# youmi-zym/TemporalStereo

Hardware: AMD Instinct MI355X
Metric: stereo pairs/sec, FlyingThings3D 540x960 D=192 (aggregation hot path) (higher is better)
Workload: dtype f32

## Files before the change

include/ts_hip.h:

```cpp
#ifndef TS_HIP_H
#define TS_HIP_H

#include <stddef.h>
#include <stdint.h>

#ifdef __cplusplus
extern "C" {
#endif

#define TS_OK 0
#define TS_ERR_NULL (-1)
#define TS_ERR_SHAPE (-2)
#define TS_ERR_UNSUPPORTED (-3)
#define TS_ERR_ALIGN (-4)

int ts_version(void);
const char* ts_last_error_string(void);

size_t ts_block_cost_workspace_bytes(int B, int C, int H, int W, int D, int scales);

int ts_block_cost_int_fwd(const float* left, const float* right, float* out, void* workspace,
                          int B, int C, int H, int W, int D, int scales, void* stream);

int ts_block_cost_sampled_fwd(const float* left, const float* right, const float* disp, float* out,
// ... 92 lines not shown

size_t ts_wasserstein_loss_workspace_bytes(int B, int H, int W);
int ts_wasserstein_loss_fwd(const float* cost, const float* offset, const float* sample, const float* gt, float* loss,
                            float* gt_scaled, void* workspace, int B, int D, int H, int W, int Hg, int Wg, float max_disp,
                            float start_disp, int sparse, void* stream);
int ts_wasserstein_loss_bwd(const float* cost, const float* offset, const float* sample, const float* gt_scaled,
                            const float* grad_loss, float* grad_cost, float* grad_offset, int B, int D, int H, int W, int Wg,
                            float max_disp, float start_disp, void* stream);
size_t ts_disp_smooth_l1_workspace_bytes(int B, int Hg, int Wg);
int ts_disp_smooth_l1_fwd(const float* est, const float* gt, float* loss_count, void* workspace, int B, int h, int w, int Hg,
                          int Wg, float max_disp, float start_disp, void* stream);
int ts_disp_smooth_l1_bwd(const float* est, const float* gt, const float* grad_loss, const float* loss_count, float* grad_est,
                          int B, int h, int w, int Hg, int Wg, float max_disp, float start_disp, void* stream);

size_t ts_disp_metrics_workspace_bytes(int B, int Hg, int Wg);
int ts_disp_metrics_fwd(const float* est0, const float* est1, const float* est2, const float* est3, int n_est, int h0, int w0,
                        int h1, int w1, int h2, int w2, int h3, int w3, const float* gt, const float* gt_right, int B, int Hg,
                        int Wg, float lb, float ub, int flags, float* out, void* workspace, void* stream);

#define TS_RENDER_EST_COLOR 1
#define TS_RENDER_GT_COLOR 2
#define TS_RENDER_ERR_CLASS 4
#define TS_RENDER_ERR_JET 8
#define TS_RENDER_U16 16
#define TS_RENDER_UINT8 32
#define TS_RENDER_CHW 64
#define TS_RENDER_BAR 128
#define TS_RENDER_CLIP 256
#define TS_RENDER_MAX_SHARED 512
#define TS_RENDER_MAX_GIVEN 1024
#define TS_RENDER_STATS_FLOATS 32
size_t ts_disp_render_workspace_bytes(int B, int Hg, int Wg);
int ts_disp_render_fwd(const float* est, const float* gt, const float* max_disp, const float* jet, int B, int h, int w, int Hg,
                       int Wg, int flags, float scale16, void* disp_color, void* err_class, void* err_jet, void* disp_u16,
                       float* stats, void* workspace, void* stream);

#define TS_FLOW_SPARSE 1
#define TS_FLOW_EST_HWC 2
#define TS_FLOW_GT_HWC 4
#define TS_FLOW_RENDER_EST_COLOR 1
#define TS_FLOW_RENDER_GT_COLOR 2
#define TS_FLOW_RENDER_ERR_CLASS 4
#define TS_FLOW_RENDER_STATS 8
#define TS_FLOW_RENDER_UINT8 16
#define TS_FLOW_RENDER_CHW 32
#define TS_FLOW_RENDER_MAX_SHARED 64
#define TS_FLOW_RENDER_MAX_GIVEN 128
#define TS_FLOW_RENDER_EST_HWC 256
#define TS_FLOW_RENDER_GT_HWC 512
#define TS_FLOW_STATS_FLOATS 16
#define TS_FLOW_U16_CHW 1
size_t ts_flow_metrics_workspace_bytes(int B, int Hg, int Wg);
int ts_flow_metrics_fwd(const float* est0, const float* est1, const float* est2, const float* est3, int n_est, int h0, int w0,
                        int h1, int w1, int h2, int w2, int h3, int w3, const float* gt, int B, int Hg, int Wg, float lb, float ub,
                        int flags, float* out, void* workspace, void* stream);
size_t ts_flow_render_workspace_bytes(int B, int Hg, int Wg);
int ts_flow_render_fwd(const float* est, const float* gt, const float* gt_val, const float* max_rad, const float* wheel, int B,
                       int h, int w, int Hg, int Wg, int flags, void* flow_color, void* err_class, float* stats, void* workspace,
                       void* stream);
int ts_flow_u16_decode_fwd(const void* raw, int B, int H, int W, int flags, float* flow, void* valid, void* stream);

#define TS_PREPARE_CHW 1
int ts_frames_prepare_fwd(const void* left, const void* right, int B, int Hs, int Ws, int flags, float mean0, float mean1,
                          float mean2, float std0, float std1, float std2, int H, int W, const int* crop, float* color_l,
                          float* color_r, long long color_stride, float* color_aug_l, float* color_aug_r,
                          long long color_aug_stride, void* stream);
int ts_intrinsics_pyramid_fwd(const void* K_norm, int is_fp64, int B, int kh, int kw, int S, float* K, float* inv_K, void* stream);
int ts_disp_u16_decode_fwd(const void* raw, int B, int H, int W, float scale, float* disp, void* valid, void* stream);

#define TS_AUGMENT_ROW_INTS 96
#define TS_AUGMENT_MAX_RECTS 4
#define TS_AUGMENT_GAMMA 1
size_t ts_frames_augment_workspace_bytes(int B, int Hs, int Ws);
int ts_frames_augment_fwd(const void* left, const void* right, int B, int Hs, int Ws, int flags, float mean0, float mean1,
                          float mean2, float std0, float std1, float std2, int H, int W, const int* table, float* color_l,
                          float* color_r, long long color_stride, float* color_aug_l, float* color_aug_r,
                          long long color_aug_stride, void* workspace, size_t workspace_bytes, void* stream);
int ts_disp_u16_window_fwd(const void* raw, int B, int Hs, int Ws, int H, int W, const int* table, float scale, float* disp,
                           void* valid, void* stream);

int ts_topk_softargmax_fwd(const float* cost, const float* sample, const float* offset, float* disp,
                           float* topk_disp, float* topk_cost, int* topk_index,
                           int B, int D, int H, int W, int k, void* stream);

int ts_topk_softargmax_bwd(const float* topk_disp, const float* topk_cost, const int* topk_index,
                           const float* disp, const float* grad_disp, const float* grad_topk_disp,
                           const float* grad_topk_cost, float* grad_cost, float* grad_sample,
                           int B, int D, int H, int W, int k, void* stream);

int ts_softargmin_fwd(const float* cost, const float* sample, float* disp, float temperature,
                      int normalize, int B, int D, int H, int W, void* stream);

int ts_softargmin_bwd(const float* cost, const float* sample, const float* disp, const float* grad_disp,
                      float* grad_cost, float* grad_sample, float temperature, int normalize,
                      int B, int D, int H, int W, void* stream);

int ts_argmax_select_fwd(const float* cost, const float* sample, float* disp, int* index,
                         int B, int D, int H, int W, void* stream);

int ts_softsplat_sum_fwd(const float* input, const float* flow, float* output,
                         int B, int C, int H, int W, void* stream);
int ts_softsplat_sum_fwd_deterministic(const float* input, const float* flow, float* output, void* workspace,
                                       int B, int C, int H, int W, void* stream);
int ts_softsplat_sum_bwd_input(const float* flow, const float* grad_output, float* grad_input,
                               int B, int C, int H, int W, void* stream);
int ts_softsplat_sum_bwd_flow(const float* input, const float* flow, const float* grad_output,
                              float* grad_flow, int B, int C, int H, int W, void* stream);
size_t ts_softsplat_softmax_workspace_bytes(int B, int C, int H, int W);
int ts_softsplat_softmax_fwd(const float* input, const float* flow, const float* metric, float* output,
                             void* workspace, int B, int C, int H, int W, void* stream);
int ts_project_to_3d_fwd(const float* depth, const float* K, const float* inv_K, const float* T,
                         float* triangular_depth, float* optical_flow, unsigned char* flow_mask,
                         int B, int C, int H, int W, int k_dim, int inv_k_dim, float eps, void* stream);

#define TS_WARP_DISPARITY 0
#define TS_WARP_FLOW 1
#define TS_WARP_DEPTH 2
#define TS_WARP_BILINEAR 0
#define TS_WARP_NEAREST 1
#define TS_WARP_BICUBIC 2
#define TS_WARP_ZEROS 0
#define TS_WARP_BORDER 1
#define TS_WARP_REFLECTION 2
int ts_inverse_warp_fwd(const float* img, const float* motion, const float* K, const float* inv_K, const float* T, float* out,
                        float* triangular_depth, float* src_pixel_coord, float* optical_flow, unsigned char* flow_mask,
                        float* homo_points_3d, int B, int C, int Hi, int Wi, int H, int W, int mode, int interp, int pad,
                        int k_dim, int inv_k_dim, float eps, void* stream);
int ts_inverse_warp_bwd(const float* img, const float* motion, const float* K, const float* inv_K, const float* T,
                        const float* grad_out, float* grad_img, float* grad_motion, int B, int C, int Hi, int Wi, int H, int W,
                        int mode, int interp, int pad, int k_dim, int inv_k_dim, float eps, void* stream);

int ts_raft_corr_pyramid_fwd(const float* fmap1, const float* fmap2, float* pyramid, int B, int C, int H, int W, int num_levels,
                             void* stream);
int ts_raft_corr_lookup_fwd(const float* pyramid, const float* disp, float* out, int B, int H, int W, int num_levels, int radius,
                            void* stream);
int ts_raft_corr_lookup_bwd(const float* pyramid, const float* disp, const float* grad_out, float* grad_disp, float* grad_pyramid,
                            int B, int H, int W, int num_levels, int radius, int fold, void* stream);
int ts_raft_corr_pyramid_bwd(const float* grad_pyramid, const float* fmap1, const float* fmap2, float* grad_fmap1, float* grad_fmap2,
                             int B, int C, int H, int W, int levels, void* stream);

int ts_flow_corr_pyramid_fwd(const float* fmap1, const float* fmap2, float* pyramid, int B, int C, int H, int W, int num_levels,
                             void* stream);
int ts_flow_corr_lookup_fwd(const float* pyramid, const float* coords, float* out, int B, int H, int W, int num_levels, int radius,
                            void* stream);
int ts_flow_corr_lookup_bwd(const float* pyramid, const float* coords, const float* grad_out, float* grad_coords, float* grad_pyramid,
                            int B, int H, int W, int num_levels, int radius, int fold, void* stream);
int ts_flow_corr_pyramid_bwd(const float* grad_pyramid, const float* fmap1, const float* fmap2, float* grad_fmap1, float* grad_fmap2,
                             int B, int C, int H, int W, int levels, void* stream);

int ts_spp3d_pool_fwd(const float* x, float* pooled, int B, int C, int D, int H, int W, int num_levels, int s0, int s1, int s2, int s3,
                      long long x_bstride, long long x_cstride, void* stream);
int ts_spp3d_pool_bwd(const float* g0, const float* g1, const float* g2, const float* g3, const float* addend, float* grad_x, int B,
                      int C, int D, int H, int W, int num_levels, int s0, int s1, int s2, int s3, long long addend_bstride,
                      long long addend_cstride, long long gx_bstride, long long gx_cstride, void* stream);
int ts_spp3d_expand_fwd(const float* x, const float* lv0, const float* lv1, const float* lv2, const float* lv3, float* cat, int B, int C,
                        int Cl, int D, int H, int W, int num_levels, int s0, int s1, int s2, int s3, long long x_bstride,
                        long long x_cstride, void* stream);
int ts_spp3d_expand_bwd(const float* grad_cat, float* g0, float* g1, float* g2, float* g3, int B, int C, int Cl, int D, int H, int W,
                        int num_levels, int s0, int s1, int s2, int s3, long long g_bstride, long long g_cstride, void* stream);
int ts_depth_sum3_fwd(const float* z0, const float* z1, const float* z2, const float* scale, const float* shift, float* y, int B, int C,
                      int D, int H, int W, int act, long long z0_bstride, long long z0_cstride, long long z1_bstride,
                      long long z1_cstride, long long z2_bstride, long long z2_cstride, long long y_bstride, long long y_cstride,
                      void* stream);

int ts_bn_small_train_bwd(const float* y, const float* g, const float* gamma, const float* beta, float* sum_g, float* sum_gx, float* dy,
                          int B, int C, int N, long long y_bstride, long long y_cstride, long long g_bstride, long long g_cstride,
                          long long dy_bstride, long long dy_cstride, float eps, int act, void* stream);

size_t ts_reproject_memory_workspace_bytes(int B, int h, int w, int k, int n_local_out);
int ts_reproject_memory_fwd(const float* prev_disp, long long disp_bstride, int full_h, int full_w,
                            const float* mem_disp, const float* mem_cost, int k,
                            const float* local_map, int n_local_in, int n_local_out,
                            const float* K, int k_dim, const float* T_a, const float* T_b,
                            const float* baseline_ptr, float baseline, float factor,
                            float* out_disp, float* out_cost, float* out_local, void* workspace,
                            int B, int h, int w, void* stream);

int ts_conv_cout_pad(int cout);
int ts_conv_weight_layout(const float* w, float* out, int A, int T, int nb, int bpad, long long stride_a, long long stride_b,
                          long long stride_t, int flip, void* stream);
typedef struct {
  const float* w; float* out;
  int A, T, nb, bpad;
  long long stride_a, stride_b, stride_t;
  int flip, reserved;
} ts_weight_layout_desc;
int ts_conv_weight_layout_many(const void* table, int n, int blocks_x, void* stream);
typedef struct {
  const float* w; float* out;
  int A, T, nb, col0;
  long long stride_a, stride_b, stride_t;
  long long out_stride_a, out_stride_t;
  int flip, reserved;
} ts_weight_layout_desc2;
int ts_conv_weight_layout_many2(const void* table, int n, int blocks_x, void* stream);
typedef struct { const float* part; float* dw; int gx, nitems, cob, Cin, Cout, KT, ciblocks, block0; } ts_wgrad_finish_desc;
int ts_conv_wgrad_defer(int on);
int ts_conv_wgrad_pending(void);
int ts_conv_wgrad_take(void* host_table, size_t capacity_bytes, int* n, int* total_blocks);
int ts_conv_wgrad_finish_many(const void* table, int n, int total_blocks, void* stream);
int ts_conv_set_chunk_cap(int cap);
int ts_conv3d_hw_fwd(const float* x, const float* w_t, const float* scale, const float* shift, float* y,
                     int B, int Cin, int Cout, int D, int H, int W, int stride, int dilation,
                     int transposed, int act, float act_param,
                     long long in_bstride, long long in_cstride, long long out_bstride,
                     long long out_cstride, const float* addend, long long addend_bstride,
                     void* workspace, size_t workspace_bytes, void* stream);
size_t ts_conv3d_hw_warp_workspace_bytes(int B, int Cout, int D, int H, int W);
int ts_conv3d_hw_warp_fwd(const float* corr, const float* w_t, const float* scale, const float* shift, float* y,
                          const float* q, const float* disp, const float* base,
                          int B, int Cc, int Cout, int D, int H, int W, int dilation, int act, float act_param,
                          long long in_bstride, long long in_cstride, long long out_bstride, long long out_cstride,
                          long long base_bstride, void* workspace, size_t workspace_bytes, void* stream);

size_t ts_conv3d_hw_workspace_bytes(int B, int Cin, int Cout, int D, int H, int W, int stride, int transposed);
int ts_conv3d_hw_x6_supported(int Cin, int Cout, int W, int stride, int dilation, int transposed);
size_t ts_conv3d_hw_x6_weight_bytes(int Cin, int Cout);
size_t ts_conv3d_hw_x6_workspace_bytes(int B, int Cin, int Cout, int D, int H, int W);
int ts_conv3d_hw_x6_weight_split(const float* w_t, void* w6, int Cin, int Cout, void* stream);
int ts_conv3d_hw_x6_weight_split_from(const float* w, void* w6, int Cin, int Cout, long long stride_ci, long long stride_co,
                                      long long stride_t, int flip, void* stream);
int ts_conv3d_hw_x6_fwd(const float* x, const void* w6, const float* scale, const float* shift, float* y,
                        int B, int Cin, int Cout, int D, int H, int W, int dilation, int act, float act_param,
                        long long in_bstride, long long in_cstride, long long out_bstride, long long out_cstride,
                        const float* addend, long long addend_bstride, void* workspace, size_t workspace_bytes, void* stream);
typedef struct ts_peer_ctx {
  void* region[8];
  int rank, world;
} ts_peer_ctx;
size_t ts_peer_region_bytes(void);
int ts_peer_max_floats(void);
int ts_peer_max_ranks(void);
int ts_peer_alloc(void** region, void* handle64);
int ts_peer_open(const void* handle64, void** region);
int ts_peer_close(void* region);
int ts_peer_free(void* region);
int ts_peer_status(const void* ctx, int* status, void* stream);
int ts_peer_status_async(const void* ctx, int* host_status, void* stream);
long long ts_peer_set_timeout_ms(long long ms);
int ts_peer_reset(const void* ctx, void* stream);
int ts_peer_all_gather(const void* ctx, const float* src, float* dst, int n, void* stream);
int ts_peer_all_reduce_sum(const void* ctx, float* buf, int n, const float* scale, void* stream);

int ts_conv3d_hw_x6s_supported(int Cin, int Cout, int H, int W, int mode);
size_t ts_conv3d_hw_x6s_weight_bytes(int Cin, int Cout, int mode);
int ts_conv3d_hw_x6s_weight_split(const float* w_t, void* w6, int Cin, int Cout, int w_pad, int mode, void* stream);
int ts_conv3d_hw_x6s_fwd(const float* x, const void* w6, const float* scale, const float* shift, float* y,
                         int B, int Cin, int Cout, int D, int H, int W, int mode, int act, float act_param,
                         long long in_bstride, long long in_cstride, long long out_bstride, long long out_cstride, void* stream);
int ts_conv3d_d_fwd(const float* x, const float* w_t, const float* scale, const float* shift, float* y,
                    int B, int Cin, int Cout, int Din, int H, int W, int k, int stride, int dilation,
                    int padding, int transposed, int act, float act_param,
                    long long in_bstride, long long in_cstride, long long out_bstride,
                    long long out_cstride, void* stream);
size_t ts_conv3d_bwd_weight_workspace_bytes(int Cin, int Cout, int taps);
int ts_conv3d_hw_bwd_data(const float* dy, const float* w_b, float* dx, int B, int Cin, int Cout, int D, int H, int W,
                          int stride, int dilation, int transposed, long long dy_bstride, long long dy_cstride,
                          long long dx_bstride, long long dx_cstride, void* stream);
int ts_conv3d_hw_bwd_weight(const float* x, const float* dy, float* dw, int B, int Cin, int Cout, int D, int H, int W,
                            int stride, int dilation, long long x_bstride, long long x_cstride, long long dy_bstride,
                            long long dy_cstride, void* workspace, size_t workspace_bytes, void* stream);
int ts_conv3d_d_bwd_data(const float* dy, const float* w_b, float* dx, int B, int Cin, int Cout, int Din, int H, int W,
                         int k, int stride, int dilation, int padding, int transposed, long long dy_bstride,
                         long long dy_cstride, long long dx_bstride, long long dx_cstride, void* stream);
int ts_conv3d_d_bwd_weight(const float* x, const float* dy, float* dw, int B, int Cin, int Cout, int Din, int H, int W,
                           int k, int stride, int dilation, int padding, long long x_bstride, long long x_cstride,
                           long long dy_bstride, long long dy_cstride, void* workspace, size_t workspace_bytes,
                           void* stream);
int ts_resize3d_add_act_fwd(const float* a, const float* add, float* out, int B, int C, int Da, int Ha, int Wa,
                            int D, int H, int W, int act, long long a_bstride, long long a_cstride,
                            long long add_bstride, long long add_cstride, long long out_bstride,
                            long long out_cstride, void* stream);
int ts_pool3d5_avgmax_fwd(const float* x, float* out_avg, float* out_max, int B, int C, int D, int H, int W,
                          long long x_bstride, long long x_cstride, long long avg_bstride, long long avg_cstride,
                          long long max_bstride, long long max_cstride, void* stream);
int ts_merge_candidates_fwd(const float* volume, const float* sample, const float* mem_sample, const float* mem_cost,
                            const float* past_w, const float* past_scale, const float* past_shift,
                            float* out_sample, float* out_volume, int B, int C, int D0, int K, int H, int W,
                            long long vol_bstride, long long vol_cstride, long long out_bstride,
                            long long out_cstride, void* stream);
int ts_convex_upsample_fwd(const float* mask, const float* disp, float* out, int B, int H, int W, int factor,
                           float disp_scale, void* stream);
int ts_convex_upsample_candidates_fwd(const float* mask, const float* disp, float* out, float* low, float* high,
                                      float* candidates, int B, int H, int W, int factor, float disp_scale, float range,
                                      int channel_offset, int channels_total, void* stream);
int ts_unet_upsample_fwd(const float* mask, const float* disp, float* out, int B, int h, int w, int Ho, int Wo,
                         void* stream);
int ts_convex_upsample_bwd(const float* mask, const float* disp, const float* grad_out, float* grad_mask, float* grad_disp,
                           int B, int H, int W, int factor, float disp_scale, void* stream);
int ts_unet_upsample_bwd(const float* mask, const float* disp, const float* grad_out, float* grad_mask, float* grad_disp,
                         void* workspace, int B, int h, int w, int Ho, int Wo, void* stream);
int ts_deconv2d_k4s2_fwd(const float* x, const float* w_t, const float* scale, const float* shift, float* y,
                         int B, int Cin, int Cout, int H, int W, int act, long long out_bstride, void* stream);
int ts_resize_bilinear_fwd(const float* x, float* out, int B, int C, int h, int w, int Ho, int Wo, float value_scale,
                           long long out_bstride, void* stream);
int ts_resize_bilinear_pair_fwd(const float* x0, const float* x1, float* out0, float* out1, int B, int C, int h, int w,
                                int Ho, int Wo, float value_scale0, float value_scale1, void* stream);
int ts_range_candidates_fwd(const float* disp, float* low, float* high, float* candidates, int B, int H, int W,
                            float range, int channel_offset, int channels_total, void* stream);

int ts_resize3d_add_act_bwd(const float* a, const float* add, const float* grad_out, float* grad_a, float* grad_add,
                            int B, int C, int Da, int Ha, int Wa, int D, int H, int W, int act, void* stream);
int ts_pool3d5_avgmax_bwd(const float* x, const float* grad_avg, const float* grad_max, float* grad_x,
                          int B, int C, int D, int H, int W, void* stream);
int ts_merge_candidates_bwd(const float* sample, const float* grad_out_volume, const float* grad_out_sample,
                            float* grad_volume, float* grad_sample, int B, int C, int DT, int H, int W, void* stream);

int ts_channel_splice_fwd(const float* first, const float* second, float* out, int B, int C, int mc, long long N,
                          long long first_bstride, long long second_bstride, long long out_bstride, void* stream);
int ts_copy_rows_fwd(const float* src, float* dst, long long rows, long long row_elems, long long src_pitch,
                     long long dst_pitch, void* stream);

typedef struct ts_opt_entry { float* param; const float* grad; float* square_avg; long long n; } ts_opt_entry;
int ts_candidates_in_range_fwd(const float* low, const float* high, float* candidates, int B, int H, int W,
                               int channel_offset, int channels_total, void* stream);
int ts_candidates_in_range_bwd(const float* low, const float* high, const float* grad_candidates, float* grad_low,
                               float* grad_high, int B, int H, int W, int channel_offset, int channels_total, void* stream);
int ts_offset_head_fwd(const float* x, float* y, long long n, float delta, void* stream);
int ts_offset_head_bwd(const float* x, const float* grad_y, float* grad_x, long long n, float delta, void* stream);
int ts_space_to_depth2_fwd(const float* x, float* z, int B, int C, int H, int W, void* stream);
int ts_deconv2d_k4s2_weight_to_conv3(const float* w, float* out, int Cin, int Cout, int cin_pad, void* stream);
int ts_deconv2d_k4s2_wgrad_from_conv3(const float* dw3, float* dw, int Cin, int Cout, void* stream);
typedef struct ts_bn_fold_entry { const float* gamma; const float* beta; const float* mean; const float* var; const float* bias;
                                  float* scale; float* shift; int C, pad; } ts_bn_fold_entry;
int ts_bn_fold_many(const void* table, int n, float eps, void* stream);
size_t ts_clip_rmsprop_workspace_bytes(int n_tensors);
int ts_clip_rmsprop_step(const void* table, int n_tensors, float max_norm, float lr, float alpha, float eps,
                         void* workspace, size_t workspace_bytes, void* stream);

typedef struct ts_plan ts_plan;
ts_plan* ts_plan_create(void);
void ts_plan_destroy(ts_plan* plan);
// ... 14 lines not shown
```

temporalstereo_amd/_lib.py:

```python
import ctypes
import os
import threading

_HERE = os.path.dirname(os.path.abspath(__file__))
LIB_PATH = os.path.join(_HERE, "libts_hip.so")

_lock = threading.Lock()
_lib = None

c_f32p = ctypes.c_void_p
c_ptr = ctypes.c_void_p
c_int = ctypes.c_int
c_size = ctypes.c_size_t
c_float = ctypes.c_float

SIGNATURES = {
    "ts_version": (c_int, []),
    "ts_last_error_string": (ctypes.c_char_p, []),
    "ts_block_cost_workspace_bytes": (c_size, [c_int] * 6),
    "ts_block_cost_int_fwd": (c_int, [c_f32p, c_f32p, c_f32p, c_ptr] + [c_int] * 6 + [c_ptr]),
    "ts_block_cost_sampled_fwd": (c_int, [c_f32p, c_f32p, c_f32p, c_f32p, c_ptr] + [c_int] * 6 + [c_ptr]),
    "ts_block_cost_sampled_warped_fwd": (c_int, [c_f32p, c_f32p, c_f32p, c_f32p, c_ptr] + [c_int] * 6 + [c_ptr]),
    "ts_block_cost_sampled_corr_fwd": (c_int, [c_f32p, c_f32p, c_f32p, c_f32p, c_ptr] + [c_int] * 6 + [c_ptr]),
    "ts_block_cost_corr_split_supported": (c_int, [c_int] * 2),
    "ts_block_cost_sampled_corr_split_fwd": (c_int, [c_f32p] * 6 + [c_ptr] + [c_int] * 7 + [ctypes.c_longlong] * 4 + [c_ptr]),
    "ts_conv3d_hw_split_supported": (c_int, [c_int] * 10),
    "ts_conv3d_hw_split_fwd": (c_int, [c_f32p] * 6 + [c_int] * 11 + [c_float] + [ctypes.c_longlong] * 6 +
                               [c_f32p, ctypes.c_longlong, c_ptr, c_size, c_ptr]),
    "ts_conv3d_d_split_supported": (c_int, [c_int] * 2),
    "ts_conv3d_d_split_fwd": (c_int, [c_f32p] * 6 + [c_int] * 13 + [c_float] + [ctypes.c_longlong] * 6 + [c_ptr]),
    "ts_conv3d_hw_x6_split_supported": (c_int, [c_int] * 5),
    "ts_conv3d_hw_x6_split_fwd": (c_int, [c_f32p, c_f32p, c_ptr, c_f32p, c_f32p, c_f32p] + [c_int] * 9 + [c_float] + [ctypes.c_longlong] * 6 +
                                  [c_f32p, ctypes.c_longlong, c_ptr, c_size, c_ptr]),
    "ts_conv3d_hw_warp_workspace_bytes": (c_size, [c_int] * 5),
    "ts_conv3d_hw_warp_fwd": (c_int, [c_f32p] * 8 + [c_int] * 8 + [c_float] + [ctypes.c_longlong] * 5 + [c_ptr, c_size, c_ptr]),
    "ts_cat_fms_fwd": (c_int, [c_f32p] * 4 + [c_int] * 5 + [c_ptr]),
    "ts_inverse_warp_3d_fwd": (c_int, [c_f32p] * 3 + [c_int] * 5 + [c_ptr]),
    "ts_dif_fms_workspace_bytes": (c_size, []),
    "ts_dif_fms_fwd": (c_int, [c_f32p] * 4 + [c_ptr] + [c_int] * 5 + [c_ptr]),
    "ts_correlation_fwd": (c_int, [c_f32p] * 3 + [c_int] * 7 + [c_ptr]),
    "ts_correlation_bwd": (c_int, [c_f32p] * 6 + [c_int] * 7 + [c_ptr]),
    "ts_block_cost_bwd_workspace_bytes": (c_size, [c_int] * 6),
    "ts_block_cost_int_bwd": (c_int, [c_f32p] * 5 + [c_ptr] + [c_int] * 6 + [c_ptr]),
    "ts_block_cost_sampled_bwd": (c_int, [c_f32p] * 7 + [c_ptr] + [c_int] * 6 + [c_ptr]),
    "ts_block_cost_sampled_warped_bwd": (c_int, [c_f32p] * 7 + [c_ptr] + [c_int] * 6 + [c_ptr]),
    "ts_calib_stream": (c_int, [c_int, c_ptr, c_ptr, c_size, c_ptr]),
    "ts_candidates_in_range_fwd": (c_int, [c_f32p] * 3 + [c_int] * 5 + [c_ptr]),
    "ts_candidates_in_range_bwd": (c_int, [c_f32p] * 5 + [c_int] * 5 + [c_ptr]),
    "ts_offset_head_fwd": (c_int, [c_f32p] * 2 + [ctypes.c_longlong, c_float, c_ptr]),
    "ts_offset_head_bwd": (c_int, [c_f32p] * 3 + [ctypes.c_longlong, c_float, c_ptr]),
    "ts_space_to_depth2_fwd": (c_int, [c_f32p] * 2 + [c_int] * 4 + [c_ptr]),
    "ts_deconv2d_k4s2_weight_to_conv3": (c_int, [c_f32p] * 2 + [c_int] * 3 + [c_ptr]),
    "ts_deconv2d_k4s2_wgrad_from_conv3": (c_int, [c_f32p] * 2 + [c_int] * 2 + [c_ptr]),
    "ts_bn_fold_many": (c_int, [c_ptr, c_int, c_float, c_ptr]),
    "ts_clip_rmsprop_workspace_bytes": (c_size, [c_int]),
    "ts_clip_rmsprop_step": (c_int, [c_ptr, c_int] + [c_float] * 4 + [c_ptr, c_size, c_ptr]),
    "ts_topk_softargmax_fwd": (c_int, [c_f32p] * 7 + [c_int] * 5 + [c_ptr]),
    "ts_topk_softargmax_bwd": (c_int, [c_f32p] * 9 + [c_int] * 5 + [c_ptr]),
    "ts_softargmin_fwd": (c_int, [c_f32p] * 3 + [c_float, c_int] + [c_int] * 4 + [c_ptr]),
    "ts_softargmin_bwd": (c_int, [c_f32p] * 6 + [c_float, c_int] + [c_int] * 4 + [c_ptr]),
    "ts_argmax_select_fwd": (c_int, [c_f32p] * 4 + [c_int] * 4 + [c_ptr]),
    "ts_bn_workspace_bytes": (c_size, [c_int, c_int, ctypes.c_longlong]),
    "ts_channel_splice_fwd": (c_int, [c_f32p] * 3 + [c_int] * 3 + [ctypes.c_longlong] * 4 + [c_ptr]),
    "ts_bn_sync_merge": (c_int, [c_f32p, c_int, c_int] + [c_f32p] * 4 + [c_float, c_f32p, c_ptr]),
    "ts_bn_train_fwd": (c_int, [c_f32p] * 5 + [c_float, c_ptr] + [c_f32p] * 3 + [c_ptr, c_int, c_int] + [ctypes.c_longlong] * 5 +
                        [c_float, c_int, c_ptr]),
    "ts_bn_train_bwd": (c_int, [c_f32p] * 9 + [c_ptr, c_int, c_int] + [ctypes.c_longlong] * 5 + [c_float, c_int, c_float, c_ptr]),
    "ts_bn_stats_fwd": (c_int, [c_f32p] * 5 + [c_float, c_ptr, c_ptr, c_int, c_int] + [ctypes.c_longlong] * 3 + [c_ptr]),
    "ts_bn_apply_act_fwd": (c_int, [c_f32p] * 6 + [c_int, c_int] + [ctypes.c_longlong] * 5 + [c_float, c_int, c_ptr]),
    "ts_bn_act_bwd_reduce": (c_int, [c_f32p] * 8 + [c_ptr, c_int, c_int] + [ctypes.c_longlong] * 5 + [c_float, c_int, c_ptr]),
    "ts_bn_act_bwd_apply": (c_int, [c_f32p] * 9 + [c_int, c_int] + [ctypes.c_longlong] * 5 + [c_float, c_int, c_int, c_float, c_ptr]),
    "ts_wasserstein_loss_workspace_bytes": (c_size, [c_int] * 3),
    "ts_wasserstein_loss_fwd": (c_int, [c_f32p] * 6 + [c_ptr] + [c_int] * 6 + [c_float, c_float, c_int, c_ptr]),
    "ts_wasserstein_loss_bwd": (c_int, [c_f32p] * 7 + [c_int] * 5 + [c_float, c_float, c_ptr]),
    "ts_disp_smooth_l1_workspace_bytes": (c_size, [c_int] * 3),
    "ts_disp_smooth_l1_fwd": (c_int, [c_f32p] * 3 + [c_ptr] + [c_int] * 5 + [c_float, c_float, c_ptr]),
    "ts_disp_smooth_l1_bwd": (c_int, [c_f32p] * 5 + [c_int] * 5 + [c_float, c_float, c_ptr]),
    "ts_disp_metrics_workspace_bytes": (c_size, [c_int] * 3),
    "ts_disp_metrics_fwd": (c_int, [c_f32p] * 4 + [c_int] * 9 + [c_f32p] * 2 + [c_int] * 3 + [c_float, c_float, c_int, c_f32p, c_ptr, c_ptr]),
    "ts_disp_render_workspace_bytes": (c_size, [c_int] * 3),
    "ts_disp_render_fwd": (c_int, [c_f32p] * 4 + [c_int] * 6 + [c_float] + [c_ptr] * 4 + [c_f32p, c_ptr, c_ptr]),
    "ts_flow_metrics_workspace_bytes": (c_size, [c_int] * 3),
    "ts_flow_metrics_fwd": (c_int, [c_f32p] * 4 + [c_int] * 9 + [c_f32p] + [c_int] * 3 + [c_float, c_float, c_int, c_f32p, c_ptr, c_ptr]),
    "ts_flow_render_workspace_bytes": (c_size, [c_int] * 3),
    "ts_flow_render_fwd": (c_int, [c_f32p] * 5 + [c_int] * 6 + [c_ptr] * 2 + [c_f32p, c_ptr, c_ptr]),
    "ts_flow_u16_decode_fwd": (c_int, [c_ptr] + [c_int] * 4 + [c_f32p, c_ptr, c_ptr]),
    "ts_frames_prepare_fwd": (c_int, [c_ptr] * 2 + [c_int] * 4 + [c_float] * 6 + [c_int] * 2 + [c_ptr] + [c_f32p] * 2 +
                              [ctypes.c_longlong] + [c_f32p] * 2 + [ctypes.c_longlong, c_ptr]),
    "ts_intrinsics_pyramid_fwd": (c_int, [c_ptr] + [c_int] * 5 + [c_f32p] * 2 + [c_ptr]),
    "ts_disp_u16_decode_fwd": (c_int, [c_ptr] + [c_int] * 3 + [c_float, c_f32p, c_ptr, c_ptr]),
    "ts_frames_augment_workspace_bytes": (c_size, [c_int] * 3),
    "ts_frames_augment_fwd": (c_int, [c_ptr] * 2 + [c_int] * 4 + [c_float] * 6 + [c_int] * 2 + [c_ptr] + [c_f32p] * 2 +
                              [ctypes.c_longlong] + [c_f32p] * 2 + [ctypes.c_longlong, c_ptr, c_size, c_ptr]),
    "ts_disp_u16_window_fwd": (c_int, [c_ptr] + [c_int] * 5 + [c_ptr, c_float, c_f32p, c_ptr, c_ptr]),
    "ts_softsplat_sum_fwd": (c_int, [c_f32p] * 3 + [c_int] * 4 + [c_ptr]),
    "ts_softsplat_sum_fwd_deterministic": (c_int, [c_f32p] * 3 + [c_ptr] + [c_int] * 4 + [c_ptr]),
    "ts_softsplat_sum_bwd_input": (c_int, [c_f32p] * 3 + [c_int] * 4 + [c_ptr]),
    "ts_softsplat_sum_bwd_flow": (c_int, [c_f32p] * 4 + [c_int] * 4 + [c_ptr]),
    "ts_softsplat_softmax_workspace_bytes": (c_size, [c_int] * 4),
    "ts_softsplat_softmax_fwd": (c_int, [c_f32p] * 4 + [c_ptr] + [c_int] * 4 + [c_ptr]),
    "ts_conv_cout_pad": (c_int, [c_int]),
    "ts_peer_region_bytes": (c_size, []),
    "ts_peer_max_floats": (c_int, []),
    "ts_peer_max_ranks": (c_int, []),
    "ts_peer_alloc": (c_int, [ctypes.POINTER(c_ptr), c_ptr]),
    "ts_peer_open": (c_int, [c_ptr, ctypes.POINTER(c_ptr)]),
    "ts_peer_close": (c_int, [c_ptr]),
    "ts_peer_free": (c_int, [c_ptr]),
    "ts_peer_status": (c_int, [c_ptr, ctypes.POINTER(c_int), c_ptr]),
    "ts_bn_set_small_elems": (ctypes.c_longlong, [ctypes.c_longlong]),
    "ts_channel_sum_fwd": (c_int, [c_f32p, c_f32p, c_ptr, c_int, c_int, ctypes.c_longlong, ctypes.c_longlong, ctypes.c_longlong, c_ptr]),
    "ts_peer_status_async": (c_int, [c_ptr, c_ptr, c_ptr]),
    "ts_peer_set_timeout_ms": (ctypes.c_longlong, [ctypes.c_longlong]),
    "ts_peer_reset": (c_int, [c_ptr, c_ptr]),
    "ts_peer_all_gather": (c_int, [c_ptr, c_f32p, c_f32p, c_int, c_ptr]),
    "ts_peer_all_reduce_sum": (c_int, [c_ptr, c_f32p, c_int, c_f32p, c_ptr]),
    "ts_conv_weight_layout": (c_int, [c_f32p, c_f32p] + [c_int] * 4 + [ctypes.c_longlong] * 3 + [c_int, c_ptr]),
    "ts_conv_weight_layout_many": (c_int, [c_ptr, c_int, c_int, c_ptr]),
    "ts_conv_weight_layout_many2": (c_int, [c_ptr, c_int, c_int, c_ptr]),
    "ts_conv_wgrad_defer": (c_int, [c_int]),
    "ts_conv_wgrad_pending": (c_int, []),
    "ts_conv_wgrad_take": (c_int, [c_ptr, c_size, ctypes.POINTER(c_int), ctypes.POINTER(c_int)]),
    "ts_conv_wgrad_finish_many": (c_int, [c_ptr, c_int, c_int, c_ptr]),
    "ts_conv_set_chunk_cap": (c_int, [c_int]),
    "ts_conv3d_hw_x6_supported": (c_int, [c_int] * 6),
    "ts_conv3d_hw_x6_weight_bytes": (ctypes.c_size_t, [c_int] * 2),
    "ts_conv3d_hw_x6_weight_split": (c_int, [c_f32p, c_ptr, c_int, c_int, c_ptr]),
    "ts_conv3d_hw_x6_weight_split_from": (c_int, [c_f32p, c_ptr, c_int, c_int] + [ctypes.c_longlong] * 3 + [c_int, c_ptr]),
    "ts_conv3d_hw_x6_workspace_bytes": (c_size, [c_int] * 6),
    "ts_conv3d_hw_x6s_supported": (c_int, [c_int] * 5),
    "ts_conv3d_hw_x6s_weight_bytes": (c_size, [c_int] * 3),
    "ts_conv3d_hw_x6s_weight_split": (c_int, [c_f32p, c_ptr, c_int, c_int, c_int, c_int, c_ptr]),
    "ts_conv3d_hw_x6s_fwd": (c_int, [c_f32p, c_ptr, c_f32p, c_f32p, c_f32p] + [c_int] * 8 + [c_float] + [ctypes.c_longlong] * 4 + [c_ptr]),
    "ts_conv3d_hw_x6_fwd": (c_int, [c_f32p, c_ptr, c_f32p, c_f32p, c_f32p] + [c_int] * 8 + [c_float] + [ctypes.c_longlong] * 4 +
                            [c_f32p, ctypes.c_longlong, c_ptr, c_size, c_ptr]),
    "ts_conv3d_hw_fwd": (c_int, [c_f32p] * 5 + [c_int] * 10 + [c_float] + [ctypes.c_longlong] * 4 +
                         [c_f32p, ctypes.c_longlong, c_ptr, c_size, c_ptr]),
    "ts_conv3d_hw_workspace_bytes": (c_size, [c_int] * 8),
    "ts_conv3d_hw_bwd_data": (c_int, [c_f32p] * 3 + [c_int] * 9 + [ctypes.c_longlong] * 4 + [c_ptr]),
    "ts_conv3d_bwd_weight_workspace_bytes": (ctypes.c_size_t, [c_int] * 3),
    "ts_conv3d_hw_bwd_weight": (c_int, [c_f32p] * 3 + [c_int] * 8 + [ctypes.c_longlong] * 4 + [c_ptr, ctypes.c_size_t, c_ptr]),
    "ts_conv3d_d_bwd_data": (c_int, [c_f32p] * 3 + [c_int] * 11 + [ctypes.c_longlong] * 4 + [c_ptr]),
    "ts_conv3d_d_bwd_weight": (c_int, [c_f32p] * 3 + [c_int] * 10 + [ctypes.c_longlong] * 4 + [c_ptr, ctypes.c_size_t, c_ptr]),
    "ts_conv3d_d_fwd": (c_int, [c_f32p] * 5 + [c_int] * 12 + [c_float] + [ctypes.c_longlong] * 4 + [c_ptr]),
    "ts_resize3d_add_act_fwd": (c_int, [c_f32p] * 3 + [c_int] * 9 + [ctypes.c_longlong] * 6 + [c_ptr]),
    "ts_pool3d5_avgmax_fwd": (c_int, [c_f32p] * 3 + [c_int] * 5 + [ctypes.c_longlong] * 6 + [c_ptr]),
    "ts_merge_candidates_fwd": (c_int, [c_f32p] * 9 + [c_int] * 6 + [ctypes.c_longlong] * 4 + [c_ptr]),
    "ts_convex_upsample_fwd": (c_int, [c_f32p] * 3 + [c_int] * 4 + [c_float, c_ptr]),
    "ts_convex_upsample_candidates_fwd": (c_int, [c_f32p] * 6 + [c_int] * 4 + [c_float, c_float, c_int, c_int, c_ptr]),
    "ts_unet_upsample_fwd": (c_int, [c_f32p] * 3 + [c_int] * 5 + [c_ptr]),
    "ts_convex_upsample_bwd": (c_int, [c_f32p] * 5 + [c_int] * 4 + [c_float, c_ptr]),
    "ts_unet_upsample_bwd": (c_int, [c_f32p] * 5 + [c_ptr] + [c_int] * 5 + [c_ptr]),
    "ts_deconv2d_k4s2_fwd": (c_int, [c_f32p] * 5 + [c_int] * 6 + [ctypes.c_longlong, c_ptr]),
    "ts_resize_bilinear_fwd": (c_int, [c_f32p] * 2 + [c_int] * 6 + [c_float, ctypes.c_longlong, c_ptr]),
    "ts_resize_bilinear_pair_fwd": (c_int, [c_f32p] * 4 + [c_int] * 6 + [c_float, c_float, c_ptr]),
    "ts_range_candidates_fwd": (c_int, [c_f32p] * 4 + [c_int] * 3 + [c_float, c_int, c_int, c_ptr]),
    "ts_project_to_3d_fwd": (c_int, [c_f32p] * 7 + [c_int] * 6 + [c_float, c_ptr]),
    "ts_inverse_warp_fwd": (c_int, [c_f32p] * 9 + [c_ptr, c_f32p] + [c_int] * 11 + [c_float, c_ptr]),
    "ts_inverse_warp_bwd": (c_int, [c_f32p] * 8 + [c_int] * 11 + [c_float, c_ptr]),
    "ts_raft_corr_pyramid_fwd": (c_int, [c_f32p] * 3 + [c_int] * 5 + [c_ptr]),
    "ts_raft_corr_lookup_fwd": (c_int, [c_f32p] * 3 + [c_int] * 5 + [c_ptr]),
    "ts_raft_corr_lookup_bwd": (c_int, [c_f32p] * 5 + [c_int] * 6 + [c_ptr]),
    "ts_raft_corr_pyramid_bwd": (c_int, [c_f32p] * 5 + [c_int] * 5 + [c_ptr]),
    "ts_flow_corr_pyramid_fwd": (c_int, [c_f32p] * 3 + [c_int] * 5 + [c_ptr]),
    "ts_flow_corr_lookup_fwd": (c_int, [c_f32p] * 3 + [c_int] * 5 + [c_ptr]),
    "ts_flow_corr_lookup_bwd": (c_int, [c_f32p] * 5 + [c_int] * 6 + [c_ptr]),
    "ts_flow_corr_pyramid_bwd": (c_int, [c_f32p] * 5 + [c_int] * 5 + [c_ptr]),
    "ts_spp3d_pool_fwd": (c_int, [c_f32p] * 2 + [c_int] * 10 + [ctypes.c_longlong] * 2 + [c_ptr]),
    "ts_spp3d_pool_bwd": (c_int, [c_f32p] * 6 +[c_int] * 10 + [ctypes.c_longlong] * 4 + [c_ptr]),
    "ts_spp3d_expand_fwd": (c_int, [c_f32p] * 6 + [c_int] * 11 + [ctypes.c_longlong] * 2 + [c_ptr]),
    "ts_spp3d_expand_bwd": (c_int, [c_f32p] * 5 + [c_int] * 11 + [ctypes.c_longlong] * 2 + [c_ptr]),
    "ts_depth_sum3_fwd": (c_int, [c_f32p] * 6 + [c_int] * 6 + [ctypes.c_longlong] * 8 + [c_ptr]),
    "ts_bn_small_train_bwd": (c_int, [c_f32p] * 7 + [c_int] * 3 + [ctypes.c_longlong] * 6 + [c_float, c_int, c_ptr]),
    "ts_reproject_memory_workspace_bytes": (c_size, [c_int] * 5),
    "ts_reproject_memory_fwd": (c_int, [c_f32p, ctypes.c_longlong, c_int, c_int, c_f32p, c_f32p, c_int, c_f32p, c_int, c_int,
                                        c_f32p, c_int, c_f32p, c_f32p, c_f32p, c_float, c_float, c_f32p, c_f32p, c_f32p,
                                        c_ptr, c_int, c_int, c_int, c_ptr]),
    "ts_resize3d_add_act_bwd": (c_int, [c_f32p] * 5 + [c_int] * 9 + [c_ptr]),
    "ts_pool3d5_avgmax_bwd": (c_int, [c_f32p] * 4 + [c_int] * 5 + [c_ptr]),
    "ts_merge_candidates_bwd": (c_int, [c_f32p] * 5 + [c_int] * 5 + [c_ptr]),
    "ts_copy_rows_fwd": (c_int, [c_f32p] * 2 + [ctypes.c_longlong] * 4 + [c_ptr]),
    "ts_plan_create": (c_ptr, []),
    "ts_plan_destroy": (None, [c_ptr]),
    "ts_plan_length": (c_int, [c_ptr]),
    "ts_plan_add_call": (c_int, [c_ptr, ctypes.c_char_p, ctypes.POINTER(ctypes.c_ulonglong), c_int]),
    "ts_plan_run": (c_int, [c_ptr]),
    "ts_stream_fork": (c_int, [c_ptr, c_ptr]),
    "ts_event_record": (c_int, [c_int, c_ptr]),
    "ts_event_wait": (c_int, [c_int, c_ptr]),
}

_QUERIES = frozenset(n for n in SIGNATURES if n.endswith("_bytes") or n.startswith("ts_plan_") or
                     n.endswith("_split_supported") or
                     n in ("ts_version", "ts_last_error_string", "ts_conv_cout_pad", "ts_conv3d_hw_x6_supported", "ts_conv3d_hw_x6s_supported", "ts_peer_max_floats", "ts_peer_max_ranks",
                           "ts_peer_alloc", "ts_peer_open", "ts_peer_close", "ts_peer_free", "ts_peer_status", "ts_peer_status_async",
                           "ts_peer_set_timeout_ms", "ts_peer_reset", "ts_bn_set_small_elems",
                           "ts_conv_wgrad_defer", "ts_conv_wgrad_pending", "ts_conv_wgrad_take"))


def lib():
    rec = getattr(_tls, "recorder", None)
    if rec is not None:
        return rec.proxy
    return _real_lib()


def _real_lib():
    global _lib
    if _lib is None:
        with _lock:
            if _lib is None:
                if not os.path.exists(LIB_PATH):
                    raise RuntimeError(
                        "temporalstereo_amd: %s is missing -- build it with "
                        "`python -m temporalstereo_amd.build` (there is no fallback path)" % LIB_PATH)
                handle = ctypes.CDLL(LIB_PATH)
# ... 116 lines not shown
```

temporalstereo_amd/aggregation/native.py:

```python
import os
import time

import torch
import torch.nn as nn

from .. import _lib
from .. import functional as TF

ACT_NONE, ACT_SILU, ACT_RELU, ACT_TANH_OFFSET, ACT_HEAD_PAIR = 0, 1, 2, 3, 4


def _stream():
    return _lib.current_stream_handle()


_PAR = {"on": False, "aux": None, "kinds": frozenset(__import__("os").environ.get("TS_BRANCHES", "hourglass").split(","))}


def _aux_stream():
    return _PAR["aux"]


_STAGE_CAP = int(os.environ.get("TS_STAGE_CHUNK_CAP", "8"))

# ... 354 lines not shown
        _lib.ptr(second)
    ob, oc = _strides5(out)
    if out_second is not None:
        if second is None or out.shape[0] != 1 or out_second.shape != out.shape or _strides5(out_second)[1] != oc:
            raise ValueError("conv_hw(out_second=...): needs `second` and two outputs of one shape and channel stride")
        ob = (out_second.data_ptr() - out.data_ptr()) // 4
        _lib.ptr(out_second)
    L = _lib.lib()
    if X6 and X6S and addend is None and (stride == 2 or transposed) and dilation == 1:
        mode = X6S_T3 if transposed else X6S_S2
        if L.ts_conv3d_hw_x6s_supported(Cin, f.cout, H, W, mode) and x6s_grid(B, f.cout, D, H, W, mode) >= (_X6S_MIN_GRID_T3 if transposed else _X6S_MIN_GRID):
            rc = L.ts_conv3d_hw_x6s_fwd(_lib.ptr(x), _lib.ptr(x6s_weights(f, mode)), _lib.ptr(f.scale), _lib.ptr(f.shift), _lib.ptr(out),
                                        B, Cin, f.cout, D, H, W, mode, f.act if act is None else act, float(act_param),
                                        ib, ic, ob, oc, _stream())
            _lib.check(rc, "ts_conv3d_hw_x6s_fwd")
            return out
    wsb = int(L.ts_conv3d_hw_workspace_bytes(B, Cin, f.cout, D, H, W, stride, int(transposed)))
    x6_grid = ((H + 7) // 8) * ((W + 31) // 32) * D * B * ((f.cout + 31) // 32)
    x6_ok = X6 and L.ts_conv3d_hw_x6_supported(Cin, f.cout, W, stride, dilation, int(transposed))
    wsb6 = int(L.ts_conv3d_hw_x6_workspace_bytes(B, Cin, f.cout, D, H, W)) if x6_ok else 0
    if x6_ok and Cin < 32 and x6_grid < 512:
        x6_ok = False
    if x6_ok and (x6_grid >= _X6_MIN_GRID or wsb6 or (not wsb and x6_grid >= _X6_MIN_GRID_UNSPLIT)):
        ws6 = torch.empty(wsb6, device=x.device, dtype=torch.uint8) if wsb6 else None
        if split is not None:
            rc = L.ts_conv3d_hw_x6_split_fwd(_lib.ptr(x), _lib.ptr(split), _lib.ptr(x6_weights(f)), _lib.ptr(f.scale), _lib.ptr(f.shift),
                                             _lib.ptr(out), B, Cin, Cs, f.cout, D, H, W, dilation, f.act if act is None else act,
                                             float(act_param), ib, ic, i2b, i2c, ob, oc, _lib.ptr(addend),
                                             addend.stride(0) if addend is not None else 0, _lib.ptr(ws6), wsb6, _stream())
            _lib.check(rc, "ts_conv3d_hw_x6_split_fwd")
            return out
        rc = L.ts_conv3d_hw_x6_fwd(_lib.ptr(x), _lib.ptr(x6_weights(f)), _lib.ptr(f.scale), _lib.ptr(f.shift), _lib.ptr(out),
                                   B, Cin, f.cout, D, H, W, dilation, f.act if act is None else act, float(act_param),
                                   ib, ic, ob, oc, _lib.ptr(addend), addend.stride(0) if addend is not None else 0, _lib.ptr(ws6), wsb6,
                                   _stream())
        _lib.check(rc, "ts_conv3d_hw_x6_fwd")
        return out
    ws = torch.empty(wsb, device=x.device, dtype=torch.uint8) if wsb else None
    if split is not None:
        rc = L.ts_conv3d_hw_split_fwd(_lib.ptr(x), _lib.ptr(split), _lib.ptr(f.w), _lib.ptr(f.scale), _lib.ptr(f.shift), _lib.ptr(out),
                                      B, Cin, Cs, f.cout, D, H, W, stride, dilation, 0, f.act if act is None else act,
                                      float(act_param), ib, ic, i2b, i2c, ob, oc, _lib.ptr(addend),
                                      addend.stride(0) if addend is not None else 0, _lib.ptr(ws), wsb, _stream())
        _lib.check(rc, "ts_conv3d_hw_split_fwd")
        return out
    rc = L.ts_conv3d_hw_fwd(_lib.ptr(x), _lib.ptr(f.w), _lib.ptr(f.scale), _lib.ptr(f.shift), _lib.ptr(out),
                            B, Cin, f.cout, D, H, W, stride, dilation, int(transposed),
                            f.act if act is None else act, float(act_param), ib, ic, ob, oc,
                            _lib.ptr(addend), addend.stride(0) if addend is not None else 0, _lib.ptr(ws), wsb, _stream())
    _lib.check(rc, "ts_conv3d_hw_fwd")
    return out


def conv_d(x, f, k, stride=1, dilation=1, padding=0, transposed=False, out=None, act=None, act_param=0.0):
    split = None
    if isinstance(x, Split):
        x, split = x.a, x.b
    B, Cin, Din, H, W = x.shape
    if split is not None:
        Cs, Cin = Cin, Cin + split.shape[1]
        i2b, i2c = _strides5(split)
    assert Cin == f.cin, (Cin, f.cin)
    Dout = 2 * Din if transposed else (Din + 2 * padding - dilation * (k - 1) - 1) // stride + 1
    if out is None:
        out = torch.empty((B, f.cout, Dout, H, W), device=x.device, dtype=torch.float32)
    ib, ic = _strides5(x)
    ob, oc = _strides5(out)
    if split is not None:
        rc = _lib.lib().ts_conv3d_d_split_fwd(_lib.ptr(x), _lib.ptr(split), _lib.ptr(f.w), _lib.ptr(f.scale), _lib.ptr(f.shift),
                                              _lib.ptr(out), B, Cin, Cs, f.cout, Din, H, W, k, stride, dilation, padding,
                                              int(transposed), f.act if act is None else act, float(act_param),
                                              ib, ic, i2b, i2c, ob, oc, _stream())
        _lib.check(rc, "ts_conv3d_d_split_fwd")
        return out
    rc = _lib.lib().ts_conv3d_d_fwd(_lib.ptr(x), _lib.ptr(f.w), _lib.ptr(f.scale), _lib.ptr(f.shift), _lib.ptr(out),
                                    B, Cin, f.cout, Din, H, W, k, stride, dilation, padding, int(transposed),
                                    f.act if act is None else act, float(act_param), ib, ic, ob, oc, _stream())
    _lib.check(rc, "ts_conv3d_d_fwd")
    return out


FUSED_K1 = os.environ.get("TS_FUSED_K1", "1") != "0"
SPLIT_INPUT = os.environ.get("TS_SPLIT_INPUT", "1") != "0"


def block_cost_corr(left, right, disp, scales):
    return TF.block_cost_corr(left, right, disp, scales)


def conv_hw_warp(corr, f, q, disp, base, dilation=1):
    B, Cc, D, H, W = corr.shape
    assert Cc == f.cin, (Cc, f.cin)
    out = torch.empty((B, f.cout, D, H, W), device=corr.device, dtype=torch.float32)
    ib, ic = _strides5(corr)
    ob, oc = _strides5(out)
    wsb = TF._q("ts_conv3d_hw_warp_workspace_bytes", B, f.cout, D, H, W)
    ws = torch.empty(wsb, device=corr.device, dtype=torch.uint8)
    rc = _lib.lib().ts_conv3d_hw_warp_fwd(_lib.ptr(corr), _lib.ptr(f.w), _lib.ptr(f.scale), _lib.ptr(f.shift), _lib.ptr(out),
                                          _lib.ptr(q), _lib.ptr(disp), _lib.ptr(base), B, Cc, f.cout, D, H, W, dilation, f.act, 0.0,
                                          ib, ic, ob, oc, base.stride(0) if base is not None else 0, _lib.ptr(ws), wsb, _stream())
    _lib.check(rc, "ts_conv3d_hw_warp_fwd")
    return out


def resize_add_act(a, add, size, act=ACT_SILU):
    B, C, Da, Ha, Wa = a.shape
    D, H, W = size
    out = torch.empty((B, C, D, H, W), device=a.device, dtype=torch.float32)
    ab, ac = _strides5(a)
    bb, bc = _strides5(add) if add is not None else (0, 0)
    ob, oc = _strides5(out)
    rc = _lib.lib().ts_resize3d_add_act_fwd(_lib.ptr(a), _lib.ptr(add), _lib.ptr(out), B, C, Da, Ha, Wa, D, H, W, act,
                                            ab, ac, bb, bc, ob, oc, _stream())
    _lib.check(rc, "ts_resize3d_add_act_fwd")
    return out


def pool5(x, out_avg, out_max):
    B, C, D, H, W = x.shape
    xb, xc = _strides5(x); ab, ac = _strides5(out_avg); mb, mc = _strides5(out_max)
    rc = _lib.lib().ts_pool3d5_avgmax_fwd(_lib.ptr(x), _lib.ptr(out_avg), _lib.ptr(out_max), B, C, D, H, W,
                                          xb, xc, ab, ac, mb, mc, _stream())
    _lib.check(rc, "ts_pool3d5_avgmax_fwd")


def resize_bilinear(x, size, value_scale=1.0, out=None):
    B, C, h, w = x.shape
    if out is None:
        out = torch.empty((B, C, size[0], size[1]), device=x.device, dtype=torch.float32)
    x = _lib.contiguous(x)
    rc = _lib.lib().ts_resize_bilinear_fwd(_lib.ptr(x), _lib.ptr(out), B, C, h, w, size[0], size[1],
                                           float(value_scale), out.stride(0), _stream())
    _lib.check(rc, "ts_resize_bilinear_fwd")
    return out


def resize_bilinear_pair(x0, x1, size, scale0, scale1):
    B, C, h, w = x0.shape
    if x1.shape != x0.shape:
        raise RuntimeError("resize_bilinear_pair: shapes differ")
    o0 = torch.empty((B, C, size[0], size[1]), device=x0.device, dtype=torch.float32)
    o1 = torch.empty_like(o0)
    x0, x1 = _lib.contiguous(x0), _lib.contiguous(x1)
    rc = _lib.lib().ts_resize_bilinear_pair_fwd(_lib.ptr(x0), _lib.ptr(x1), _lib.ptr(o0), _lib.ptr(o1),
                                                B, C, h, w, size[0], size[1], float(scale0), float(scale1), _stream())
    _lib.check(rc, "ts_resize_bilinear_pair_fwd")
    return o0, o1


def copy_rows(src, dst):
    B = src.shape[0]
    n = src[0].numel()
    src = _lib.contiguous(src)
    rc = _lib.lib().ts_copy_rows_fwd(_lib.ptr(src), _lib.ptr(dst), B, n, n, dst.stride(0), _stream())
    _lib.check(rc, "ts_copy_rows_fwd")


def range_candidates(disp, rng, extra_front=0):
    B, _, H, W = disp.shape
    low = torch.empty_like(disp)
    high = torch.empty_like(disp)
    cand = torch.empty((B, extra_front + 5, H, W), device=disp.device, dtype=torch.float32)
    rc = _lib.lib().ts_range_candidates_fwd(_lib.ptr(disp), _lib.ptr(low), _lib.ptr(high), _lib.ptr(cand), B, H, W,
                                            float(rng), extra_front, extra_front + 5, _stream())
    _lib.check(rc, "ts_range_candidates_fwd")
    return low, high, cand
# ... 39 lines not shown
        return conv_d(y, self.f1, self.k, self.stride, self.dil, self.pad_d, self.transposed, out=out)


class Hourglass:

    def __init__(self, mod):
        self.c1, self.c2, self.c3, self.c4 = (SepConv(getattr(mod, n)) for n in ("conv1", "conv2", "conv3", "conv4"))
        self.c5, self.c6 = SepConv(mod.conv5, True), SepConv(mod.conv6, True)
        self.s5, self.s6 = SepConv(mod.shortcut5), SepConv(mod.shortcut6)
        self.c4.f1.act = ACT_SILU

    def __call__(self, x):
        pre = self.c2(self.c1(x))
        br = Branch("hourglass")
        with br:
            s6 = self.s6(x)
            s5 = self.s5(pre)
        out = self.c5(self.c4(self.c3(pre)))
        br.join()
        out = resize_add_act(out, s5, pre.shape[-3:])
        return resize_add_act(self.c6(out), s6, x.shape[-3:])


class Heads:

    def __init__(self, mod):
        self.delta = float(mod.delta)
        c0, self.c1 = fold_wrapper(mod.cost_head[0], "d"), fold_wrapper(mod.cost_head[1], "hw")
        o0, self.o1 = fold_wrapper(mod.off_head[0], "d"), fold_wrapper(mod.off_head[1], "hw")
        self.C = C = c0.cout
        self.co0 = fold_concat(c0, o0)
        f = object.__new__(Folded)
        f.cin, f.cout, f.kind, f.act, f.kshape = 2 * C, 2, "hw", ACT_HEAD_PAIR, self.c1.kshape
        pad = int(_lib.lib().ts_conv_cout_pad(2))
        f.w = torch.zeros(2 * C, self.c1.w.shape[1], pad, device=self.c1.w.device, dtype=torch.float32)
        f.w[:C, :, 0] = self.c1.w[:, :, 0]
        f.w[C:, :, 1] = self.o1.w[:, :, 0]
        f.scale = torch.ones(pad, device=f.w.device); f.shift = torch.zeros(pad, device=f.w.device)
        f.scale[0], f.scale[1] = self.c1.scale[0], self.o1.scale[0]
        f.shift[0], f.shift[1] = self.c1.shift[0], self.o1.shift[0]
        f._tape = _TAPE
        if _TAPE is not None:
            for k, (m, g) in enumerate(((mod.cost_head[1], self.c1), (mod.off_head[1], self.o1))):
                _TAPE.layout(f.w[k * C:(k + 1) * C], m.weight.detach(), False, col0=k)
                _TAPE.fold(f.scale[k:k + 1], f.shift[k:k + 1], m.bias, getattr(m, "norm", None), 1)
        self.pair = f

    def __call__(self, x):
        y = conv_d(x, self.co0, 3, 1, 1, 1)
        B, _, D, H, W = y.shape
        both = torch.empty((2, B, D, H, W), device=y.device, dtype=torch.float32)
        conv_hw(y, self.pair, out=both.permute(1, 0, 2, 3, 4), act_param=self.delta)
        return both[0], both[1]


class ConvexUp:

    def __init__(self, mod):
        self.r, self.k = mod.upscale_factor, mod.window_size
        if self.k != 3:
            raise NotImplementedError("window_size != 3")
        self.m0 = Folded(mod.mask[0].weight.unsqueeze(2), mod.mask[0].bias, mod.mask[1], ACT_SILU, False, "hw")
        w3 = mod.mask[3].weight
        self.m3 = Folded(w3.reshape(w3.shape[0], w3.shape[1], 1, 1, 1), mod.mask[3].bias, None, ACT_NONE, False, "d")

    def mask(self, feat):
        return conv_d(conv_hw(feat.unsqueeze(2), self.m0), self.m3, 1)

    def with_candidates(self, feat, disp, m, rng, extra_front=0):
        B, _, H, W = disp.shape
        if m is None:
            m = self.mask(feat)
        Ho, Wo = H * self.r, W * self.r
        out = torch.empty((B, 1, Ho, Wo), device=disp.device, dtype=torch.float32)
        low, high = torch.empty_like(out), torch.empty_like(out)
        cand = torch.empty((B, extra_front + 5, Ho, Wo), device=disp.device, dtype=torch.float32)
        disp = _lib.contiguous(disp)
        rc = _lib.lib().ts_convex_upsample_candidates_fwd(_lib.ptr(m), _lib.ptr(disp), _lib.ptr(out), _lib.ptr(low),
                                                          _lib.ptr(high), _lib.ptr(cand), B, H, W, self.r, float(self.r), float(rng),
                                                          extra_front, extra_front + 5, _stream())
        _lib.check(rc, "ts_convex_upsample_candidates_fwd")
        return out, low, high, cand

    def __call__(self, feat, disp, m=None):
        B, _, H, W = disp.shape
        if m is None:
            m = self.mask(feat)
        out = torch.empty((B, 1, H * self.r, W * self.r), device=disp.device, dtype=torch.float32)
        disp = _lib.contiguous(disp)
        rc = _lib.lib().ts_convex_upsample_fwd(_lib.ptr(m), _lib.ptr(disp), _lib.ptr(out), B, H, W, self.r,
                                               float(self.r), _stream())
        _lib.check(rc, "ts_convex_upsample_fwd")
        return out


class _LevelBase:
    def __init__(self, mod):
        self.mod = mod
        self.C, self.topk, self.scales = mod.C, mod.topk, mod.block_cost_scale
        self.init0, self.hg, self.init2 = SepConv(mod.init3d[0]), Hourglass(mod.init3d[1]), SepConv(mod.init3d[2])
        self.heads = Heads(mod.pred_heads)

    def init3d(self, raw, addend=None):
        return self.init2(self.hg(self.init0(raw, addend=addend)))

    def split_reference_half(self):
        if self.init0.stride != 1 or self.init0.transposed:
            raise NotImplementedError("first aggregation layer is not a stride-1 conv over [left | warped | corr]")
        self.init0_left, self.init0.f0, self.init0_corr, self.init0_q = split_sampled_first_layer(self.init0.f0, self.scales)

    def left_term(self, left):
        return conv_hw(left.unsqueeze(2), self.init0_left, 1, self.init0.dil)

    def right_term(self, right):
        return conv_d(right.unsqueeze(2), self.init0_q, 1).squeeze(2)

    def first_layer_fused(self, left, right, ds, lterm, rterm):
        corr = block_cost_corr(left, right, ds, self.scales)
        i0 = self.init0
        y = conv_hw_warp(corr, self.init0_corr, rterm, ds, lterm.squeeze(2) if lterm.dim() == 5 else lterm, i0.dil)
        return conv_d(y, i0.f1, i0.k, i0.stride, i0.dil, i0.pad_d, i0.transposed)

    def init3d_from(self, first):
        return self.init2(self.hg(first))

    def feature_terms(self, left, right):
        return self.left_term(left), (self.right_term(right) if FUSED_K1 else None)


class _MergingLevel(_LevelBase):
    def __init__(self, mod):
        super().__init__(mod)
        pc = mod.past_conv
        f = fold_wrapper(pc, "d")
        self.past_w = f.w.reshape(-1)[:self.C].contiguous()
        self.past_scale, self.past_shift = f.scale[:self.C].contiguous(), f.shift[:self.C].contiguous()
        self.fusion = mod.spatial_fusion
        if self.fusion:
            self.conv5 = fold_wrapper(mod.fuse.conv_5x5, "d")
            self.fuse_conv = SepConv(mod.fuse.conv_fuse)
        self.up = ConvexUp(mod.convex_upsample)

    def merge(self, vol, samples, prev_info, resize_memory):
        B, C, D0, H, W = vol.shape
        K = self.topk
        memory = prev_info.get('cost_memory', None)
        mem_s = mem_c = None
        if memory is not None and prev_info.get('use_past_cost', False):
            mem_s, mem_c = memory['disp_sample'], memory['cost_volume']
            if resize_memory:
                mem_s, mem_c = resize_bilinear_pair(mem_s, mem_c, (H, W), W / mem_s.shape[-1], 1.0)
            mem_s, mem_c = _lib.contiguous(mem_s), _lib.contiguous(mem_c)
        Dm = D0 + K
        nch = 4 * C if self.fusion else C
        cat4 = torch.empty((B, nch, Dm, H, W), device=vol.device, dtype=torch.float32)
        samp = torch.empty((B, Dm, H, W), device=vol.device, dtype=torch.float32)
        x0 = cat4[:, :C]
        vb, vc = _strides5(vol); ob, oc = _strides5(x0)
        rc = _lib.lib().ts_merge_candidates_fwd(_lib.ptr(vol), _lib.ptr(samples), _lib.ptr(mem_s), _lib.ptr(mem_c),
                                                _lib.ptr(self.past_w), _lib.ptr(self.past_scale), _lib.ptr(self.past_shift),
                                                _lib.ptr(samp), _lib.ptr(x0), B, C, D0, K, H, W, vb, vc, ob, oc, _stream())
        _lib.check(rc, "ts_merge_candidates_fwd")
        return cat4, samp

    def fuse(self, cat4):
        C = self.C
        x0 = cat4[:, :C]
        if not self.fusion:
            return x0
        br = Branch("pool")
        with br:
            pool5(x0, cat4[:, 2 * C:3 * C], cat4[:, 3 * C:])
        conv_d(x0, self.conv5, 5, 1, 1, 2, out=cat4[:, C:2 * C])
        br.join()
        return self.fuse_conv(cat4)

    def merge_fuse_predict(self, vol, samples, prev_info, feat, resize_memory, mask=None, next_range=None):
        cat4, samp = self.merge(vol, samples, prev_info, resize_memory)
        cost, off = self.heads(self.fuse(cat4))
        disp, _, _ = TF.topk_softargmax(cost, samp, off, k=self.topk)
        if callable(mask):
            mask = mask()
        if next_range is not None:
            return self.up.with_candidates(feat, disp, mask, *next_range), cost, off, samp
        return self.up(feat, disp, mask), cost, off, samp


class NativeCoarse(_MergingLevel):
    def early(self, left, right):
        return self.init3d(TF.block_cost(left, right, int(self.mod.num_sample), self.scales))

    def __call__(self, left, right, prev_info, mask=None, next_range=None, vol=None):
        if vol is None:
            vol = self.early(left, right)
        return self.merge_fuse_predict(vol, None, prev_info, left, resize_memory=True, mask=mask, next_range=next_range)


class NativeFine(_MergingLevel):
    def __init__(self, mod):
        super().__init__(mod)
        self.split_reference_half()

    def early(self, left, right, ds, terms=None):
        lt, rt = terms() if callable(terms) else (terms if terms is not None else self.feature_terms(left, right))
        if rt is not None:
            return self.init3d_from(self.first_layer_fused(left, right, ds, lt, rt))
        return self.init3d(TF.block_cost_warped(left, right, ds, self.scales), lt)

    def __call__(self, left, right, ds, prev_info, mask=None, terms=None, next_range=None, vol=None):
        if vol is None:
            vol = self.early(left, right, ds, terms)
        return self.merge_fuse_predict(vol, ds, prev_info, left, resize_memory=False, mask=mask, next_range=next_range)


class SplitBoth:

    def __init__(self, left, right, spx4):
        self.left, self.right, self.spx4 = left, right, spx4

    device = property(lambda self: self.spx4.device)
    shape = property(lambda self: (self.spx4.shape[0], self.left.shape[1] + self.spx4.shape[1]) + tuple(self.spx4.shape[2:]))

    def pair(self):
        B = self.left.shape[0]
        return Split(self.left, self.spx4[:B]), Split(self.right, self.spx4[B:])

    def __getitem__(self, idx):
        return torch.cat([s.cat() for s in self.pair()], 0)[idx]


class NativePrecise(_LevelBase):
    def __init__(self, mod):
        super().__init__(mod)
        u = mod.refinement
        self.enc = [fold_wrapper(m, "hw") for m in (u.conv2[0], u.conv2[1], u.conv4[0], u.conv4[1])]
        self.enc_stride = [u.conv2[0].stride[0], u.conv2[1].stride[0], u.conv4[0].stride[0], u.conv4[1].stride[0]]
        self.fuse = [fold_wrapper(u.fuse[0], "hw"), fold_wrapper(u.fuse[1], "hw")]
        self.deconv4 = Folded(u.deconv4.weight, u.deconv4.bias, u.deconv4.norm, _act_code(u.deconv4.activation), True, "deconv2d")
        self.concat = fold_wrapper(u.concat, "hw")
        self.deconv2 = Folded(u.deconv2.weight, u.deconv2.bias, None, ACT_NONE, True, "deconv2d")
        self.in_planes = mod.in_planes
        self.split_reference_half()

    @staticmethod
    def _c2d(x, f, stride, out=None):
        return conv_hw(x, f, stride, 1, out=out)

    def encode(self, left_image, right_image, cat4, s2_left):
        B = left_image.shape[0]
        e, st = self.enc, self.enc_stride
        li, ri = left_image.unsqueeze(2), right_image.unsqueeze(2)
        s2_right = torch.empty((B,) + tuple(s2_left.shape[1:]), device=li.device, dtype=torch.float32)
        if B == 1:
            x = conv_hw(li, e[0], st[0], 1, second=ri)
            conv_hw(x[:1], e[1], st[1], 1, out=s2_left, second=x[1:], out_second=s2_right)
            x = conv_hw(s2_left, e[2], st[2], 1, second=s2_right)
        else:
            Hx, Wx = (li.shape[-2] - 1) // st[0] + 1, (li.shape[-1] - 1) // st[0] + 1
            x = torch.empty((2 * B, e[0].cout, 1, Hx, Wx), device=li.device, dtype=torch.float32)
            conv_hw(li, e[0], st[0], 1, out=x[:B]); conv_hw(ri, e[0], st[0], 1, out=x[B:])
            conv_hw(x[:B], e[1], st[1], 1, out=s2_left); conv_hw(x[B:], e[1], st[1], 1, out=s2_right)
            Hy, Wy = (s2_left.shape[-2] - 1) // st[2] + 1, (s2_left.shape[-1] - 1) // st[2] + 1
            y = torch.empty((2 * B, e[2].cout, 1, Hy, Wy), device=li.device, dtype=torch.float32)
            conv_hw(s2_left, e[2], st[2], 1, out=y[:B]); conv_hw(s2_right, e[2], st[2], 1, out=y[B:])
            x = y
        self._c2d(x, e[3], st[3], out=(cat4.spx4 if isinstance(cat4, SplitBoth) else cat4[:, self.in_planes:]).unsqueeze(2))

    def _deconv(self, x, f, out, out_bstride):
        B, Cin, H, W = x.shape
        L = _lib.lib()
        if X6 and X6S and L.ts_conv3d_hw_x6s_supported(Cin, f.cout, H, W, X6S_T4) and x6s_grid(B, f.cout, 1, H, W, X6S_T4) >= _X6S_MIN_GRID:
            rc = L.ts_conv3d_hw_x6s_fwd(_lib.ptr(x), _lib.ptr(x6s_weights(f, X6S_T4)), _lib.ptr(f.scale), _lib.ptr(f.shift), _lib.ptr(out),
                                        B, Cin, f.cout, 1, H, W, X6S_T4, f.act, 0.0, Cin * H * W, H * W, out_bstride, 4 * H * W, _stream())
            _lib.check(rc, "ts_conv3d_hw_x6s_fwd")
            return
        rc = _lib.lib().ts_deconv2d_k4s2_fwd(_lib.ptr(x), _lib.ptr(f.w), _lib.ptr(f.scale), _lib.ptr(f.shift), _lib.ptr(out),
                                             B, Cin, f.cout, H, W, f.act, out_bstride, _stream())
        _lib.check(rc, "ts_deconv2d_k4s2_fwd")

    def unet_features(self, left, right, left_image, right_image):
        both, lterm, st = self.unet_encode(left, right, left_image, right_image)
        return both, (self.unet_decode(st), lterm)

    def split_input_ok(self, B, Cf, H, W):
        L = _lib.lib()
        if self.in_planes != Cf or self.enc[3].cout != Cf:
            return False
        hw = lambda f, dil: L.ts_conv3d_hw_split_supported(B, 2 * Cf, Cf, f.cout, 1, H, W, 1, dil, 0)
        return bool(L.ts_block_cost_corr_split_supported(2 * Cf, Cf) and hw(self.init0_left, self.init0.dil) and hw(self.fuse[0], 1) and
                    (not FUSED_K1 or L.ts_conv3d_d_split_supported(2 * Cf, Cf)) and
                    (not X6 or not L.ts_conv3d_hw_x6_supported(2 * Cf, self.fuse[0].cout, W, 1, 1, 0) or
                     L.ts_conv3d_hw_x6_split_supported(2 * Cf, Cf, self.fuse[0].cout, W, 1)))

    def unet_encode(self, left, right, left_image, right_image):
        B, Cf, H, W = left.shape
        if SPLIT_INPUT and FUSED_K1 and self.split_input_ok(B, Cf, H, W):
            left, right = _lib.contiguous(left), _lib.contiguous(right)
            both = SplitBoth(left, right, torch.empty((2 * B, Cf, H, W), device=left.device, dtype=torch.float32))
            lcat, rcat = both.pair()
        else:
            both = torch.empty((2 * B, 2 * Cf, H, W), device=left.device, dtype=torch.float32)
            lcat, rcat = both[:B], both[B:]
            copy_rows(left, lcat[:, :Cf]); copy_rows(right, rcat[:, :Cf])
        C32, C2 = self.deconv4.cout, self.enc[1].cout
        cat2 = torch.empty((B, C32 + C2, 2 * H, 2 * W), device=left.device, dtype=torch.float32)
        self.encode(left_image, right_image, both, cat2[:, C32:].unsqueeze(2))
        lterm = self.feature_terms(lcat, rcat)
        return both, lterm, (lcat, cat2, B, H, W)

    def unet_decode(self, st):
        lcat, cat2, B, H, W = st
        f = self._c2d(self._c2d(lcat.unsqueeze(2), self.fuse[0], 1), self.fuse[1], 1).squeeze(2)
        self._deconv(_lib.contiguous(f), self.deconv4, cat2, cat2.stride(0))
        g = _lib.contiguous(self._c2d(cat2.unsqueeze(2), self.concat, 1).squeeze(2))
        mask = torch.empty((B, 9, 4 * H, 4 * W), device=lcat.device, dtype=torch.float32)
        self._deconv(g, self.deconv2, mask, mask.stride(0))
        return mask

    def early(self, both, lterm, ds):
        B = both.shape[0] // 2
        lcat, rcat = both.pair() if isinstance(both, SplitBoth) else (both[:B], both[B:])
        lt, rt = lterm
        if rt is not None:
            return self.init3d_from(self.first_layer_fused(lcat, rcat, ds, lt, rt))
        return self.init3d(TF.block_cost_warped(lcat, rcat, ds, self.scales), lt)

    def __call__(self, both, mask_lterm, ds, prev_info, vol=None):
        B = both.shape[0] // 2
        H, W = both.shape[-2:]
        mask, lterm = mask_lterm
        mask = mask() if callable(mask) else mask
        if vol is None:
            vol = self.early(both, lterm, ds)
        cost, off = self.heads(vol)
        disp, mem_s, mem_c = TF.topk_softargmax(cost, ds, off, k=self.topk)
        full = torch.empty((B, 1, 4 * H, 4 * W), device=both.device, dtype=torch.float32)
        rc = _lib.lib().ts_unet_upsample_fwd(_lib.ptr(mask), _lib.ptr(disp), _lib.ptr(full), B, H, W, 4 * H, 4 * W, _stream())
        _lib.check(rc, "ts_unet_upsample_fwd")
        prev_info['prev_disp'] = full
        mem_s, mem_c = resize_bilinear_pair(mem_s, mem_c, (H // 2, W // 2), 0.5, 1.0)
        prev_info['cost_memory'] = {'disp_sample': mem_s, 'cost_volume': mem_c}
        return full, disp, cost, off, ds


class NativeAggregator:

    def __init__(self, net, private_streams=False):
        if net.training:
            raise RuntimeError("NativeAggregator folds BatchNorm: put the module in eval() first")
        if any(p.device.type != "cuda" for p in net.parameters()):
            raise RuntimeError("NativeAggregator needs the module on the GPU (there is no CPU path)")
        dev = next(net.parameters()).device
        self.device = dev
        with torch.cuda.device(dev):
            self._build(net)
            torch.cuda.synchronize(dev)
        self.fast, self.aux = qualified_streams(dev, 2, private=private_streams)
        self._extra_streams = qualified_streams(dev, 3, private=True)
        self._stage_sets = {}
        self.pipeline_slot = None
        self.overlap = True

    def _build(self, net):
        self.tape = Tape()
        with self.tape:
            self.coarse, self.fine, self.precise = NativeCoarse(net.coarse), NativeFine(net.fine), NativePrecise(net.precise)

    def refresh_weights(self):
        with torch.cuda.device(self.device):
            self.tape.refresh(self.device)

    def _coarse_level(self, l16, r16, prev_info, out, mask=None, vol=None):
        rng = 4
        disps, costs, offs, samples, ranges = out
        lm = prev_info.get('local_map', None)
        nl = lm.shape[1] if (lm is not None and prev_info.get('local_map_size', 0) > 0) else 0
        (d, low, high, ds), c, o, s = self.coarse(_lib.contiguous(l16), _lib.contiguous(r16), prev_info, mask, (rng, nl), vol=vol)
        if nl:
            resize_bilinear(lm, d.shape[-2:], d.shape[-1] / lm.shape[-1], out=ds[:, :nl])
        disps.append(d); costs.append(c); offs.append(o); samples.append(s); ranges.append({'low': low, 'high': high})
        return ds

    def _fine_level(self, l8, r8, ds, prev_info, out, mask=None, terms=None, vol=None):
        rng = 4
        disps, costs, offs, samples, ranges = out
        (d, low, high, ds), c, o, s = self.fine(_lib.contiguous(l8), _lib.contiguous(r8), ds, prev_info, mask, terms, (rng, 0), vol=vol)
        disps.append(d); costs.append(c); offs.append(o); samples.append(s); ranges.append({'low': low, 'high': high})
        return ds

    def _stages_for(self, batch):
        nst = int(os.environ.get("TS_STAGES", "6" if batch == 1 else "5"))
        key = (nst, os.environ.get("TS_STAGE_ORDER", ""), batch == 1)
        smap = os.environ.get("TS_STAGE_MAP", "")
        if smap:
            key = ("map", smap)
            if key not in self._stage_sets:
                pool = [self.fast, self.aux] + list(self._extra_streams)
                S = {"coarse": self.fast, "fine": self.aux, "unet": None, "coarse2": self.fast, "fine2": self.aux, "tail": None, "unet2": None}
                for item in smap.split(","):
                    role, idx = item.split(":")
                    S[role] = None if idx == "m" else pool[int(idx)]
                self._stage_sets[key] = S
            return self._stage_sets[key]
        if key not in self._stage_sets:
            extra = self._extra_streams[:max(0, min(nst, 6) - 3)]
            S = {"coarse": self.fast, "fine": self.aux}
            order = [r for r in os.environ.get("TS_STAGE_ORDER", "unet,coarse2,fine2" if batch == 1 else "unet,unet2").split(",") if r]
            order += [r for r in ("unet", "coarse2", "fine2", "tail", "unet2") if r not in order]
            parent = {"unet": None, "coarse2": "coarse", "fine2": "fine", "tail": None, "unet2": "unet"}
            for i, role in enumerate(order):
                S[role] = extra[i] if i < len(extra) else None
            for role in order:
                if S[role] is None and parent[role]:
                    S[role] = S[parent[role]]
            self._stage_sets[key] = S
        return self._stage_sets[key]

    def _staged_pass(self, l4, l8, l16, r4, r8, r16, left_image, right_image, prev_info, out):
        L = _lib.lib()
        main = torch.cuda.current_stream()
        slot = self.pipeline_slot
        P = lambda st: _lib.ctypes.c_void_p(st.cuda_stream)
        S = {k: (v if v is not None else main) for k, v in self._stages_for(l4.shape[0]).items()}
        for st in {id(v): v for v in S.values() if v is not main}.values():
            _lib.check(L.ts_event_wait(slot, P(st)), "ts_event_wait")
        on = torch.cuda.stream

        def edge(a, b):
            if a is not b:
                _edge(a, b)
        try:
            _chunk_cap(8)
            l16c, r16c, l8c, r8c = _lib.contiguous(l16), _lib.contiguous(r16), _lib.contiguous(l8), _lib.contiguous(r8)
            with on(S["coarse"]):
                mc = self.coarse.up.mask(l16c)
                cvol = self.coarse.early(l16c, r16c)
            with on(S["fine"]):
                mf = self.fine.up.mask(l8c)
                ltf = self.fine.feature_terms(l8c, r8c)
            with on(S["unet"]):
                both, lterm, ust = self.precise.unet_encode(l4, r4, left_image, right_image)
            edge(S["unet"], S["unet2"])
            with on(S["unet2"]):
                mask = self.precise.unet_decode(ust)
            edge(S["coarse"], S["coarse2"])
            with on(S["coarse2"]):
                ds = self._coarse_level(l16, r16, prev_info, out, lambda: mc, vol=cvol)
            edge(S["coarse2"], S["fine"])
            with on(S["fine"]):
                fvol = self.fine.early(l8c, r8c, ds, ltf)
            edge(S["fine"], S["fine2"])
            with on(S["fine2"]):
                ds = self._fine_level(l8, r8, ds, prev_info, out, lambda: mf, None, vol=fvol)
            edge(S["fine2"], S["tail"]); edge(S["unet"], S["tail"])
            with on(S["tail"]):
                pvol = self.precise.early(both, lterm, ds)
            edge(S["tail"], main); edge(S["unet2"], main)
            res = self.precise(both, (mask, lterm), ds, prev_info, vol=pvol)
            _lib.check(L.ts_event_record(slot, P(main)), "ts_event_record")
        finally:
            _chunk_cap(32)
        return res

    @torch.no_grad()
    def begin(self, left_feats, right_feats, left_image, right_image, slots):
        with torch.cuda.device(self.device):
            L = _lib.lib()
            P = lambda st: _lib.ctypes.c_void_p(st.cuda_stream)
            l4, l8, l16 = left_feats
            r4, r8, r16 = right_feats
            left_image, right_image = _lib.contiguous(left_image), _lib.contiguous(right_image)
            _lib.check(L.ts_event_wait(slots[0], P(self.fast)), "ts_event_wait")
            _lib.check(L.ts_event_wait(slots[0], P(self.aux)), "ts_event_wait")
            try:
                _chunk_cap(8)
                with torch.cuda.stream(self.aux):
                    mc, mf = self.coarse.up.mask(_lib.contiguous(l16)), self.fine.up.mask(_lib.contiguous(l8))
                    ltf = self.fine.feature_terms(_lib.contiguous(l8), _lib.contiguous(r8))
                    _lib.check(L.ts_event_record(slots[1], P(self.aux)), "ts_event_record")
                with torch.cuda.stream(self.fast):
                    vol = self.coarse.early(_lib.contiguous(l16), _lib.contiguous(r16))
                with torch.cuda.stream(self.aux):
                    both, mask = self.precise.unet_features(l4, r4, left_image, right_image)
            finally:
                _chunk_cap(32)
            return dict(mc=mc, mf=mf, ltf=ltf, vol=vol, both=both, mask=mask, feats=(l8, l16, r8, r16), slots=slots)

    @torch.no_grad()
    def finish(self, ctx, prev_info):
        with torch.cuda.device(self.device):
            L = _lib.lib()
            P = lambda st: _lib.ctypes.c_void_p(st.cuda_stream)
            main = torch.cuda.current_stream()
            l8, l16, r8, r16 = ctx["feats"]
            out = ([], [], [], [], [])
            disps, costs, offs, samples, ranges = out
            _edge(main, self.fast)
            try:
                _chunk_cap(8)
                with torch.cuda.stream(self.fast):
                    _lib.check(L.ts_event_wait(ctx["slots"][1], P(self.fast)), "ts_event_wait")
                    ds = self._coarse_level(l16, r16, prev_info, out, ctx["mc"], vol=ctx["vol"])
                    ds = self._fine_level(l8, r8, ds, prev_info, out, ctx["mf"], ctx["ltf"])
                _edge(self.fast, main)
                _edge(self.aux, main)
                full, d, c, o, s = self.precise(ctx["both"], ctx["mask"], ds, prev_info)
                _lib.check(L.ts_event_record(ctx["slots"][0], P(main)), "ts_event_record")
            finally:
                _chunk_cap(32)
            disps += [d, full]; costs.append(c); offs.append(o); samples.append(s)
            return disps[::-1], costs[::-1], samples[::-1], offs[::-1], ranges[::-1], prev_info

    @torch.no_grad()
    def __call__(self, left_feats, right_feats, left_image, right_image, prev_info):
        if left_image.device != self.device:
            raise RuntimeError("NativeAggregator lives on %s, inputs are on %s" % (self.device, left_image.device))
        with torch.cuda.device(self.device):
            return self._pass(left_feats, right_feats, left_image, right_image, prev_info)

    def _pass(self, left_feats, right_feats, left_image, right_image, prev_info):
        l4, l8, l16 = left_feats
        r4, r8, r16 = right_feats
        out = ([], [], [], [], [])
        disps, costs, offs, samples, ranges = out
        left_image, right_image = _lib.contiguous(left_image), _lib.contiguous(right_image)
        if self.overlap and self.pipeline_slot is not None:
            full, d, c, o, s = self._staged_pass(l4, l8, l16, r4, r8, r16, left_image, right_image, prev_info, out)
# ... 40 lines not shown
```

temporalstereo_amd/csrc/conv_x6s.hip:

```cpp
#include "conv_common.hpp"

namespace {

enum { XS_S2 = 0, XS_T3 = 1, XS_T4 = 2 };

template <int MODE, int TR = 8>
struct XG {
  static constexpr bool T = MODE != XS_S2;
  static constexpr int in_rows = T ? TR + 2 : 9;
  static constexpr int QPR = T ? 10 : 18;
  static constexpr int LCOLS = 4 * QPR;
  static constexpr int NPIX = in_rows * LCOLS, NPIXP = NPIX + 1;
  static constexpr int SLOTS = in_rows * QPR;
  static constexpr int NSLOT = T ? 16 : 12;
  static constexpr int NU = T ? 4 : 3;
  static constexpr int NPB = T ? TR / 2 : 2;
  static constexpr int EPI = T ? TR * 64 + 4 : 132;
};
constexpr int kEpiS2 = 132;

inline int slot_tap(int mode, int s) {
  if (mode == XS_S2) return s < 9 ? s : -1;
  const int ks = mode == XS_T4 ? 4 : 3;
  const int cls = s >> 2, a = (s >> 1) & 1, b = s & 1, pa = cls >> 1, pb = cls & 1;
  auto k = [&](int par, int opt) { return par ? (opt ? 0 : 2) : (opt ? (ks == 4 ? 3 : -1) : 1); };
  const int ky = k(pa, a), kx = k(pb, b);
  return (ky < 0 || kx < 0) ? -1 : ky * ks + kx;
}

struct SlotMap { int tap[16]; };

__global__ void __launch_bounds__(256)
weight_split6_g8_kernel(const float* __restrict__ w_t, u32x4* __restrict__ w6, int Cin, int ntaps, int wpad, int coutp, int nchunk,
                        int nslot, const SlotMap m) {
  const int n = nchunk * nslot * coutp;
  for (int i = blockIdx.x * blockDim.x + threadIdx.x; i < n; i += gridDim.x * blockDim.x) {
    const int co = i % coutp;
    const int r = i / coutp;
    const int slot = r % nslot, chunk = r / nslot;
    const int tap = m.tap[slot];
    float v[8];
#pragma unroll
    for (int e = 0; e < 8; ++e) {
      const int ci = chunk * 8 + e;
      v[e] = (tap >= 0 && ci < Cin && co < wpad) ? w_t[(static_cast<size_t>(ci) * ntaps + tap) * wpad + co] : 0.f;
    }
    unsigned part[3][4];
#pragma unroll
    for (int e = 0; e < 4; ++e) split6(v[2 * e], v[2 * e + 1], part[0][e], part[1][e], part[2][e]);
#pragma unroll
    for (int pt = 0; pt < 3; ++pt)
      w6[((static_cast<size_t>(chunk) * 3 + pt) * nslot + slot) * coutp + co] = u32x4{part[pt][0], part[pt][1], part[pt][2], part[pt][3]};
  }
}

template <int MODE, int CB, int TR = 8>
__global__ void __launch_bounds__(256, TR == 4 ? 3 : 2)
ig_conv_x6s_kernel(const float* __restrict__ x, const u32x4* __restrict__ w6, const float* __restrict__ scale,
                   const float* __restrict__ shift, float* __restrict__ y, const IG p) {
  extern __shared__ __attribute__((aligned(16))) u32x4 lds6[];
  using G = XG<MODE, TR>;
  constexpr bool T = G::T;
  static_assert(!T || CB == 1, "transposed forms: 16 output channels per workgroup (four classes of accumulators)");
  constexpr int LCOLS = G::LCOLS, NPIXP = G::NPIXP, NSLOT = G::NSLOT, NU = G::NU, NPB = G::NPB, SLOTS = G::SLOTS;
  constexpr int COB = CB * 16;
  constexpr int WV = 3 * NSLOT * COB, RWN = (WV + 255) / 256;
  constexpr int NCH = T ? 4 : 8;
  u32x4* in6 = lds6;
  u32x4* w6s = lds6 + 3 * NPIXP;

  const int wave = threadIdx.x >> 6, lane = threadIdx.x & 63;
  const int j = lane & 15, kq = lane >> 4;
  unsigned lin = blockIdx.x + gridDim.x * (blockIdx.y + gridDim.y * blockIdx.z);
  {
    const unsigned total = gridDim.x * gridDim.y * gridDim.z, per = total / 8;
    if (p.xcd && lin < per * 8) lin = (lin % 8) * per + lin / 8;
  }
  const int tile = lin % gridDim.x;
  const int od = (lin / gridDim.x) % gridDim.y;
  const int bz = lin / (gridDim.x * gridDim.y);
  const int cog = bz % p.co_groups, b = bz / p.co_groups;
  const int co0 = cog * COB;
  const int ty0 = (tile / p.tiles_x) * (T ? TR : 4), tx0 = (tile % p.tiles_x) * 32;
  const int row0 = T ? ty0 - 1 : 2 * ty0 - 1, col0 = T ? tx0 - 4 : 2 * tx0 - 4;
  const unsigned HW = static_cast<unsigned>(p.H) * p.W;
  const unsigned cstride_b = static_cast<unsigned>(p.in_cstride) * 4u;

  const int half = T ? static_cast<int>(threadIdx.x >> 7) : 0;
  const int sslot = T ? static_cast<int>(threadIdx.x & 127) : static_cast<int>(threadIdx.x);
  const bool stager = sslot < SLOTS;
  const int srow = sslot / G::QPR, squad = sslot - srow * G::QPR;
  unsigned goff = kOOB;
  {
    const int gy = row0 + srow, gx = col0 + 4 * squad;
    if (stager && gy >= 0 && gy < p.H && gx >= 0 && gx < p.W)
      goff = (static_cast<unsigned>(od) * HW + static_cast<unsigned>(gy) * p.W + gx) * 4u;
  }
  const int lpix = srow * LCOLS + 4 * squad;

  unsigned woff[RWN];
  int wl[RWN];
#pragma unroll
  for (int q = 0; q < RWN; ++q) {
    const int v = threadIdx.x + 256 * q;
    const int col = v % COB, r = v / COB;
    const bool ok = v < WV && co0 + col < p.coutp;
    woff[q] = ok ? static_cast<unsigned>(r * p.coutp + co0 + col) * 16u : kOOB;
    wl[q] = v < WV ? v : WV;
  }
  const __amdgpu_buffer_rsrc_t xr = ig_rsrc(x + static_cast<long long>(b) * p.in_bstride, p.in_bytes);
  const __amdgpu_buffer_rsrc_t wr = ig_rsrc(w6, p.w_bytes);
  const unsigned wchunk_b = static_cast<unsigned>(3 * NSLOT * p.coutp) * 16u;

  int boff[NPB], toff[NU];
#pragma unroll
  for (int pb = 0; pb < NPB; ++pb) {
    if (T) boff[pb] = ((TR == 8 ? wave * 2 + (pb >> 1) : wave) + 1) * LCOLS + 4 + (pb & 1) * 16 + j;
    else boff[pb] = (2 * wave) * LCOLS + 3 + 2 * (pb * 16 + j);
  }
#pragma unroll
  for (int u = 0; u < NU; ++u) {
    if (T) {
      const int pa = u >> 1, pbit = u & 1, a = kq >> 1, bq = kq & 1;
      const int dy = a ? (pa ? 1 : (MODE == XS_T4 ? -1 : 0)) : 0, dx = bq ? (pbit ? 1 : (MODE == XS_T4 ? -1 : 0)) : 0;
      toff[u] = dy * LCOLS + dx;
    } else {
      const int s = 4 * u + kq;
      toff[u] = s < 9 ? (s / 3) * LCOLS + (s % 3) : 0;
    }
  }
  const int aoff = kq * COB + j;

  v4f acc[T ? 4 : 1][CB][NPB];
#pragma unroll
  for (int c = 0; c < (T ? 4 : 1); ++c)
#pragma unroll
    for (int cb = 0; cb < CB; ++cb)
#pragma unroll
      for (int pb = 0; pb < NPB; ++pb) acc[c][cb][pb] = v4f{0.f, 0.f, 0.f, 0.f};
  float esc[CB][4], esh[CB][4];
#pragma unroll
  for (int cb = 0; cb < CB; ++cb)
// ... 36 lines not shown

  fetch(0);
  for (int c0 = 0; c0 < p.Cin; c0 += 8) {
    __syncthreads();
    commit();
    __syncthreads();
    if (c0 + 8 < p.Cin) fetch(c0 + 8);
    v4f part[CB][NPB];
    auto zero_part = [&]() {
#pragma unroll
      for (int cb = 0; cb < CB; ++cb)
#pragma unroll
        for (int pb = 0; pb < NPB; ++pb) part[cb][pb] = v4f{0.f, 0.f, 0.f, 0.f};
    };
    zero_part();
    bf16x8 a[2][3][CB], bv[2][3][NPB];
    auto load_frag = [&](int u, int buf) {
#pragma unroll
      for (int pt = 0; pt < 3; ++pt) {
#pragma unroll
        for (int cb = 0; cb < CB; ++cb) a[buf][pt][cb] = __builtin_bit_cast(bf16x8, w6s[(pt * NSLOT + 4 * u) * COB + aoff + cb * 16]);
#pragma unroll
        for (int pb = 0; pb < NPB; ++pb) bv[buf][pt][pb] = __builtin_bit_cast(bf16x8, in6[pt * NPIXP + boff[pb] + toff[u]]);
      }
    };
    load_frag(0, 0);
#pragma unroll
    for (int u = 0; u < NU; ++u) {
      if (u + 1 < NU) load_frag(u + 1, (u + 1) & 1);
      constexpr int PA[6] = {0, 2, 1, 0, 1, 0}, PB[6] = {2, 0, 1, 1, 0, 0};
#pragma unroll
      for (int t = 0; t < 6; ++t)
#pragma unroll
        for (int cb = 0; cb < CB; ++cb)
#pragma unroll
          for (int pb = 0; pb < NPB; ++pb)
            part[cb][pb] = __builtin_amdgcn_mfma_f32_16x16x32_bf16(a[u & 1][PA[t]][cb], bv[u & 1][PB[t]][pb], part[cb][pb], 0, 0, 0);
      if (T) {
#pragma unroll
        for (int cb = 0; cb < CB; ++cb)
#pragma unroll
          for (int pb = 0; pb < NPB; ++pb) acc[u][cb][pb] += part[cb][pb];
        zero_part();
      }
    }
    if (!T) {
#pragma unroll
      for (int cb = 0; cb < CB; ++cb)
#pragma unroll
        for (int pb = 0; pb < NPB; ++pb) acc[0][cb][pb] += part[cb][pb];
    }
  }

  const unsigned hw_o = static_cast<unsigned>(p.Ho) * p.Wo;
  const __amdgpu_buffer_rsrc_t yr = ig_rsrc(y + static_cast<long long>(b) * p.out_bstride, p.out_bytes);
  const unsigned ocs = static_cast<unsigned>(p.out_cstride) * 4u;
  const unsigned obase = static_cast<unsigned>(od) * hw_o;
  float* epi = reinterpret_cast<float*>(lds6);
  if constexpr (!T) {
    __syncthreads();
#pragma unroll
    for (int cb = 0; cb < CB; ++cb)
#pragma unroll
      for (int pb = 0; pb < NPB; ++pb)
#pragma unroll
        for (int r = 0; r < 4; ++r) {
          const int co = co0 + cb * 16 + kq * 4 + r;
          epi[(cb * 16 + kq * 4 + r) * kEpiS2 + wave * 32 + pb * 16 + j] =
              apply_act(acc[0][cb][pb][r] * esc[cb][r] + esh[cb][r], p.act, p.act_param, co);
        }
    __syncthreads();
#pragma unroll
    for (int it = 0; it < CB * 2; ++it) {
      const int idx = static_cast<int>(threadIdx.x) + 256 * it;
      const int col = idx >> 5, q = idx & 31;
      const int oy = ty0 + (q >> 3), ox = tx0 + (q & 7) * 4;
      const u32x4 val = *reinterpret_cast<const u32x4*>(epi + col * kEpiS2 + q * 4);
      const int co = co0 + col;
      const unsigned off = (oy < p.Ho && ox < p.Wo && co < p.Cout)
          ? (obase + static_cast<unsigned>(oy) * p.Wo + ox) * 4u + static_cast<unsigned>(co) * ocs : kOOB;
      __builtin_amdgcn_raw_buffer_store_b128(val, yr, off, 0, 0);
    }
  } else {
#pragma unroll
    for (int pa = 0; pa < 2; ++pa) {
      __syncthreads();
#pragma unroll
      for (int pbit = 0; pbit < 2; ++pbit)
#pragma unroll
        for (int pb = 0; pb < NPB; ++pb)
#pragma unroll
          for (int r = 0; r < 4; ++r) {
            const int co = co0 + kq * 4 + r;
            epi[(kq * 4 + r) * G::EPI + (TR == 8 ? wave * 2 + (pb >> 1) : wave) * 64 + 2 * ((pb & 1) * 16 + j) + pbit] =
                apply_act(acc[pa * 2 + pbit][0][pb][r] * esc[0][r] + esh[0][r], p.act, p.act_param, co);
          }
      __syncthreads();
#pragma unroll
      for (int it = 0; it < TR; ++it) {
        const int idx = static_cast<int>(threadIdx.x) + 256 * it;
        const int col = idx / (TR * 16), rem = idx % (TR * 16);
        const int row = rem >> 4, q = rem & 15;
        const int iy = ty0 + row, oy = 2 * iy + pa, ox = 2 * tx0 + 4 * q;
        const u32x4 val = *reinterpret_cast<const u32x4*>(epi + col * G::EPI + row * 64 + q * 4);
        const int co = co0 + col;
        const unsigned off = (iy < p.H && oy < p.Ho && ox < p.Wo && co < p.Cout)
            ? (obase + static_cast<unsigned>(oy) * p.Wo + ox) * 4u + static_cast<unsigned>(co) * ocs : kOOB;
        __builtin_amdgcn_raw_buffer_store_b128(val, yr, off, 0, 0);
      }
    }
  }
}

template <int MODE, int CB, int TR = 8>
int launch_x6s(const float* x, const void* w6, const float* scale, const float* shift, float* y, const IG& p, dim3 grid, hipStream_t st) {
  using G = XG<MODE, TR>;
  constexpr size_t main_b = (static_cast<size_t>(3) * G::NPIXP + 3 * G::NSLOT * CB * 16 + 1) * 16;
  constexpr size_t epi_b = G::T ? static_cast<size_t>(16) * G::EPI * 4 : static_cast<size_t>(CB) * 16 * kEpiS2 * 4;
  constexpr size_t lds = main_b > epi_b ? main_b : epi_b;
  static_assert(lds <= 64 * 1024, "ig_conv_x6s_kernel: LDS tile");
  hipLaunchKernelGGL((ig_conv_x6s_kernel<MODE, CB, TR>), grid, dim3(256), lds, st, x, static_cast<const u32x4*>(w6), scale, shift, y, p);
  return ts::launched("ig_conv_x6s_kernel");
}

inline int coutp6(int Cout) { return (Cout + 15) / 16 * 16; }
inline int mode_taps(int mode) { return mode == XS_T4 ? 16 : 9; }
inline int mode_slots(int mode) { return mode == XS_S2 ? 12 : 16; }
}

extern "C" int ts_conv3d_hw_x6s_supported(int Cin, int Cout, int H, int W, int mode) {
  if (mode < 0 || mode > 2 || Cin < 16 || Cout <= 0 || Cout > 512 || H <= 0 || W <= 0 || W % 4) return 0;
  if (mode == XS_S2) return (((W - 1) / 2 + 1) % 4) == 0;
  return 1;
}

extern "C" size_t ts_conv3d_hw_x6s_weight_bytes(int Cin, int Cout, int mode) {
  if (Cin <= 0 || Cout <= 0 || Cout > 512 || mode < 0 || mode > 2) return 0;
  return static_cast<size_t>((Cin + 7) / 8) * 3 * mode_slots(mode) * coutp6(Cout) * 16;
}

extern "C" int ts_conv3d_hw_x6s_weight_split(const float* w_t, void* w6, int Cin, int Cout, int w_pad, int mode, void* stream) {
  TS_REQUIRE(Cin > 0 && Cout > 0 && Cout <= 512 && w_pad >= Cout, TS_ERR_SHAPE, "conv3d_hw_x6s_weight_split: bad channel counts");
  TS_REQUIRE(mode >= 0 && mode <= 2, TS_ERR_SHAPE, "conv3d_hw_x6s_weight_split: unknown mode %d", mode);
  TS_REQUIRE_PTR(w_t); TS_REQUIRE_PTR(w6);
  const int nchunk = (Cin + 7) / 8, nslot = mode_slots(mode), cp = coutp6(Cout);
  SlotMap m;
  for (int s = 0; s < 16; ++s) m.tap[s] = s < nslot ? slot_tap(mode, s) : -1;
  const int n = nchunk * nslot * cp;
  hipLaunchKernelGGL(weight_split6_g8_kernel, dim3((n + 255) / 256), dim3(256), 0, ts::as_stream(stream), w_t,
                     static_cast<u32x4*>(w6), Cin, mode_taps(mode), w_pad, cp, nchunk, nslot, m);
  return ts::launched("weight_split6_g8_kernel");
}

extern "C" int ts_conv3d_hw_x6s_fwd(const float* x, const void* w6, const float* scale, const float* shift, float* y,
                                    int B, int Cin, int Cout, int D, int H, int W, int mode, int act, float act_param,
                                    long long in_bstride, long long in_cstride, long long out_bstride, long long out_cstride,
                                    void* stream) {
  TS_REQUIRE(B > 0 && Cin > 0 && Cout > 0 && D > 0 && H > 0 && W > 0, TS_ERR_SHAPE, "conv3d_hw_x6s: non-positive size");
  TS_REQUIRE(ts_conv3d_hw_x6s_supported(Cin, Cout, H, W, mode), TS_ERR_UNSUPPORTED,
             "conv3d_hw_x6s: needs Cin >= 16, Cout <= 512, W %% 4 == 0 and Wo %% 4 == 0 (Cin=%d Cout=%d W=%d mode=%d)", Cin, Cout, W, mode);
  TS_REQUIRE(act >= 0 && act <= 4, TS_ERR_SHAPE, "conv3d_hw_x6s: unknown activation");
  TS_REQUIRE(D <= 65535, TS_ERR_UNSUPPORTED, "conv3d_hw_x6s: grid too large");
  TS_REQUIRE_PTR(x); TS_REQUIRE_PTR(w6); TS_REQUIRE_PTR(y);
  IG p;
  p.Cin = Cin; p.Cout = Cout; p.coutp = coutp6(Cout); p.D = D; p.H = H; p.W = W; p.Do = D;
  if (mode == XS_S2) { p.Ho = (H - 1) / 2 + 1; p.Wo = (W - 1) / 2 + 1; }
  else { p.Ho = 2 * H; p.Wo = 2 * W; }
  p.stride = 2; p.dil = 1; p.pad = 1; p.k = mode == XS_T4 ? 4 : 3; p.transposed = mode != XS_S2;
  p.act = act; p.act_param = act_param;
  p.in_bstride = in_bstride; p.in_cstride = in_cstride; p.out_bstride = out_bstride; p.out_cstride = out_cstride;
  p.ksplit = 1; p.kspan = Cin; p.partial = nullptr; p.B = B; p.part_bytes = 0;
  p.addend = nullptr; p.add_bstride = p.add_cstride = p.add_dstride = 0;
  static const int xcd = ts::env_not_zero("TS_X6_XCD") ? 1 : 0;
  p.xcd = xcd;
  {
    const unsigned long long in_b = (static_cast<unsigned long long>(Cin - 1) * in_cstride + static_cast<unsigned long long>(D) * H * W) * 4ull;
    const unsigned long long out_b = (static_cast<unsigned long long>(Cout - 1) * out_cstride + static_cast<unsigned long long>(D) * p.Ho * p.Wo) * 4ull;
    const unsigned long long w_b = ts_conv3d_hw_x6s_weight_bytes(Cin, Cout, mode);
    TS_REQUIRE(in_b < 0x7fffffffull && out_b < 0x7fffffffull && w_b < 0x7fffffffull && in_cstride >= 0 && out_cstride >= 0,
               TS_ERR_UNSUPPORTED, "conv3d_hw_x6s: a batch element spans 2 GiB or more");
    p.in_bytes = static_cast<unsigned>(in_b); p.out_bytes = static_cast<unsigned>(out_b); p.w_bytes = static_cast<unsigned>(w_b);
  }
  hipStream_t st = ts::as_stream(stream);
  TS_REQUIRE(static_cast<long long>(B) * ((p.coutp + 15) / 16) <= 65535, TS_ERR_UNSUPPORTED, "conv3d_hw_x6s: batch x channel groups beyond the grid's z extent");
  if (mode == XS_S2) {
    p.tiles_x = (p.Wo + 31) / 32;
    const int tiles = ((p.Ho + 3) / 4) * p.tiles_x;
    const int cb = Cout > 16 ? 2 : 1;
    p.co_groups = (p.coutp / 16 + cb - 1) / cb;
    const dim3 grid(tiles, D, B * p.co_groups);
    return cb == 2 ? launch_x6s<XS_S2, 2>(x, w6, scale, shift, y, p, grid, st) : launch_x6s<XS_S2, 1>(x, w6, scale, shift, y, p, grid, st);
  }
  p.tiles_x = (W + 31) / 32;
  p.co_groups = p.coutp / 16;
  static const long long tr_env = ts::env_ll("TS_X6S_TR", 0);
  const long long wgs8 = static_cast<long long>((H + 7) / 8) * p.tiles_x * D * B * p.co_groups;
  const long long tr = tr_env ? tr_env : (wgs8 < 3 * ts::kNumCU / 2 ? 4 : 8);
  if (tr == 4) {
    const dim3 grid(((H + 3) / 4) * p.tiles_x, D, B * p.co_groups);
    return mode == XS_T4 ? launch_x6s<XS_T4, 1, 4>(x, w6, scale, shift, y, p, grid, st) : launch_x6s<XS_T3, 1, 4>(x, w6, scale, shift, y, p, grid, st);
  }
  const int tiles = ((H + 7) / 8) * p.tiles_x;
  const dim3 grid(tiles, D, B * p.co_groups);
  return mode == XS_T4 ? launch_x6s<XS_T4, 1>(x, w6, scale, shift, y, p, grid, st) : launch_x6s<XS_T3, 1>(x, w6, scale, shift, y, p, grid, st);
}
```

temporalstereo_amd/csrc/plan.hip:

```cpp
#include <cstdint>
#include <cstring>
#include <mutex>
#include <string>
#include <utility>
#include <vector>

#include "ts_common.hpp"

namespace {

constexpr int kMaxWords = 32;

template <class T>
T unpack(unsigned long long w) {
  static_assert(sizeof(T) <= sizeof(unsigned long long), "argument wider than a plan word");
  T v;
  std::memcpy(&v, &w, sizeof(T));
  return v;
}

template <class... A, size_t... I>
int call_with(int (*f)(A...), const unsigned long long* w, std::index_sequence<I...>) {
  return f(unpack<A>(w[I])...);
}
template <class... A>
int call_with(int (*f)(A...), const unsigned long long* w) {
  return call_with(f, w, std::index_sequence_for<A...>{});
}
template <class... A>
constexpr int arity(int (*)(A...)) { return static_cast<int>(sizeof...(A)); }

struct Entry {
  const char* name;
  int (*thunk)(const unsigned long long*);
  int nargs;
};

#define TS_PLAN_OP(fn) Entry{#fn, [](const unsigned long long* w) { return call_with(&fn, w); }, arity(&fn)}

const Entry kTable[] = {
    TS_PLAN_OP(ts_block_cost_int_fwd),      TS_PLAN_OP(ts_block_cost_sampled_fwd),
    TS_PLAN_OP(ts_block_cost_sampled_warped_fwd),
    TS_PLAN_OP(ts_block_cost_sampled_corr_fwd), TS_PLAN_OP(ts_conv3d_hw_warp_fwd),
    TS_PLAN_OP(ts_cat_fms_fwd),             TS_PLAN_OP(ts_dif_fms_fwd),             TS_PLAN_OP(ts_inverse_warp_3d_fwd),
    TS_PLAN_OP(ts_block_cost_int_bwd),      TS_PLAN_OP(ts_block_cost_sampled_bwd),
    TS_PLAN_OP(ts_topk_softargmax_fwd),     TS_PLAN_OP(ts_topk_softargmax_bwd),
    TS_PLAN_OP(ts_softargmin_fwd),          TS_PLAN_OP(ts_softargmin_bwd),
    TS_PLAN_OP(ts_argmax_select_fwd),       TS_PLAN_OP(ts_softsplat_sum_fwd),
    TS_PLAN_OP(ts_softsplat_sum_fwd_deterministic), TS_PLAN_OP(ts_softsplat_sum_bwd_input), TS_PLAN_OP(ts_softsplat_sum_bwd_flow),
    TS_PLAN_OP(ts_softsplat_softmax_fwd),   TS_PLAN_OP(ts_project_to_3d_fwd),
    TS_PLAN_OP(ts_conv3d_hw_fwd),           TS_PLAN_OP(ts_conv3d_d_fwd),
    TS_PLAN_OP(ts_conv3d_hw_bwd_data),      TS_PLAN_OP(ts_conv3d_hw_bwd_weight),
    TS_PLAN_OP(ts_conv3d_d_bwd_data),       TS_PLAN_OP(ts_conv3d_d_bwd_weight),
    TS_PLAN_OP(ts_resize3d_add_act_fwd),    TS_PLAN_OP(ts_pool3d5_avgmax_fwd),
    TS_PLAN_OP(ts_merge_candidates_fwd),    TS_PLAN_OP(ts_convex_upsample_fwd),
    TS_PLAN_OP(ts_convex_upsample_candidates_fwd),
    TS_PLAN_OP(ts_unet_upsample_fwd),       TS_PLAN_OP(ts_deconv2d_k4s2_fwd),
    TS_PLAN_OP(ts_resize_bilinear_fwd),     TS_PLAN_OP(ts_range_candidates_fwd),
    TS_PLAN_OP(ts_copy_rows_fwd),           TS_PLAN_OP(ts_stream_fork),
    TS_PLAN_OP(ts_event_record),            TS_PLAN_OP(ts_event_wait),
    TS_PLAN_OP(ts_resize3d_add_act_bwd),    TS_PLAN_OP(ts_pool3d5_avgmax_bwd),
    TS_PLAN_OP(ts_merge_candidates_bwd),
    TS_PLAN_OP(ts_reproject_memory_fwd),
    TS_PLAN_OP(ts_resize_bilinear_pair_fwd),
    TS_PLAN_OP(ts_calib_stream),             TS_PLAN_OP(ts_conv_set_chunk_cap),
    TS_PLAN_OP(ts_wasserstein_loss_fwd),     TS_PLAN_OP(ts_wasserstein_loss_bwd),
    TS_PLAN_OP(ts_disp_smooth_l1_fwd),       TS_PLAN_OP(ts_disp_smooth_l1_bwd),
    TS_PLAN_OP(ts_disp_metrics_fwd),         TS_PLAN_OP(ts_disp_render_fwd),
    TS_PLAN_OP(ts_correlation_fwd),          TS_PLAN_OP(ts_correlation_bwd),
    TS_PLAN_OP(ts_bn_stats_fwd),             TS_PLAN_OP(ts_bn_apply_act_fwd),
    TS_PLAN_OP(ts_bn_act_bwd_reduce),        TS_PLAN_OP(ts_bn_act_bwd_apply),
    TS_PLAN_OP(ts_convex_upsample_bwd),      TS_PLAN_OP(ts_unet_upsample_bwd),
    TS_PLAN_OP(ts_conv_weight_layout),      TS_PLAN_OP(ts_conv_weight_layout_many),
    TS_PLAN_OP(ts_conv3d_hw_x6_fwd),        TS_PLAN_OP(ts_conv3d_hw_x6_weight_split), TS_PLAN_OP(ts_conv3d_hw_x6_weight_split_from),
    TS_PLAN_OP(ts_conv3d_hw_x6s_fwd),       TS_PLAN_OP(ts_conv3d_hw_x6s_weight_split),
    TS_PLAN_OP(ts_peer_all_gather),         TS_PLAN_OP(ts_peer_all_reduce_sum),
    TS_PLAN_OP(ts_bn_train_fwd),            TS_PLAN_OP(ts_bn_train_bwd),
    TS_PLAN_OP(ts_channel_splice_fwd),
    TS_PLAN_OP(ts_candidates_in_range_fwd), TS_PLAN_OP(ts_candidates_in_range_bwd),
    TS_PLAN_OP(ts_offset_head_fwd),         TS_PLAN_OP(ts_offset_head_bwd),
    TS_PLAN_OP(ts_space_to_depth2_fwd),
    TS_PLAN_OP(ts_deconv2d_k4s2_weight_to_conv3), TS_PLAN_OP(ts_deconv2d_k4s2_wgrad_from_conv3),
    TS_PLAN_OP(ts_clip_rmsprop_step),       TS_PLAN_OP(ts_bn_sync_merge),
    TS_PLAN_OP(ts_bn_fold_many),
    TS_PLAN_OP(ts_conv_weight_layout_many2), TS_PLAN_OP(ts_conv_wgrad_finish_many), TS_PLAN_OP(ts_channel_sum_fwd),
    TS_PLAN_OP(ts_block_cost_sampled_warped_bwd),
    TS_PLAN_OP(ts_frames_prepare_fwd),      TS_PLAN_OP(ts_intrinsics_pyramid_fwd),  TS_PLAN_OP(ts_disp_u16_decode_fwd),
    TS_PLAN_OP(ts_frames_augment_fwd),      TS_PLAN_OP(ts_disp_u16_window_fwd),
    TS_PLAN_OP(ts_block_cost_sampled_corr_split_fwd), TS_PLAN_OP(ts_conv3d_hw_split_fwd),
    TS_PLAN_OP(ts_conv3d_d_split_fwd),      TS_PLAN_OP(ts_conv3d_hw_x6_split_fwd),
    TS_PLAN_OP(ts_inverse_warp_fwd),        TS_PLAN_OP(ts_inverse_warp_bwd),
    TS_PLAN_OP(ts_raft_corr_pyramid_fwd),   TS_PLAN_OP(ts_raft_corr_lookup_fwd),
    TS_PLAN_OP(ts_raft_corr_lookup_bwd),    TS_PLAN_OP(ts_raft_corr_pyramid_bwd),
    TS_PLAN_OP(ts_flow_corr_pyramid_fwd),   TS_PLAN_OP(ts_flow_corr_lookup_fwd),
    TS_PLAN_OP(ts_flow_corr_lookup_bwd),    TS_PLAN_OP(ts_flow_corr_pyramid_bwd),
    TS_PLAN_OP(ts_flow_metrics_fwd),        TS_PLAN_OP(ts_flow_render_fwd),         TS_PLAN_OP(ts_flow_u16_decode_fwd),
    TS_PLAN_OP(ts_spp3d_pool_fwd),          TS_PLAN_OP(ts_spp3d_pool_bwd),
    TS_PLAN_OP(ts_spp3d_expand_fwd),        TS_PLAN_OP(ts_spp3d_expand_bwd),        TS_PLAN_OP(ts_depth_sum3_fwd),
    TS_PLAN_OP(ts_bn_small_train_bwd),
};

struct Call {
  const Entry* op;
  unsigned long long w[kMaxWords];
};

__global__ void __launch_bounds__(256)
copy_rows_kernel(const float* __restrict__ src, float* __restrict__ dst, long long rows, long long row_elems,
                 long long src_pitch, long long dst_pitch) {
  const long long n = rows * row_elems;
  for (long long i = static_cast<long long>(blockIdx.x) * blockDim.x + threadIdx.x; i < n;
       i += static_cast<long long>(gridDim.x) * blockDim.x) {
    const long long r = i / row_elems, c = i - r * row_elems;
    dst[r * dst_pitch + c] = src[r * src_pitch + c];
  }
}

__global__ void __launch_bounds__(256)
copy_rows4_kernel(const float4* __restrict__ src, float4* __restrict__ dst, long long row_quads, long long src_pitch_q,
                  long long dst_pitch_q) {
  const float4* s = src + blockIdx.y * src_pitch_q;
  float4* d = dst + blockIdx.y * dst_pitch_q;
  for (long long i = static_cast<long long>(blockIdx.x) * blockDim.x + threadIdx.x; i < row_quads;
       i += static_cast<long long>(gridDim.x) * blockDim.x)
    d[i] = s[i];
}

}

struct ts_plan {
  std::vector<Call> calls;
};

extern "C" ts_plan* ts_plan_create(void) { return new (std::nothrow) ts_plan(); }

extern "C" void ts_plan_destroy(ts_plan* plan) { delete plan; }

extern "C" int ts_plan_length(const ts_plan* plan) { return plan ? static_cast<int>(plan->calls.size()) : -1; }

extern "C" int ts_plan_add_call(ts_plan* plan, const char* name, const unsigned long long* words, int n_words) {
  TS_REQUIRE_PTR(plan); TS_REQUIRE_PTR(name);
  TS_REQUIRE(n_words >= 0 && n_words <= kMaxWords, TS_ERR_SHAPE, "plan: %d argument words", n_words);
  TS_REQUIRE(n_words == 0 || words != nullptr, TS_ERR_NULL, "plan: words is NULL");
  for (const Entry& e : kTable) {
    if (std::strcmp(e.name, name) != 0) continue;
    TS_REQUIRE(e.nargs == n_words, TS_ERR_SHAPE, "plan: %s takes %d arguments, got %d", name, e.nargs, n_words);
    Call c;
    c.op = &e;
    std::memset(c.w, 0, sizeof(c.w));
    if (n_words) std::memcpy(c.w, words, sizeof(unsigned long long) * n_words);
    plan->calls.push_back(c);
    return TS_OK;
  }
  return ts::fail(TS_ERR_UNSUPPORTED, "plan: %s is not a launching entry point", name);
}

extern "C" int ts_plan_run(ts_plan* plan) {
  TS_REQUIRE_PTR(plan);
  for (const Call& c : plan->calls) {
    const int rc = c.op->thunk(c.w);
    if (rc != TS_OK) return rc;
  }
  return TS_OK;
}

extern "C" int ts_stream_fork(void* from_stream, void* to_stream) {
  constexpr int kRing = 64;
  constexpr int kMaxDev = 16;
  struct Ring { hipEvent_t ev[kRing]; int made = 0, next = 0; };
  static thread_local Ring rings[kMaxDev];
  int dev = 0;
  hipError_t e = hipGetDevice(&dev);
  if (e != hipSuccess) return ts::fail(static_cast<int>(e), "stream_fork: %s", hipGetErrorString(e));
  TS_REQUIRE(dev >= 0 && dev < kMaxDev, TS_ERR_UNSUPPORTED, "stream_fork: device %d", dev);
  Ring& r = rings[dev];
  if (r.made < kRing && r.next == r.made) {
    e = hipEventCreateWithFlags(&r.ev[r.made], hipEventDisableTiming);
    if (e != hipSuccess) return ts::fail(static_cast<int>(e), "stream_fork: %s", hipGetErrorString(e));
    ++r.made;
  }
  hipEvent_t ev = r.ev[r.next];
  r.next = (r.next + 1) % kRing;
// ... 81 lines not shown
```

temporalstereo_amd/csrc/pyramid_ops.hip:

```cpp
#include "ts_common.hpp"

namespace {

__device__ __forceinline__ float silu(float v) {
#ifdef TS_EXACT_SILU
  return v / (1.f + expf(-v));
#endif
  const float d = 1.f + __builtin_amdgcn_exp2f(v * -1.4426950408889634f);
  const float r = __builtin_amdgcn_rcpf(d);
  const float rn = fmaf(fmaf(-d, r, 1.f), r, r);
  return v * (d < 3.0e38f ? rn : r);
}

unsigned grid_for(long long n, int threads) {
  long long blocks = (n + threads - 1) / threads;
  const long long cap = static_cast<long long>(ts::kNumCU) * 16;
  if (blocks > cap) blocks = cap;
  if (blocks < 1) blocks = 1;
  return static_cast<unsigned>(blocks);
}

unsigned exact_grid(long long n) { return static_cast<unsigned>((n + 255) / 256); }

__device__ __forceinline__ void lin_src(float scale, int dst, int in_size, int& i0, int& i1, float& l1) {
  const float s = scale * static_cast<float>(dst);
  i0 = static_cast<int>(s);
  i1 = i0 + ((i0 < in_size - 1) ? 1 : 0);
  l1 = s - static_cast<float>(i0);
}

inline float ac_scale(int in_size, int out_size) {
  return out_size > 1 ? static_cast<float>(in_size - 1) / static_cast<float>(out_size - 1) : 0.f;
}

struct Resize3 {
  int C, Da, Ha, Wa, D, H, W;
  float sd, sh, sw;
  int act;
  long long a_bstride, a_cstride, b_bstride, b_cstride, o_bstride, o_cstride;
};

__global__ void __launch_bounds__(256)
resize_add_act_kernel(const float* __restrict__ a, const float* __restrict__ bsrc, float* __restrict__ out, const Resize3 p) {
  const int c = blockIdx.y, b = blockIdx.z;
  const int n = p.D * p.H * p.W;
  const float* ap = a + static_cast<size_t>(b) * p.a_bstride + static_cast<size_t>(c) * p.a_cstride;
  const float* bp = bsrc ? bsrc + static_cast<size_t>(b) * p.b_bstride + static_cast<size_t>(c) * p.b_cstride : nullptr;
  float* op = out + static_cast<size_t>(b) * p.o_bstride + static_cast<size_t>(c) * p.o_cstride;
  for (int i = blockIdx.x * blockDim.x + threadIdx.x; i < n; i += gridDim.x * blockDim.x) {
    const int x = i % p.W;
    const int t = i / p.W;
    const int y = t % p.H, d = t / p.H;
    int d0, d1, y0, y1, x0, x1;
    float ld, ly, lx;
    lin_src(p.sd, d, p.Da, d0, d1, ld);
    lin_src(p.sh, y, p.Ha, y0, y1, ly);
    lin_src(p.sw, x, p.Wa, x0, x1, lx);
    const size_t HWa = static_cast<size_t>(p.Ha) * p.Wa;
    const float* p0 = ap + d0 * HWa;
    const float* p1 = ap + d1 * HWa;
    const float v00 = (1.f - lx) * p0[y0 * p.Wa + x0] + lx * p0[y0 * p.Wa + x1];
    const float v01 = (1.f - lx) * p0[y1 * p.Wa + x0] + lx * p0[y1 * p.Wa + x1];
    const float v10 = (1.f - lx) * p1[y0 * p.Wa + x0] + lx * p1[y0 * p.Wa + x1];
    const float v11 = (1.f - lx) * p1[y1 * p.Wa + x0] + lx * p1[y1 * p.Wa + x1];
    float v = (1.f - ld) * ((1.f - ly) * v00 + ly * v01) + ld * ((1.f - ly) * v10 + ly * v11);
    if (bp) v += bp[i];
    op[i] = p.act == 1 ? silu(v) : v;
  }
}

constexpr int PT_Y = 8, PT_X = 32;
struct Pool5 {
  int C, D, H, W;
  long long x_bstride, x_cstride, avg_bstride, avg_cstride, max_bstride, max_cstride;
};

__global__ void __launch_bounds__(256)
pool5_avgmax_kernel(const float* __restrict__ x, float* __restrict__ oavg, float* __restrict__ omax, const Pool5 p) {
  __shared__ float tile_s[PT_Y + 4][PT_X + 4 + 1];
  __shared__ float tile_m[PT_Y + 4][PT_X + 4 + 1];
  const int tiles_x = (p.W + PT_X - 1) / PT_X;
  const int ty0 = (blockIdx.x / tiles_x) * PT_Y, tx0 = (blockIdx.x % tiles_x) * PT_X;
  const int c = blockIdx.y, b = blockIdx.z;
  const int tx = threadIdx.x & (PT_X - 1), ty = threadIdx.x / PT_X;
  const int y = ty0 + ty, xx = tx0 + tx;
  const size_t HW = static_cast<size_t>(p.H) * p.W;
  const float* xp = x + static_cast<size_t>(b) * p.x_bstride + static_cast<size_t>(c) * p.x_cstride;
  float* ap = oavg + static_cast<size_t>(b) * p.avg_bstride + static_cast<size_t>(c) * p.avg_cstride;
  float* mp = omax + static_cast<size_t>(b) * p.max_bstride + static_cast<size_t>(c) * p.max_cstride;
  constexpr int TW = PT_X + 4, TN = (PT_Y + 4) * TW;
  int soff[2], lidx[2];
  bool pad[2];
#pragma unroll
  for (int e = 0; e < 2; ++e) {
    const int i = min(static_cast<int>(threadIdx.x) + 256 * e, TN - 1);
    const int cx = i % TW, cy = i / TW;
    const int gy = ty0 + cy - 2, gx = tx0 + cx - 2;
    pad[e] = !(gy >= 0 && gy < p.H && gx >= 0 && gx < p.W);
    soff[e] = min(max(gy, 0), p.H - 1) * p.W + min(max(gx, 0), p.W - 1);
    lidx[e] = cy * (TW + 1) + cx;
  }
  float* tls = &tile_s[0][0];
  float* tlm = &tile_m[0][0];
  float nxt[2];
#pragma unroll
  for (int e = 0; e < 2; ++e) nxt[e] = xp[soff[e]];
  float rs[5], rm[5];
#pragma unroll
  for (int i = 0; i < 5; ++i) { rs[i] = 0.f; rm[i] = -INFINITY; }
  for (int d = 0; d < p.D + 2; ++d) {
    float s2 = 0.f, m2 = -INFINITY;
    if (d < p.D) {
// ... 28 lines not shown
    }
  }
}

constexpr int MERGE_DMAX = 20;
struct Merge {
  int B, C, D0, K, HW;
  int implicit_samples;
  long long vol_bstride, vol_cstride, out_bstride, out_cstride;
};

constexpr int MERGE_CPB = 2;

template <int DM>
__global__ void __launch_bounds__(256)
merge_candidates_kernel(const float* __restrict__ vol, const float* __restrict__ samp, const float* __restrict__ mem_samp,
                        const float* __restrict__ mem_cost, const float* __restrict__ pw, const float* __restrict__ pscale,
                        const float* __restrict__ pshift, float* __restrict__ out_samp, float* __restrict__ out_vol,
                        const Merge p) {
  const int DT = p.D0 + p.K;
  const int c0 = blockIdx.y * MERGE_CPB;
  const long long n = static_cast<long long>(p.B) * p.HW;
  const bool has_mem = mem_samp != nullptr && mem_cost != nullptr && p.K > 0;
  const float* ms = has_mem ? mem_samp : vol;
  const float* mc = has_mem ? mem_cost : vol;
  const int Kc = max(p.K, 1);
  float w_[MERGE_CPB], sc_[MERGE_CPB], sh_[MERGE_CPB];
#pragma unroll
  for (int cc = 0; cc < MERGE_CPB; ++cc) {
    const int c = min(c0 + cc, p.C - 1);
    w_[cc] = p.K > 0 ? pw[c] : 0.f; sc_[cc] = p.K > 0 ? pscale[c] : 0.f; sh_[cc] = p.K > 0 ? pshift[c] : 0.f;
  }
  for (long long i = static_cast<long long>(blockIdx.x) * blockDim.x + threadIdx.x; i < n;
       i += static_cast<long long>(gridDim.x) * blockDim.x) {
    const int b = static_cast<int>(i / p.HW);
    const int px = static_cast<int>(i - static_cast<long long>(b) * p.HW);
    float s[DM], m[DM], v[DM][MERGE_CPB];
    const float* vb = vol + static_cast<size_t>(b) * p.vol_bstride + px;
#pragma unroll
    for (int j = 0; j < DM; ++j) {
      const int jv = min(j, p.D0 - 1), jm = min(max(j - p.D0, 0), Kc - 1);
      const size_t mo = has_mem ? (static_cast<size_t>(b) * p.K + jm) * p.HW + px : 0;
      s[j] = p.implicit_samples ? static_cast<float>(j) : samp[(static_cast<size_t>(b) * p.D0 + jv) * p.HW + px];
      const float a = ms[mo];
      m[j] = mc[mo];
      if (j >= p.D0) s[j] = (j < DT) ? (has_mem ? a : 0.f) : INFINITY;
      if (!has_mem) m[j] = 0.f;
#pragma unroll
      for (int cc = 0; cc < MERGE_CPB; ++cc)
        v[j][cc] = vb[static_cast<size_t>(jv) * p.HW + static_cast<size_t>(min(c0 + cc, p.C - 1)) * p.vol_cstride];
    }
#pragma unroll
    for (int j = 0; j < DM; ++j) {
      int rank = 0;
#pragma unroll
      for (int q = 0; q < DM; ++q) rank += (s[q] < s[j]) || (s[q] == s[j] && q < j);
      if (j < DT) {
        if (c0 == 0) out_samp[(static_cast<size_t>(b) * DT + rank) * p.HW + px] = s[j];
        float* ov = out_vol + static_cast<size_t>(b) * p.out_bstride + static_cast<size_t>(rank) * p.HW + px;
#pragma unroll
        for (int cc = 0; cc < MERGE_CPB; ++cc) {
          const float val = (j < p.D0) ? v[j][cc] : silu(w_[cc] * m[j] * sc_[cc] + sh_[cc]);
          if (c0 + cc < p.C) ov[static_cast<size_t>(c0 + cc) * p.out_cstride] = val;
        }
      }
    }
  }
}

__global__ void __launch_bounds__(256)
convex_upsample_kernel(const float* __restrict__ mask, const float* __restrict__ disp, float* __restrict__ out,
                       int B, int H, int W, int r, float disp_scale,
                       float* __restrict__ low, float* __restrict__ high, float* __restrict__ cand, float range, int coff, int ctot) {
  const int HW = H * W, Ho = H * r, Wo = W * r;
  const long long n = static_cast<long long>(B) * Ho * Wo;
  for (long long i = static_cast<long long>(blockIdx.x) * blockDim.x + threadIdx.x; i < n;
       i += static_cast<long long>(gridDim.x) * blockDim.x) {
    const int ox = static_cast<int>(i % Wo);
    const long long t = i / Wo;
    const int oy = static_cast<int>(t % Ho), b = static_cast<int>(t / Ho);
    const int y = oy / r, ry = oy - y * r, x = ox / r, rx = ox - x * r;
    const float* mp = mask + (static_cast<size_t>(b) * 9 * r * r + ry * r + rx) * HW + static_cast<size_t>(y) * W + x;
    const float* dp = disp + static_cast<size_t>(b) * HW;
    float m[9], mx = -INFINITY;
#pragma unroll
    for (int k = 0; k < 9; ++k) { m[k] = mp[static_cast<size_t>(k) * r * r * HW]; mx = fmaxf(mx, m[k]); }
    float den = 0.f, acc = 0.f;
#pragma unroll
    for (int k = 0; k < 9; ++k) {
      const float e = expf(m[k] - mx);
      den += e;
      const int yy = y + k / 3 - 1, xx = x + k % 3 - 1;
      const float dv = dp[min(max(yy, 0), H - 1) * W + min(max(xx, 0), W - 1)];
      const float v = (yy >= 0 && yy < H && xx >= 0 && xx < W) ? dv * disp_scale : 0.f;
      acc += e * v;
    }
    const float dup = acc / den;
    out[i] = dup;
    if (low) {
      const float lo = dup - range, hi = dup + range;
      low[i] = lo; high[i] = hi;
      const float span = fabsf(hi - lo), base = fminf(lo, hi);
      const size_t HWo = static_cast<size_t>(Ho) * Wo;
      float* c = cand + (static_cast<size_t>(b) * ctot + coff) * HWo + static_cast<size_t>(oy) * Wo + ox;
      c[0] = span * 0.f + base;
      c[HWo] = span * 0.375f + base;
      c[2 * HWo] = span * 0.5f + base;
      c[3 * HWo] = span * 0.625f + base;
      c[4 * HWo] = span * 1.f + base;
    }
  }
}

template <int V>
__global__ void __launch_bounds__(256)
unet_upsample_kernel(const float* __restrict__ mask, const float* __restrict__ disp, float* __restrict__ out,
                     int B, int h, int w, int Ho, int Wo, float sh, float sw) {
  const int Wv = Wo / V;
  const long long n = static_cast<long long>(B) * Ho * Wv;
  const size_t HWo = static_cast<size_t>(Ho) * Wo;
  for (long long i = static_cast<long long>(blockIdx.x) * blockDim.x + threadIdx.x; i < n;
       i += static_cast<long long>(gridDim.x) * blockDim.x) {
    const int oxv = static_cast<int>(i % Wv) * V;
    const long long t = i / Wv;
    const int oy = static_cast<int>(t % Ho), b = static_cast<int>(t / Ho);
    const float* mp = mask + static_cast<size_t>(b) * 9 * HWo + static_cast<size_t>(oy) * Wo + oxv;
    const float* dp = disp + static_cast<size_t>(b) * h * w;
    float m[9][V];
#pragma unroll
    for (int k = 0; k < 9; ++k) {
      if constexpr (V == 4) {
        const float4 q = *reinterpret_cast<const float4*>(mp + k * HWo);
        m[k][0] = q.x; m[k][1] = q.y; m[k][2] = q.z; m[k][3] = q.w;
      } else {
        m[k][0] = mp[k * HWo];
      }
    }
    int y0, y1;
    float ly;
    lin_src(sh, oy, h, y0, y1, ly);
    const bool iy = y1 > y0;
    constexpr int XS = (V == 4) ? 1 : 0;
    int xb, xb1;
    float lxb;
    lin_src(sw, oxv, w, xb, xb1, lxb);
    int xe = xb, xe1;
    float lxe;
    if (V > 1) lin_src(sw, oxv + V - 1, w, xe, xe1, lxe);
    const bool shared = (xe - xb) <= XS;
    float P[4][4 + XS];
#pragma unroll
    for (int r = 0; r < 4; ++r)
#pragma unroll
      for (int c = 0; c < 4 + XS; ++c) {
        const int yy = y0 - 1 + r, xx = xb - 1 + c;
        const float dv = dp[min(max(yy, 0), h - 1) * w + min(max(xx, 0), w - 1)];
        P[r][c] = (yy >= 0 && yy < h && xx >= 0 && xx < w) ? dv * static_cast<float>(Wo) / static_cast<float>(w) : 0.f;
      }
    float res[V];
#pragma unroll
    for (int v = 0; v < V; ++v) {
      const int ox = oxv + v;
      int x0, x1;
      float lx;
      lin_src(sw, ox, w, x0, x1, lx);
      float pd[4][4];
      if (shared) {
        const bool sh = XS && (x0 != xb);
#pragma unroll
        for (int r = 0; r < 4; ++r)
#pragma unroll
          for (int c = 0; c < 4; ++c) pd[r][c] = sh ? P[r][c + XS] : P[r][c];
      } else {
#pragma unroll
        for (int r = 0; r < 4; ++r)
#pragma unroll
          for (int c = 0; c < 4; ++c) {
            const int yy = y0 - 1 + r, xx = x0 - 1 + c;
            const float dv = dp[min(max(yy, 0), h - 1) * w + min(max(xx, 0), w - 1)];
            pd[r][c] = (yy >= 0 && yy < h && xx >= 0 && xx < w) ? dv * static_cast<float>(Wo) / static_cast<float>(w) : 0.f;
          }
      }
      float mx = -INFINITY;
#pragma unroll
      for (int k = 0; k < 9; ++k) mx = fmaxf(mx, m[k][v]);
      const bool ix = x1 > x0;
      float den = 0.f, acc = 0.f;
#pragma unroll
      for (int k = 0; k < 9; ++k) {
        const float e = expf(m[k][v] - mx);
        den += e;
        const int ry = k / 3, rx = k % 3;
        const float a00 = pd[ry][rx];
        const float a01 = ix ? pd[ry][rx + 1] : a00;
        const float a10 = iy ? pd[ry + 1][rx] : a00;
        const float a11 = iy ? (ix ? pd[ry + 1][rx + 1] : pd[ry + 1][rx]) : a01;
        const float top = (1.f - lx) * a00 + lx * a01;
        const float bot = (1.f - lx) * a10 + lx * a11;
        acc += e * ((1.f - ly) * top + ly * bot);
      }
      res[v] = acc / den;
    }
    float* op = out + static_cast<size_t>(b) * HWo + static_cast<size_t>(oy) * Wo + oxv;
    if constexpr (V == 4) *reinterpret_cast<float4*>(op) = make_float4(res[0], res[1], res[2], res[3]);
    else op[0] = res[0];
  }
}

__global__ void __launch_bounds__(256)
resize_bilinear_kernel(const float* __restrict__ x, float* __restrict__ out, int BC, int C, int h, int w, int Ho, int Wo,
                       float sh, float sw, float vscale, long long out_bstride) {
  const long long n = static_cast<long long>(BC) * Ho * Wo;
  for (long long i = static_cast<long long>(blockIdx.x) * blockDim.x + threadIdx.x; i < n;
       i += static_cast<long long>(gridDim.x) * blockDim.x) {
    const int ox = static_cast<int>(i % Wo);
    const long long t = i / Wo;
    const int oy = static_cast<int>(t % Ho), bc = static_cast<int>(t / Ho);
    int y0, y1, x0, x1;
    float ly, lx;
    lin_src(sh, oy, h, y0, y1, ly);
    lin_src(sw, ox, w, x0, x1, lx);
    const float* p = x + static_cast<size_t>(bc) * h * w;
    const float top = (1.f - lx) * p[y0 * w + x0] + lx * p[y0 * w + x1];
    const float bot = (1.f - lx) * p[y1 * w + x0] + lx * p[y1 * w + x1];
    const int b = bc / C, c = bc - b * C;
    out[static_cast<size_t>(b) * out_bstride + (static_cast<size_t>(c) * Ho + oy) * Wo + ox] = ((1.f - ly) * top + ly * bot) * vscale;
  }
}

__global__ void __launch_bounds__(256)
resize_bilinear_pair_kernel(const float* __restrict__ x0, const float* __restrict__ x1, float* __restrict__ out0,
                            float* __restrict__ out1, int BC, int h, int w, int Ho, int Wo, float sh, float sw, float vs0,
                            float vs1) {
  const float* x = blockIdx.y ? x1 : x0;
  float* out = blockIdx.y ? out1 : out0;
  const float vscale = blockIdx.y ? vs1 : vs0;
  const long long n = static_cast<long long>(BC) * Ho * Wo;
  for (long long i = static_cast<long long>(blockIdx.x) * blockDim.x + threadIdx.x; i < n;
       i += static_cast<long long>(gridDim.x) * blockDim.x) {
    const int ox = static_cast<int>(i % Wo);
    const long long t = i / Wo;
    const int oy = static_cast<int>(t % Ho), bc = static_cast<int>(t / Ho);
    int y0, y1, xa, xb;
    float ly, lx;
    lin_src(sh, oy, h, y0, y1, ly);
    lin_src(sw, ox, w, xa, xb, lx);
    const float* p = x + static_cast<size_t>(bc) * h * w;
    const float top = (1.f - lx) * p[y0 * w + xa] + lx * p[y0 * w + xb];
    const float bot = (1.f - lx) * p[y1 * w + xa] + lx * p[y1 * w + xb];
    out[i] = ((1.f - ly) * top + ly * bot) * vscale;
  }
}

__global__ void __launch_bounds__(256)
range_candidates_kernel(const float* __restrict__ disp, float* __restrict__ low, float* __restrict__ high,
                        float* __restrict__ cand, int B, int HW, float range, int coff, int ctot) {
  const long long n = static_cast<long long>(B) * HW;
  for (long long i = static_cast<long long>(blockIdx.x) * blockDim.x + threadIdx.x; i < n;
       i += static_cast<long long>(gridDim.x) * blockDim.x) {
    const int b = static_cast<int>(i / HW);
    const int px = static_cast<int>(i - static_cast<long long>(b) * HW);
    const float d = disp[i];
    const float lo = d - range, hi = d + range;
    low[i] = lo; high[i] = hi;
    const float span = fabsf(hi - lo), base = fminf(lo, hi);
    float* c = cand + (static_cast<size_t>(b) * ctot + coff) * HW + px;
    c[0] = span * 0.f + base;
    c[static_cast<size_t>(1) * HW] = span * 0.375f + base;
    c[static_cast<size_t>(2) * HW] = span * 0.5f + base;
    c[static_cast<size_t>(3) * HW] = span * 0.625f + base;
    c[static_cast<size_t>(4) * HW] = span * 1.f + base;
  }
}

struct Resize3B {
  Resize3 f;
  long long g_bstride, g_cstride, ga_bstride, ga_cstride, gb_bstride, gb_cstride;
};

__global__ void __launch_bounds__(256)
resize_add_act_bwd_kernel(const float* __restrict__ a, const float* __restrict__ bsrc, const float* __restrict__ gout,
                          float* __restrict__ ga, float* __restrict__ gadd, const Resize3B q) {
  const Resize3& p = q.f;
  const int c = blockIdx.y, b = blockIdx.z;
  const int n = p.D * p.H * p.W;
  const float* ap = a + static_cast<size_t>(b) * p.a_bstride + static_cast<size_t>(c) * p.a_cstride;
  const float* bp = bsrc ? bsrc + static_cast<size_t>(b) * p.b_bstride + static_cast<size_t>(c) * p.b_cstride : nullptr;
  const float* gp = gout + static_cast<size_t>(b) * q.g_bstride + static_cast<size_t>(c) * q.g_cstride;
  float* gap = ga + static_cast<size_t>(b) * q.ga_bstride + static_cast<size_t>(c) * q.ga_cstride;
  float* gbp = gadd ? gadd + static_cast<size_t>(b) * q.gb_bstride + static_cast<size_t>(c) * q.gb_cstride : nullptr;
  const size_t HWa = static_cast<size_t>(p.Ha) * p.Wa;
  for (int i = blockIdx.x * blockDim.x + threadIdx.x; i < n; i += gridDim.x * blockDim.x) {
    const int x = i % p.W;
    const int t = i / p.W;
    const int y = t % p.H, d = t / p.H;
    int d0, d1, y0, y1, x0, x1;
    float ld, ly, lx;
    lin_src(p.sd, d, p.Da, d0, d1, ld);
    lin_src(p.sh, y, p.Ha, y0, y1, ly);
    lin_src(p.sw, x, p.Wa, x0, x1, lx);
    float g = gp[i];
    if (p.act == 1) {
      const float* p0 = ap + d0 * HWa;
      const float* p1 = ap + d1 * HWa;
      const float v00 = (1.f - lx) * p0[y0 * p.Wa + x0] + lx * p0[y0 * p.Wa + x1];
      const float v01 = (1.f - lx) * p0[y1 * p.Wa + x0] + lx * p0[y1 * p.Wa + x1];
      const float v10 = (1.f - lx) * p1[y0 * p.Wa + x0] + lx * p1[y0 * p.Wa + x1];
      const float v11 = (1.f - lx) * p1[y1 * p.Wa + x0] + lx * p1[y1 * p.Wa + x1];
      float v = (1.f - ld) * ((1.f - ly) * v00 + ly * v01) + ld * ((1.f - ly) * v10 + ly * v11);
      if (bp) v += bp[i];
      const float sg = 1.f / (1.f + expf(-v));
      g *= sg * (1.f + v * (1.f - sg));
    }
    if (gbp) gbp[i] = g;
    const float wd[2] = {1.f - ld, ld}, wy[2] = {1.f - ly, ly}, wx[2] = {1.f - lx, lx};
    const int dd[2] = {d0, d1}, yy[2] = {y0, y1}, xx[2] = {x0, x1};
#pragma unroll
    for (int k = 0; k < 8; ++k) {
      const int kd = k >> 2, ky = (k >> 1) & 1, kx = k & 1;
      const float w = wd[kd] * wy[ky] * wx[kx];
      if (w != 0.f) atomicAdd(gap + dd[kd] * HWa + static_cast<size_t>(yy[ky]) * p.Wa + xx[kx], g * w);
    }
  }
}

__global__ void __launch_bounds__(256)
pool5_max_bwd_kernel(const float* __restrict__ x, const float* __restrict__ gmax, float* __restrict__ gx, const Pool5 p) {
  __shared__ float tile[PT_Y + 4][PT_X + 4 + 1];
  const int tiles_x = (p.W + PT_X - 1) / PT_X;
  const int ty0 = (blockIdx.x / tiles_x) * PT_Y, tx0 = (blockIdx.x % tiles_x) * PT_X;
  const int c = blockIdx.y, b = blockIdx.z;
  const int tx = threadIdx.x & (PT_X - 1), ty = threadIdx.x / PT_X;
  const int y = ty0 + ty, xx = tx0 + tx;
// ... 480 lines not shown
```

temporalstereo_amd/csrc/regress.hip:

```cpp
#include "ts_common.hpp"

namespace {

constexpr int KMAX = 8;

template <int K>
__global__ void __launch_bounds__(256)
topk_softargmax_fwd(const float* __restrict__ cost, const float* __restrict__ samp, const float* __restrict__ off,
                    float* __restrict__ disp, float* __restrict__ tdisp, float* __restrict__ tcost,
                    int* __restrict__ tidx, int B, int D, int HW) {
  const long long n = static_cast<long long>(B) * HW;
  for (long long i = static_cast<long long>(blockIdx.x) * blockDim.x + threadIdx.x; i < n;
       i += static_cast<long long>(gridDim.x) * blockDim.x) {
    const int b = static_cast<int>(i / HW);
    const int p = static_cast<int>(i - static_cast<long long>(b) * HW);
    const size_t base = static_cast<size_t>(b) * D * HW + p;
    float bc[K];
    int bi[K];
#pragma unroll
    for (int j = 0; j < K; ++j) { bc[j] = -INFINITY; bi[j] = -1; }
    for (int d0 = 0; d0 < D; d0 += 8) {
      float cc[8];
#pragma unroll
      for (int u = 0; u < 8; ++u) cc[u] = cost[base + static_cast<size_t>(min(d0 + u, D - 1)) * HW];
#pragma unroll
      for (int u = 0; u < 8; ++u) {
        float c = cc[u];
        int ci = d0 + u;
        const bool real = ci < D;
#pragma unroll
        for (int j = 0; j < K; ++j) {
          const bool take = real && ((c > bc[j]) || (bi[j] < 0));
          const float tc = bc[j];
          const int ti = bi[j];
          if (take) { bc[j] = c; bi[j] = ci; c = tc; ci = ti; }
        }
      }
    }
    float w[K], den = 0.f;
#pragma unroll
    for (int j = 0; j < K; ++j) { w[j] = expf(bc[j] - bc[0]); den += w[j]; }
    float acc = 0.f;
#pragma unroll
    for (int j = 0; j < K; ++j) {
      const size_t o = base + static_cast<size_t>(bi[j]) * HW;
      const float td = samp[o] + off[o];
      acc += (w[j] / den) * td;
      const size_t ko = (static_cast<size_t>(b) * K + j) * HW + p;
      tdisp[ko] = td;
      tcost[ko] = bc[j];
      if (tidx) tidx[ko] = bi[j];
    }
    disp[i] = acc;
  }
}

template <int K>
__global__ void __launch_bounds__(256)
topk_softargmax_bwd(const float* __restrict__ tdisp, const float* __restrict__ tcost, const int* __restrict__ tidx,
                    const float* __restrict__ disp, const float* __restrict__ gdisp, const float* __restrict__ gtd,
                    const float* __restrict__ gtc, float* __restrict__ gcost, float* __restrict__ gsamp,
                    int B, int D, int HW) {
  const long long n = static_cast<long long>(B) * HW;
  for (long long i = static_cast<long long>(blockIdx.x) * blockDim.x + threadIdx.x; i < n;
       i += static_cast<long long>(gridDim.x) * blockDim.x) {
    const int b = static_cast<int>(i / HW);
    const int p = static_cast<int>(i - static_cast<long long>(b) * HW);
    const size_t base = static_cast<size_t>(b) * D * HW + p;
    for (int d = 0; d < D; ++d) {
      if (gcost) gcost[base + static_cast<size_t>(d) * HW] = 0.f;
      if (gsamp) gsamp[base + static_cast<size_t>(d) * HW] = 0.f;
    }
    float c[K], td[K], w[K], den = 0.f;
    int idx[K];
#pragma unroll
    for (int j = 0; j < K; ++j) {
      const size_t ko = (static_cast<size_t>(b) * K + j) * HW + p;
      c[j] = tcost[ko]; td[j] = tdisp[ko]; idx[j] = tidx[ko];
    }
#pragma unroll
    for (int j = 0; j < K; ++j) { w[j] = expf(c[j] - c[0]); den += w[j]; }
    const float g = gdisp ? gdisp[i] : 0.f;
    const float dv = disp[i];
#pragma unroll
    for (int j = 0; j < K; ++j) {
      const size_t ko = (static_cast<size_t>(b) * K + j) * HW + p;
      const float pj = w[j] / den;
      const size_t o = base + static_cast<size_t>(idx[j]) * HW;
      if (gcost) gcost[o] = g * pj * (td[j] - dv) + (gtc ? gtc[ko] : 0.f);
      if (gsamp) gsamp[o] = g * pj + (gtd ? gtd[ko] : 0.f);
    }
  }
}

struct Partial { float m, s, ws; };

__device__ __forceinline__ Partial merge(Partial a, Partial b) {
  const float m = fmaxf(a.m, b.m);
  const float ea = (a.m == -INFINITY) ? 0.f : expf(a.m - m);
  const float eb = (b.m == -INFINITY) ? 0.f : expf(b.m - m);
  return Partial{m, a.s * ea + b.s * eb, a.ws * ea + b.ws * eb};
}

template <bool NORMALIZE>
__global__ void __launch_bounds__(256)
soft_argmin_fwd(const float* __restrict__ cost, const float* __restrict__ samp, float* __restrict__ disp,
                float temperature, int B, int D, int HW) {
  const int lane = threadIdx.x & 63;
  const int slice = lane >> 4;
  const long long wave = (static_cast<long long>(blockIdx.x) * blockDim.x + threadIdx.x) >> 6;
  const long long nwave = (static_cast<long long>(gridDim.x) * blockDim.x) >> 6;
  const long long npix = static_cast<long long>(B) * HW;
  for (long long p0 = wave * 16; p0 < npix; p0 += nwave * 16) {
    const long long i = p0 + (lane & 15);
    const bool ok = i < npix;
    const int b = ok ? static_cast<int>(i / HW) : 0;
    const int p = ok ? static_cast<int>(i - static_cast<long long>(b) * HW) : 0;
    const size_t base = static_cast<size_t>(b) * D * HW + p;
    Partial a{-INFINITY, 0.f, 0.f};
    float lin = 0.f;
    if (ok) {
      for (int d = slice; d < D; d += 4) {
        const float c = cost[base + static_cast<size_t>(d) * HW] * temperature;
        const float sv = samp[base + static_cast<size_t>(d) * HW];
        if constexpr (NORMALIZE) {
          a = merge(a, Partial{c, 1.f, sv});
        } else {
          lin += c * sv;
        }
      }
    }
    if constexpr (NORMALIZE) {
#pragma unroll
      for (int s = 16; s <= 32; s <<= 1) {
        Partial o{__shfl_xor(a.m, s), __shfl_xor(a.s, s), __shfl_xor(a.ws, s)};
        a = merge(a, o);
      }
      if (ok && slice == 0) disp[i] = a.ws / a.s;
    } else {
      lin += __shfl_xor(lin, 16);
      lin += __shfl_xor(lin, 32);
      if (ok && slice == 0) disp[i] = lin;
    }
  }
}

template <bool NORMALIZE>
__global__ void __launch_bounds__(256)
soft_argmin_bwd(const float* __restrict__ cost, const float* __restrict__ samp, const float* __restrict__ disp,
                const float* __restrict__ gdisp, float* __restrict__ gcost, float* __restrict__ gsamp,
                float temperature, int B, int D, int HW) {
  const long long n = static_cast<long long>(B) * HW;
  for (long long i = static_cast<long long>(blockIdx.x) * blockDim.x + threadIdx.x; i < n;
       i += static_cast<long long>(gridDim.x) * blockDim.x) {
    const int b = static_cast<int>(i / HW);
    const int p = static_cast<int>(i - static_cast<long long>(b) * HW);
    const size_t base = static_cast<size_t>(b) * D * HW + p;
    const float g = gdisp[i];
    if constexpr (NORMALIZE) {
      float m = -INFINITY, s = 0.f;
      for (int d = 0; d < D; ++d) {
        const float c = cost[base + static_cast<size_t>(d) * HW] * temperature;
        const float mn = fmaxf(m, c);
        s = s * expf(m - mn) + expf(c - mn);
        m = mn;
      }
      const float dv = disp[i];
      for (int d = 0; d < D; ++d) {
        const size_t o = base + static_cast<size_t>(d) * HW;
        const float pd = expf(cost[o] * temperature - m) / s;
        if (gcost) gcost[o] = g * temperature * pd * (samp[o] - dv);
        if (gsamp) gsamp[o] = g * pd;
      }
    } else {
      for (int d = 0; d < D; ++d) {
        const size_t o = base + static_cast<size_t>(d) * HW;
        if (gcost) gcost[o] = g * temperature * samp[o];
        if (gsamp) gsamp[o] = g * temperature * cost[o];
      }
    }
  }
}

__global__ void __launch_bounds__(256)
argmax_select_fwd(const float* __restrict__ cost, const float* __restrict__ samp, float* __restrict__ disp,
                  int* __restrict__ idx, int B, int D, int HW) {
  const long long n = static_cast<long long>(B) * HW;
  for (long long i = static_cast<long long>(blockIdx.x) * blockDim.x + threadIdx.x; i < n;
       i += static_cast<long long>(gridDim.x) * blockDim.x) {
    const int b = static_cast<int>(i / HW);
    const int p = static_cast<int>(i - static_cast<long long>(b) * HW);
    const size_t base = static_cast<size_t>(b) * D * HW + p;
    float best = -INFINITY;
    int bi = 0;
    for (int d = 0; d < D; ++d) {
      const float c = cost[base + static_cast<size_t>(d) * HW];
      if (c > best) { best = c; bi = d; }
    }
    disp[i] = samp[base + static_cast<size_t>(bi) * HW];
    if (idx) idx[i] = bi;
  }
}

int check_bdhw(int B, int D, int H, int W, const char* who) {
  TS_REQUIRE(B > 0 && D > 0 && H > 0 && W > 0, TS_ERR_SHAPE, "%s: non-positive size", who);
  TS_REQUIRE(static_cast<long long>(H) * W < (1ll << 31), TS_ERR_UNSUPPORTED, "%s: plane too large", who);
  return TS_OK;
}

unsigned grid_for(long long n, int threads) {
  long long blocks = (n + threads - 1) / threads;
  const long long cap = static_cast<long long>(ts::kNumCU) * 8;
  if (blocks > cap) blocks = cap;
  if (blocks < 1) blocks = 1;
  return static_cast<unsigned>(blocks);
}

}

extern "C" int ts_topk_softargmax_fwd(const float* cost, const float* sample, const float* offset, float* disp,
                                      float* topk_disp, float* topk_cost, int* topk_index,
                                      int B, int D, int H, int W, int k, void* stream) {
  if (int rc = check_bdhw(B, D, H, W, "topk_softargmax")) return rc;
  TS_REQUIRE(k >= 1 && k <= KMAX && k <= D, TS_ERR_UNSUPPORTED, "topk_softargmax: k=%d outside 1..min(%d, D)", k, KMAX);
  TS_REQUIRE_PTR(cost); TS_REQUIRE_PTR(sample); TS_REQUIRE_PTR(offset);
  TS_REQUIRE_PTR(disp); TS_REQUIRE_PTR(topk_disp); TS_REQUIRE_PTR(topk_cost);
  const int HW = H * W;
  const dim3 grid(grid_for(static_cast<long long>(B) * HW, 256));
  hipStream_t st = ts::as_stream(stream);
#define TS_CASE(KK)                                                                                     \
  case KK:                                                                                              \
    hipLaunchKernelGGL(topk_softargmax_fwd<KK>, grid, dim3(256), 0, st, cost, sample, offset, disp,      \
                       topk_disp, topk_cost, topk_index, B, D, HW);                                     \
    break;
  switch (k) { TS_CASE(1) TS_CASE(2) TS_CASE(3) TS_CASE(4) TS_CASE(5) TS_CASE(6) TS_CASE(7) TS_CASE(8) }
#undef TS_CASE
  return ts::launched("topk_softargmax_fwd");
}

extern "C" int ts_topk_softargmax_bwd(const float* topk_disp, const float* topk_cost, const int* topk_index,
                                      const float* disp, const float* grad_disp, const float* grad_topk_disp,
                                      const float* grad_topk_cost, float* grad_cost, float* grad_sample,
                                      int B, int D, int H, int W, int k, void* stream) {
  if (int rc = check_bdhw(B, D, H, W, "topk_softargmax_bwd")) return rc;
  TS_REQUIRE(k >= 1 && k <= KMAX && k <= D, TS_ERR_UNSUPPORTED, "topk_softargmax_bwd: k=%d outside 1..min(%d, D)", k, KMAX);
  TS_REQUIRE_PTR(topk_disp); TS_REQUIRE_PTR(topk_cost); TS_REQUIRE_PTR(topk_index); TS_REQUIRE_PTR(disp);
  const int HW = H * W;
  const dim3 grid(grid_for(static_cast<long long>(B) * HW, 256));
  hipStream_t st = ts::as_stream(stream);
#define TS_CASE(KK)                                                                                      \
  case KK:                                                                                               \
    hipLaunchKernelGGL(topk_softargmax_bwd<KK>, grid, dim3(256), 0, st, topk_disp, topk_cost, topk_index, \
                       disp, grad_disp, grad_topk_disp, grad_topk_cost, grad_cost, grad_sample, B, D, HW); \
    break;
  switch (k) { TS_CASE(1) TS_CASE(2) TS_CASE(3) TS_CASE(4) TS_CASE(5) TS_CASE(6) TS_CASE(7) TS_CASE(8) }
#undef TS_CASE
  return ts::launched("topk_softargmax_bwd");
}

extern "C" int ts_softargmin_fwd(const float* cost, const float* sample, float* disp, float temperature,
                                 int normalize, int B, int D, int H, int W, void* stream) {
  if (int rc = check_bdhw(B, D, H, W, "softargmin")) return rc;
  TS_REQUIRE_PTR(cost); TS_REQUIRE_PTR(sample); TS_REQUIRE_PTR(disp);
  const int HW = H * W;
  const long long nthreads = (static_cast<long long>(B) * HW + 15) / 16 * 64;
  const dim3 grid(grid_for(nthreads, 256));
  hipStream_t st = ts::as_stream(stream);
  if (normalize) hipLaunchKernelGGL(soft_argmin_fwd<true>, grid, dim3(256), 0, st, cost, sample, disp, temperature, B, D, HW);
  else hipLaunchKernelGGL(soft_argmin_fwd<false>, grid, dim3(256), 0, st, cost, sample, disp, temperature, B, D, HW);
  return ts::launched("softargmin_fwd");
}

extern "C" int ts_softargmin_bwd(const float* cost, const float* sample, const float* disp, const float* grad_disp,
                                 float* grad_cost, float* grad_sample, float temperature, int normalize,
                                 int B, int D, int H, int W, void* stream) {
  if (int rc = check_bdhw(B, D, H, W, "softargmin_bwd")) return rc;
  TS_REQUIRE_PTR(cost); TS_REQUIRE_PTR(sample); TS_REQUIRE_PTR(disp); TS_REQUIRE_PTR(grad_disp);
  const int HW = H * W;
  const dim3 grid(grid_for(static_cast<long long>(B) * HW, 256));
  hipStream_t st = ts::as_stream(stream);
  if (normalize) hipLaunchKernelGGL(soft_argmin_bwd<true>, grid, dim3(256), 0, st, cost, sample, disp, grad_disp, grad_cost, grad_sample, temperature, B, D, HW);
  else hipLaunchKernelGGL(soft_argmin_bwd<false>, grid, dim3(256), 0, st, cost, sample, disp, grad_disp, grad_cost, grad_sample, temperature, B, D, HW);
  return ts::launched("softargmin_bwd");
}

extern "C" int ts_argmax_select_fwd(const float* cost, const float* sample, float* disp, int* index,
                                    int B, int D, int H, int W, void* stream) {
  if (int rc = check_bdhw(B, D, H, W, "argmax_select")) return rc;
  TS_REQUIRE_PTR(cost); TS_REQUIRE_PTR(sample); TS_REQUIRE_PTR(disp);
  const int HW = H * W;
  hipLaunchKernelGGL(argmax_select_fwd, dim3(grid_for(static_cast<long long>(B) * HW, 256)), dim3(256), 0,
                     ts::as_stream(stream), cost, sample, disp, index, B, D, HW);
  return ts::launched("argmax_select_fwd");
}
```

temporalstereo_amd/csrc/ts_common.hpp:

```cpp
#pragma once
#include <hip/hip_runtime.h>

#include <cstdarg>
#include <cstdint>
#include <cstdio>
#include <cstdlib>
#include <type_traits>

#include "../../include/ts_hip.h"

#define TS_ABI_VERSION 18

namespace ts {

char* err_buf();
int fail(int code, const char* fmt, ...);

inline hipStream_t as_stream(void* s) { return reinterpret_cast<hipStream_t>(s); }

inline bool aligned16(const void* p) { return (reinterpret_cast<uintptr_t>(p) & 15u) == 0; }

inline size_t round_up(size_t v, size_t a) { return (v + a - 1) / a * a; }

inline int launched(const char* what) {
  hipError_t e = hipGetLastError();
  if (e != hipSuccess) return fail(static_cast<int>(e), "%s: %s", what, hipGetErrorString(e));
  return TS_OK;
}

template <class F>
inline void dispatch_bool(bool b, F&& f) {
  if (b) f(std::true_type{});
  else f(std::false_type{});
}

inline long long env_ll(const char* name, long long dflt) { const char* e = getenv(name); return e ? atoll(e) : dflt; }
inline bool env_not_zero(const char* name) { const char* e = getenv(name); return !(e && e[0] == '0'); }

constexpr int kWave = 64;
constexpr int kNumCU = 256;
constexpr int kNumXCD = 8;

}

#define TS_REQUIRE_PTR(p)                                                     \
  do {                                                                        \
    if ((p) == nullptr) return ts::fail(TS_ERR_NULL, "%s is NULL", #p);       \
  } while (0)
#define TS_REQUIRE_ALIGNED(p)                                                          \
  do {                                                                                 \
    if (!ts::aligned16(p)) return ts::fail(TS_ERR_ALIGN, "%s not 16-byte aligned", #p); \
  } while (0)
#define TS_REQUIRE(cond, code, ...)                       \
  do {                                                    \
    if (!(cond)) return ts::fail((code), __VA_ARGS__);    \
  } while (0)
```

Baseline: 1562.

## Fuse regression tails: topk softargmax with convex upsample, deconv with unet upsample

Adds a kernel that runs top-k soft-argmax regression and convex upsampling with range candidates in one pass. It also adds an epilogue variant of the x6s transposed-conv kernel that applies the unet disparity upsample directly, so the 9-channel mask is never written to global memory. A half-resolution top-k kernel is added as well. The goal is fewer launches and less intermediate memory traffic, at the cost of extra LDS and register pressure in the conv epilogue and more kernel variants to maintain.

Measured after the change: 1631, median of 6. 4.4% higher.

```diff
diff --git a/include/ts_hip.h b/include/ts_hip.h
--- a/include/ts_hip.h
+++ b/include/ts_hip.h
@@ -198,6 +198,14 @@
 int ts_topk_softargmax_fwd(const float* cost, const float* sample, const float* offset, float* disp,
                            float* topk_disp, float* topk_cost, int* topk_index,
                            int B, int D, int H, int W, int k, void* stream);
+
+int ts_regress_convex_upsample_fwd(const float* cost, const float* sample, const float* offset, const float* mask,
+                                   float* out, float* low, float* high, float* candidates, int B, int D, int H, int W,
+                                   int k, int factor, float disp_scale, float range, int channel_offset,
+                                   int channels_total, void* stream);
+
+int ts_topk_softargmax_half_fwd(const float* cost, const float* sample, const float* offset, float* disp,
+                                float* mem_sample, float* mem_cost, int B, int D, int H, int W, int k, void* stream);
 
 int ts_topk_softargmax_bwd(const float* topk_disp, const float* topk_cost, const int* topk_index,
                            const float* disp, const float* grad_disp, const float* grad_topk_disp,
@@ -364,6 +372,9 @@
 int ts_conv3d_hw_x6s_fwd(const float* x, const void* w6, const float* scale, const float* shift, float* y,
                          int B, int Cin, int Cout, int D, int H, int W, int mode, int act, float act_param,
                          long long in_bstride, long long in_cstride, long long out_bstride, long long out_cstride, void* stream);
+int ts_deconv2d_k4s2_unet_upsample_fwd(const float* x, const void* w6, const float* scale, const float* shift,
+                                       const float* disp, float* out, int B, int Cin, int Cout, int H, int W,
+                                       long long in_bstride, long long in_cstride, void* stream);
 int ts_conv3d_d_fwd(const float* x, const float* w_t, const float* scale, const float* shift, float* y,
                     int B, int Cin, int Cout, int Din, int H, int W, int k, int stride, int dilation,
                     int padding, int transposed, int act, float act_param,
diff --git a/temporalstereo_amd/_lib.py b/temporalstereo_amd/_lib.py
--- a/temporalstereo_amd/_lib.py
+++ b/temporalstereo_amd/_lib.py
@@ -56,6 +56,8 @@
     "ts_clip_rmsprop_workspace_bytes": (c_size, [c_int]),
     "ts_clip_rmsprop_step": (c_int, [c_ptr, c_int] + [c_float] * 4 + [c_ptr, c_size, c_ptr]),
     "ts_topk_softargmax_fwd": (c_int, [c_f32p] * 7 + [c_int] * 5 + [c_ptr]),
+    "ts_regress_convex_upsample_fwd": (c_int, [c_f32p] * 8 + [c_int] * 6 + [c_float, c_float, c_int, c_int, c_ptr]),
+    "ts_topk_softargmax_half_fwd": (c_int, [c_f32p] * 6 + [c_int] * 5 + [c_ptr]),
     "ts_topk_softargmax_bwd": (c_int, [c_f32p] * 9 + [c_int] * 5 + [c_ptr]),
     "ts_softargmin_fwd": (c_int, [c_f32p] * 3 + [c_float, c_int] + [c_int] * 4 + [c_ptr]),
     "ts_softargmin_bwd": (c_int, [c_f32p] * 6 + [c_float, c_int] + [c_int] * 4 + [c_ptr]),
@@ -132,6 +134,7 @@
     "ts_conv3d_hw_x6s_weight_bytes": (c_size, [c_int] * 3),
     "ts_conv3d_hw_x6s_weight_split": (c_int, [c_f32p, c_ptr, c_int, c_int, c_int, c_int, c_ptr]),
     "ts_conv3d_hw_x6s_fwd": (c_int, [c_f32p, c_ptr, c_f32p, c_f32p, c_f32p] + [c_int] * 8 + [c_float] + [ctypes.c_longlong] * 4 + [c_ptr]),
+    "ts_deconv2d_k4s2_unet_upsample_fwd": (c_int, [c_f32p, c_ptr, c_f32p, c_f32p, c_f32p, c_f32p] + [c_int] * 5 + [ctypes.c_longlong] * 2 + [c_ptr]),
     "ts_conv3d_hw_x6_fwd": (c_int, [c_f32p, c_ptr, c_f32p, c_f32p, c_f32p] + [c_int] * 8 + [c_float] + [ctypes.c_longlong] * 4 +
                             [c_f32p, ctypes.c_longlong, c_ptr, c_size, c_ptr]),
     "ts_conv3d_hw_fwd": (c_int, [c_f32p] * 5 + [c_int] * 10 + [c_float] + [ctypes.c_longlong] * 4 +
diff --git a/temporalstereo_amd/aggregation/native.py b/temporalstereo_amd/aggregation/native.py
--- a/temporalstereo_amd/aggregation/native.py
+++ b/temporalstereo_amd/aggregation/native.py
@@ -460,6 +460,13 @@
 
 FUSED_K1 = os.environ.get("TS_FUSED_K1", "1") != "0"
 SPLIT_INPUT = os.environ.get("TS_SPLIT_INPUT", "1") != "0"
+def _fused_tails(value):
+    if value == "0":
+        return frozenset()
+    return frozenset(("convex", "deconv")) if value in ("", "1") else frozenset(value.split(","))
+
+
+FUSED_TAILS = _fused_tails(os.environ.get("TS_FUSED_TAILS", "1"))
 
 
 def block_cost_corr(left, right, disp, scales):
@@ -665,6 +672,21 @@
         _lib.check(rc, "ts_convex_upsample_candidates_fwd")
         return out, low, high, cand
 
+    def regress_with_candidates(self, feat, cost, samp, off, k, m, rng, extra_front=0):
+        B, _, H, W = cost.shape
+        if m is None:
+            m = self.mask(feat)
+        Ho, Wo = H * self.r, W * self.r
+        out = torch.empty((B, 1, Ho, Wo), device=cost.device, dtype=torch.float32)
+        low, high = torch.empty_like(out), torch.empty_like(out)
+        cand = torch.empty((B, extra_front + 5, Ho, Wo), device=cost.device, dtype=torch.float32)
+        cost, samp, off = _lib.contiguous(cost), _lib.contiguous(samp), _lib.contiguous(off)
+        rc = _lib.lib().ts_regress_convex_upsample_fwd(_lib.ptr(cost), _lib.ptr(samp), _lib.ptr(off), _lib.ptr(m), _lib.ptr(out),
+                                                       _lib.ptr(low), _lib.ptr(high), _lib.ptr(cand), B, cost.shape[1], H, W, int(k),
+                                                       self.r, float(self.r), float(rng), extra_front, extra_front + 5, _stream())
+        _lib.check(rc, "ts_regress_convex_upsample_fwd")
+        return out, low, high, cand
+
     def __call__(self, feat, disp, m=None):
         B, _, H, W = disp.shape
         if m is None:
@@ -761,6 +783,10 @@
     def merge_fuse_predict(self, vol, samples, prev_info, feat, resize_memory, mask=None, next_range=None):
         cat4, samp = self.merge(vol, samples, prev_info, resize_memory)
         cost, off = self.heads(self.fuse(cat4))
+        if "convex" in FUSED_TAILS and next_range is not None and self.up.r <= 8:
+            if callable(mask):
+                mask = mask()
+            return self.up.regress_with_candidates(feat, cost, samp, off, self.topk, mask, *next_range), cost, off, samp
         disp, _, _ = TF.topk_softargmax(cost, samp, off, k=self.topk)
         if callable(mask):
             mask = mask()
@@ -810,6 +836,12 @@
 
     def __getitem__(self, idx):
         return torch.cat([s.cat() for s in self.pair()], 0)[idx]
+
+
+class DecoderHead:
+
+    def __init__(self, g):
+        self.g = g
 
 
 class NativePrecise(_LevelBase):
@@ -892,13 +924,26 @@
         return both, lterm, (lcat, cat2, B, H, W)
 
     def unet_decode(self, st):
+        return self.unet_logits(self.unet_decode_head(st))
+
+    def unet_decode_head(self, st):
         lcat, cat2, B, H, W = st
         f = self._c2d(self._c2d(lcat.unsqueeze(2), self.fuse[0], 1), self.fuse[1], 1).squeeze(2)
         self._deconv(_lib.contiguous(f), self.deconv4, cat2, cat2.stride(0))
-        g = _lib.contiguous(self._c2d(cat2.unsqueeze(2), self.concat, 1).squeeze(2))
-        mask = torch.empty((B, 9, 4 * H, 4 * W), device=lcat.device, dtype=torch.float32)
+        return _lib.contiguous(self._c2d(cat2.unsqueeze(2), self.concat, 1).squeeze(2))
+
+    def unet_logits(self, g):
+        B, _, H2, W2 = g.shape
+        mask = torch.empty((B, 9, 2 * H2, 2 * W2), device=g.device, dtype=torch.float32)
         self._deconv(g, self.deconv2, mask, mask.stride(0))
         return mask
+
+    def fused_upsample_ok(self, g):
+        B, Cin, H2, W2 = g.shape
+        f = self.deconv2
+        return bool("deconv" in FUSED_TAILS and X6 and X6S and f.act == ACT_NONE and 9 <= f.cout <= 16 and H2 % 2 == 0 and W2 % 2 == 0 and
+                    _lib.lib().ts_conv3d_hw_x6s_supported(Cin, f.cout, H2, W2, X6S_T4) and
+                    x6s_grid(B, f.cout, 1, H2, W2, X6S_T4) >= _X6S_MIN_GRID)
 
     def early(self, both, lterm, ds):
         B = both.shape[0] // 2
@@ -918,8 +963,16 @@
         cost, off = self.heads(vol)
         disp, mem_s, mem_c = TF.topk_softargmax(cost, ds, off, k=self.topk)
         full = torch.empty((B, 1, 4 * H, 4 * W), device=both.device, dtype=torch.float32)
-        rc = _lib.lib().ts_unet_upsample_fwd(_lib.ptr(mask), _lib.ptr(disp), _lib.ptr(full), B, H, W, 4 * H, 4 * W, _stream())
-        _lib.check(rc, "ts_unet_upsample_fwd")
+        if isinstance(mask, DecoderHead):
+            g, f = mask.g, self.deconv2
+            Cin = g.shape[1]
+            rc = _lib.lib().ts_deconv2d_k4s2_unet_upsample_fwd(_lib.ptr(g), _lib.ptr(x6s_weights(f, X6S_T4)), _lib.ptr(f.scale),
+                                                               _lib.ptr(f.shift), _lib.ptr(disp), _lib.ptr(full), B, Cin, f.cout,
+                                                               2 * H, 2 * W, Cin * 4 * H * W, 4 * H * W, _stream())
+            _lib.check(rc, "ts_deconv2d_k4s2_unet_upsample_fwd")
+        else:
+            rc = _lib.lib().ts_unet_upsample_fwd(_lib.ptr(mask), _lib.ptr(disp), _lib.ptr(full), B, H, W, 4 * H, 4 * W, _stream())
+            _lib.check(rc, "ts_unet_upsample_fwd")
         prev_info['prev_disp'] = full
         mem_s, mem_c = resize_bilinear_pair(mem_s, mem_c, (H // 2, W // 2), 0.5, 1.0)
         prev_info['cost_memory'] = {'disp_sample': mem_s, 'cost_volume': mem_c}
@@ -1025,7 +1078,8 @@
                 both, lterm, ust = self.precise.unet_encode(l4, r4, left_image, right_image)
             edge(S["unet"], S["unet2"])
             with on(S["unet2"]):
-                mask = self.precise.unet_decode(ust)
+                mask = self.precise.unet_decode_head(ust)
+                mask = DecoderHead(mask) if self.precise.fused_upsample_ok(mask) else self.precise.unet_logits(mask)
             edge(S["coarse"], S["coarse2"])
             with on(S["coarse2"]):
                 ds = self._coarse_level(l16, r16, prev_info, out, lambda: mc, vol=cvol)
diff --git a/temporalstereo_amd/csrc/conv_x6s.hip b/temporalstereo_amd/csrc/conv_x6s.hip
--- a/temporalstereo_amd/csrc/conv_x6s.hip
+++ b/temporalstereo_amd/csrc/conv_x6s.hip
@@ -1,4 +1,5 @@
 #include "conv_common.hpp"
+#include "regress_tails.hpp"
 
 namespace {
 
@@ -54,10 +55,18 @@
   }
 }
 
-template <int MODE, int CB, int TR = 8>
+struct StoreRows {};
+struct UnetUp {
+  const float* disp;
+  float* out;
+  int h, w;
+  float sh, sw;
+};
+
+template <int MODE, int CB, int TR = 8, class EP = StoreRows>
 __global__ void __launch_bounds__(256, TR == 4 ? 3 : 2)
 ig_conv_x6s_kernel(const float* __restrict__ x, const u32x4* __restrict__ w6, const float* __restrict__ scale,
-                   const float* __restrict__ shift, float* __restrict__ y, const IG p) {
+                   const float* __restrict__ shift, float* __restrict__ y, const IG p, const EP ep) {
   extern __shared__ __attribute__((aligned(16))) u32x4 lds6[];
   using G = XG<MODE, TR>;
   constexpr bool T = G::T;
@@ -260,9 +269,25 @@
       __builtin_amdgcn_raw_buffer_store_b128(val, yr, off, 0, 0);
     }
   } else {
+    constexpr int PR = TR / 2 + 5, PC = 21;
+    float* patch = epi + 16 * G::EPI;
+    int pyb = 0, pxb = 0;
+    if constexpr (std::is_same_v<EP, UnetUp>) {
+      int i1;
+      float l1;
+      ts_tail::lin_src(ep.sh, 2 * ty0, ep.h, pyb, i1, l1);
+      ts_tail::lin_src(ep.sw, 2 * tx0, ep.w, pxb, i1, l1);
+    }
 #pragma unroll
     for (int pa = 0; pa < 2; ++pa) {
       __syncthreads();
+      if constexpr (std::is_same_v<EP, UnetUp>) {
+        if (pa == 0) {
+          const float* dp = ep.disp + static_cast<size_t>(b) * ep.h * ep.w;
+          for (int i = threadIdx.x; i < PR * PC; i += 256)
+            patch[i] = ts_tail::unet_patch_value(dp, pyb - 1 + i / PC, pxb - 1 + i % PC, ep.h, ep.w, p.Wo);
+        }
+      }
 #pragma unroll
       for (int pbit = 0; pbit < 2; ++pbit)
 #pragma unroll
@@ -274,17 +299,41 @@
                 apply_act(acc[pa * 2 + pbit][0][pb][r] * esc[0][r] + esh[0][r], p.act, p.act_param, co);
           }
       __syncthreads();
-#pragma unroll
-      for (int it = 0; it < TR; ++it) {
-        const int idx = static_cast<int>(threadIdx.x) + 256 * it;
-        const int col = idx / (TR * 16), rem = idx % (TR * 16);
-        const int row = rem >> 4, q = rem & 15;
-        const int iy = ty0 + row, oy = 2 * iy + pa, ox = 2 * tx0 + 4 * q;
-        const u32x4 val = *reinterpret_cast<const u32x4*>(epi + col * G::EPI + row * 64 + q * 4);
-        const int co = co0 + col;
-        const unsigned off = (iy < p.H && oy < p.Ho && ox < p.Wo && co < p.Cout)
-            ? (obase + static_cast<unsigned>(oy) * p.Wo + ox) * 4u + static_cast<unsigned>(co) * ocs : kOOB;
-        __builtin_amdgcn_raw_buffer_store_b128(val, yr, off, 0, 0);
+      if constexpr (std::is_same_v<EP, UnetUp>) {
+#pragma unroll
+        for (int it = 0; it < TR / 4; ++it) {
+          const int idx = static_cast<int>(threadIdx.x) + 256 * it;
+          const int row = idx >> 6, c = idx & 63;
+          const int iy = ty0 + row, oy = 2 * iy + pa, ox = 2 * tx0 + c;
+          if (iy >= p.H || ox >= p.Wo) continue;
+          float m[9];
+#pragma unroll
+          for (int k = 0; k < 9; ++k) m[k] = epi[k * G::EPI + row * 64 + c];
+          int y0, y1, x0, x1;
+          float ly, lx;
+          ts_tail::lin_src(ep.sh, oy, ep.h, y0, y1, ly);
+          ts_tail::lin_src(ep.sw, ox, ep.w, x0, x1, lx);
+          const float* pp = patch + min(y0 - pyb, PR - 4) * PC + min(x0 - pxb, PC - 4);
+          float pd[4][4];
+#pragma unroll
+          for (int r = 0; r < 4; ++r)
+#pragma unroll
+            for (int cc = 0; cc < 4; ++cc) pd[r][cc] = pp[r * PC + cc];
+          ep.out[static_cast<size_t>(b) * hw_o + static_cast<size_t>(oy) * p.Wo + ox] = ts_tail::unet_combine(m, pd, lx, ly, x1 > x0, y1 > y0);
+        }
+      } else {
+#pragma unroll
+        for (int it = 0; it < TR; ++it) {
+          const int idx = static_cast<int>(threadIdx.x) + 256 * it;
+          const int col = idx / (TR * 16), rem = idx % (TR * 16);
+          const int row = rem >> 4, q = rem & 15;
+          const int iy = ty0 + row, oy = 2 * iy + pa, ox = 2 * tx0 + 4 * q;
+          const u32x4 val = *reinterpret_cast<const u32x4*>(epi + col * G::EPI + row * 64 + q * 4);
+          const int co = co0 + col;
+          const unsigned off = (iy < p.H && oy < p.Ho && ox < p.Wo && co < p.Cout)
+              ? (obase + static_cast<unsigned>(oy) * p.Wo + ox) * 4u + static_cast<unsigned>(co) * ocs : kOOB;
+          __builtin_amdgcn_raw_buffer_store_b128(val, yr, off, 0, 0);
+        }
       }
     }
   }
@@ -297,7 +346,7 @@
   constexpr size_t epi_b = G::T ? static_cast<size_t>(16) * G::EPI * 4 : static_cast<size_t>(CB) * 16 * kEpiS2 * 4;
   constexpr size_t lds = main_b > epi_b ? main_b : epi_b;
   static_assert(lds <= 64 * 1024, "ig_conv_x6s_kernel: LDS tile");
-  hipLaunchKernelGGL((ig_conv_x6s_kernel<MODE, CB, TR>), grid, dim3(256), lds, st, x, static_cast<const u32x4*>(w6), scale, shift, y, p);
+  hipLaunchKernelGGL((ig_conv_x6s_kernel<MODE, CB, TR>), grid, dim3(256), lds, st, x, static_cast<const u32x4*>(w6), scale, shift, y, p, StoreRows{});
   return ts::launched("ig_conv_x6s_kernel");
 }
 
@@ -330,17 +379,14 @@
   return ts::launched("weight_split6_g8_kernel");
 }
 
-extern "C" int ts_conv3d_hw_x6s_fwd(const float* x, const void* w6, const float* scale, const float* shift, float* y,
-                                    int B, int Cin, int Cout, int D, int H, int W, int mode, int act, float act_param,
-                                    long long in_bstride, long long in_cstride, long long out_bstride, long long out_cstride,
-                                    void* stream) {
-  TS_REQUIRE(B > 0 && Cin > 0 && Cout > 0 && D > 0 && H > 0 && W > 0, TS_ERR_SHAPE, "conv3d_hw_x6s: non-positive size");
+namespace {
+int x6s_params(IG& p, const char* who, int B, int Cin, int Cout, int D, int H, int W, int mode, int act, float act_param,
+               long long in_bstride, long long in_cstride, long long out_bstride, long long out_cstride) {
+  TS_REQUIRE(B > 0 && Cin > 0 && Cout > 0 && D > 0 && H > 0 && W > 0, TS_ERR_SHAPE, "%s: non-positive size", who);
   TS_REQUIRE(ts_conv3d_hw_x6s_supported(Cin, Cout, H, W, mode), TS_ERR_UNSUPPORTED,
-             "conv3d_hw_x6s: needs Cin >= 16, Cout <= 512, W %% 4 == 0 and Wo %% 4 == 0 (Cin=%d Cout=%d W=%d mode=%d)", Cin, Cout, W, mode);
-  TS_REQUIRE(act >= 0 && act <= 4, TS_ERR_SHAPE, "conv3d_hw_x6s: unknown activation");
-  TS_REQUIRE(D <= 65535, TS_ERR_UNSUPPORTED, "conv3d_hw_x6s: grid too large");
-  TS_REQUIRE_PTR(x); TS_REQUIRE_PTR(w6); TS_REQUIRE_PTR(y);
-  IG p;
+             "%s: needs Cin >= 16, Cout <= 512, W %% 4 == 0 and Wo %% 4 == 0 (Cin=%d Cout=%d W=%d mode=%d)", who, Cin, Cout, W, mode);
+  TS_REQUIRE(act >= 0 && act <= 4, TS_ERR_SHAPE, "%s: unknown activation", who);
+  TS_REQUIRE(D <= 65535, TS_ERR_UNSUPPORTED, "%s: grid too large", who);
   p.Cin = Cin; p.Cout = Cout; p.coutp = coutp6(Cout); p.D = D; p.H = H; p.W = W; p.Do = D;
   if (mode == XS_S2) { p.Ho = (H - 1) / 2 + 1; p.Wo = (W - 1) / 2 + 1; }
   else { p.Ho = 2 * H; p.Wo = 2 * W; }
@@ -356,11 +402,22 @@
     const unsigned long long out_b = (static_cast<unsigned long long>(Cout - 1) * out_cstride + static_cast<unsigned long long>(D) * p.Ho * p.Wo) * 4ull;
     const unsigned long long w_b = ts_conv3d_hw_x6s_weight_bytes(Cin, Cout, mode);
     TS_REQUIRE(in_b < 0x7fffffffull && out_b < 0x7fffffffull && w_b < 0x7fffffffull && in_cstride >= 0 && out_cstride >= 0,
-               TS_ERR_UNSUPPORTED, "conv3d_hw_x6s: a batch element spans 2 GiB or more");
+               TS_ERR_UNSUPPORTED, "%s: a batch element spans 2 GiB or more", who);
     p.in_bytes = static_cast<unsigned>(in_b); p.out_bytes = static_cast<unsigned>(out_b); p.w_bytes = static_cast<unsigned>(w_b);
   }
+  TS_REQUIRE(static_cast<long long>(B) * ((p.coutp + 15) / 16) <= 65535, TS_ERR_UNSUPPORTED, "%s: batch x channel groups beyond the grid's z extent", who);
+  return TS_OK;
+}
+}
+
+extern "C" int ts_conv3d_hw_x6s_fwd(const float* x, const void* w6, const float* scale, const float* shift, float* y,
+                                    int B, int Cin, int Cout, int D, int H, int W, int mode, int act, float act_param,
+                                    long long in_bstride, long long in_cstride, long long out_bstride, long long out_cstride,
+                                    void* stream) {
+  IG p;
+  if (int rc = x6s_params(p, "conv3d_hw_x6s", B, Cin, Cout, D, H, W, mode, act, act_param, in_bstride, in_cstride, out_bstride, out_cstride)) return rc;
+  TS_REQUIRE_PTR(x); TS_REQUIRE_PTR(w6); TS_REQUIRE_PTR(y);
   hipStream_t st = ts::as_stream(stream);
-  TS_REQUIRE(static_cast<long long>(B) * ((p.coutp + 15) / 16) <= 65535, TS_ERR_UNSUPPORTED, "conv3d_hw_x6s: batch x channel groups beyond the grid's z extent");
   if (mode == XS_S2) {
     p.tiles_x = (p.Wo + 31) / 32;
     const int tiles = ((p.Ho + 3) / 4) * p.tiles_x;
@@ -382,3 +439,27 @@
   const dim3 grid(tiles, D, B * p.co_groups);
   return mode == XS_T4 ? launch_x6s<XS_T4, 1>(x, w6, scale, shift, y, p, grid, st) : launch_x6s<XS_T3, 1>(x, w6, scale, shift, y, p, grid, st);
 }
+
+extern "C" int ts_deconv2d_k4s2_unet_upsample_fwd(const float* x, const void* w6, const float* scale, const float* shift,
+                                                  const float* disp, float* out, int B, int Cin, int Cout, int H, int W,
+                                                  long long in_bstride, long long in_cstride, void* stream) {
+  IG p;
+  if (int rc = x6s_params(p, "deconv2d_k4s2_unet_upsample", B, Cin, Cout, 1, H, W, XS_T4, 0, 0.f, in_bstride, in_cstride, 0, 0)) return rc;
+  TS_REQUIRE(Cout >= 9 && Cout <= 16, TS_ERR_UNSUPPORTED, "deconv2d_k4s2_unet_upsample: %d output channels (nine logits, one channel group)", Cout);
+  TS_REQUIRE(H % 2 == 0 && W % 2 == 0, TS_ERR_UNSUPPORTED, "deconv2d_k4s2_unet_upsample: the disparity is half the input's size (H=%d W=%d)", H, W);
+  TS_REQUIRE_PTR(x); TS_REQUIRE_PTR(w6); TS_REQUIRE_PTR(disp); TS_REQUIRE_PTR(out);
+  UnetUp ep;
+  ep.disp = disp; ep.out = out; ep.h = H / 2; ep.w = W / 2;
+  ep.sh = p.Ho > 1 ? static_cast<float>(ep.h - 1) / static_cast<float>(p.Ho - 1) : 0.f;
+  ep.sw = p.Wo > 1 ? static_cast<float>(ep.w - 1) / static_cast<float>(p.Wo - 1) : 0.f;
+  p.tiles_x = (W + 31) / 32;
+  p.co_groups = 1;
+  using G = XG<XS_T4, 4>;
+  constexpr size_t main_b = (static_cast<size_t>(3) * G::NPIXP + 3 * G::NSLOT * 16 + 1) * 16;
+  constexpr size_t epi_b = (static_cast<size_t>(16) * G::EPI + (4 / 2 + 5) * 21) * 4;
+  constexpr size_t lds = main_b > epi_b ? main_b : epi_b;
+  const dim3 grid(((H + 3) / 4) * p.tiles_x, 1, B);
+  hipLaunchKernelGGL((ig_conv_x6s_kernel<XS_T4, 1, 4, UnetUp>), grid, dim3(256), lds, ts::as_stream(stream), x,
+                     static_cast<const u32x4*>(w6), scale, shift, static_cast<float*>(nullptr), p, ep);
+  return ts::launched("ig_conv_x6s_kernel<UnetUp>");
+}
diff --git a/temporalstereo_amd/csrc/plan.hip b/temporalstereo_amd/csrc/plan.hip
--- a/temporalstereo_amd/csrc/plan.hip
+++ b/temporalstereo_amd/csrc/plan.hip
@@ -98,6 +98,8 @@
     TS_PLAN_OP(ts_spp3d_pool_fwd),          TS_PLAN_OP(ts_spp3d_pool_bwd),
     TS_PLAN_OP(ts_spp3d_expand_fwd),        TS_PLAN_OP(ts_spp3d_expand_bwd),        TS_PLAN_OP(ts_depth_sum3_fwd),
     TS_PLAN_OP(ts_bn_small_train_bwd),
+    TS_PLAN_OP(ts_regress_convex_upsample_fwd), TS_PLAN_OP(ts_topk_softargmax_half_fwd),
+    TS_PLAN_OP(ts_deconv2d_k4s2_unet_upsample_fwd),
 };
 
 struct Call {
diff --git a/temporalstereo_amd/csrc/pyramid_ops.hip b/temporalstereo_amd/csrc/pyramid_ops.hip
--- a/temporalstereo_amd/csrc/pyramid_ops.hip
+++ b/temporalstereo_amd/csrc/pyramid_ops.hip
@@ -1,3 +1,4 @@
+#include "regress_tails.hpp"
 #include "ts_common.hpp"
 
 namespace {
@@ -22,12 +23,7 @@
 
 unsigned exact_grid(long long n) { return static_cast<unsigned>((n + 255) / 256); }
 
-__device__ __forceinline__ void lin_src(float scale, int dst, int in_size, int& i0, int& i1, float& l1) {
-  const float s = scale * static_cast<float>(dst);
-  i0 = static_cast<int>(s);
-  i1 = i0 + ((i0 < in_size - 1) ? 1 : 0);
-  l1 = s - static_cast<float>(i0);
-}
+using ts_tail::lin_src;
 
 inline float ac_scale(int in_size, int out_size) {
   return out_size > 1 ? static_cast<float>(in_size - 1) / static_cast<float>(out_size - 1) : 0.f;
@@ -222,32 +218,18 @@
     const int y = oy / r, ry = oy - y * r, x = ox / r, rx = ox - x * r;
     const float* mp = mask + (static_cast<size_t>(b) * 9 * r * r + ry * r + rx) * HW + static_cast<size_t>(y) * W + x;
     const float* dp = disp + static_cast<size_t>(b) * HW;
-    float m[9], mx = -INFINITY;
-#pragma unroll
-    for (int k = 0; k < 9; ++k) { m[k] = mp[static_cast<size_t>(k) * r * r * HW]; mx = fmaxf(mx, m[k]); }
-    float den = 0.f, acc = 0.f;
-#pragma unroll
-    for (int k = 0; k < 9; ++k) {
-      const float e = expf(m[k] - mx);
-      den += e;
+    float m[9];
+    const float mx = ts_tail::convex_logits(mp, static_cast<size_t>(r) * r * HW, m);
+    const float dup = ts_tail::convex_combine(m, mx, [&](int k) {
       const int yy = y + k / 3 - 1, xx = x + k % 3 - 1;
       const float dv = dp[min(max(yy, 0), H - 1) * W + min(max(xx, 0), W - 1)];
-      const float v = (yy >= 0 && yy < H && xx >= 0 && xx < W) ? dv * disp_scale : 0.f;
-      acc += e * v;
-    }
-    const float dup = acc / den;
+      return ts_tail::convex_tap_value(dv, yy >= 0 && yy < H && xx >= 0 && xx < W, disp_scale);
+    });
     out[i] = dup;
     if (low) {
-      const float lo = dup - range, hi = dup + range;
-      low[i] = lo; high[i] = hi;
-      const float span = fabsf(hi - lo), base = fminf(lo, hi);
       const size_t HWo = static_cast<size_t>(Ho) * Wo;
-      float* c = cand + (static_cast<size_t>(b) * ctot + coff) * HWo + static_cast<size_t>(oy) * Wo + ox;
-      c[0] = span * 0.f + base;
-      c[HWo] = span * 0.375f + base;
-      c[2 * HWo] = span * 0.5f + base;
-      c[3 * HWo] = span * 0.625f + base;
-      c[4 * HWo] = span * 1.f + base;
+      ts_tail::convex_store_range(dup, range, low + i, high + i,
+                                  cand + (static_cast<size_t>(b) * ctot + coff) * HWo + static_cast<size_t>(oy) * Wo + ox, HWo);
     }
   }
 }
@@ -292,11 +274,7 @@
 #pragma unroll
     for (int r = 0; r < 4; ++r)
 #pragma unroll
-      for (int c = 0; c < 4 + XS; ++c) {
-        const int yy = y0 - 1 + r, xx = xb - 1 + c;
-        const float dv = dp[min(max(yy, 0), h - 1) * w + min(max(xx, 0), w - 1)];
-        P[r][c] = (yy >= 0 && yy < h && xx >= 0 && xx < w) ? dv * static_cast<float>(Wo) / static_cast<float>(w) : 0.f;
-      }
+      for (int c = 0; c < 4 + XS; ++c) P[r][c] = ts_tail::unet_patch_value(dp, y0 - 1 + r, xb - 1 + c, h, w, Wo);
     float res[V];
 #pragma unroll
     for (int v = 0; v < V; ++v) {
@@ -315,31 +293,12 @@
 #pragma unroll
         for (int r = 0; r < 4; ++r)
 #pragma unroll
-          for (int c = 0; c < 4; ++c) {
-            const int yy = y0 - 1 + r, xx = x0 - 1 + c;
-            const float dv = dp[min(max(yy, 0), h - 1) * w + min(max(xx, 0), w - 1)];
-            pd[r][c] = (yy >= 0 && yy < h && xx >= 0 && xx < w) ? dv * static_cast<float>(Wo) / static_cast<float>(w) : 0.f;
-          }
+          for (int c = 0; c < 4; ++c) pd[r][c] = ts_tail::unet_patch_value(dp, y0 - 1 + r, x0 - 1 + c, h, w, Wo);
       }
-      float mx = -INFINITY;
-#pragma unroll
-      for (int k = 0; k < 9; ++k) mx = fmaxf(mx, m[k][v]);
-      const bool ix = x1 > x0;
-      float den = 0.f, acc = 0.f;
-#pragma unroll
-      for (int k = 0; k < 9; ++k) {
-        const float e = expf(m[k][v] - mx);
-        den += e;
-        const int ry = k / 3, rx = k % 3;
-        const float a00 = pd[ry][rx];
-        const float a01 = ix ? pd[ry][rx + 1] : a00;
-        const float a10 = iy ? pd[ry + 1][rx] : a00;
-        const float a11 = iy ? (ix ? pd[ry + 1][rx + 1] : pd[ry + 1][rx]) : a01;
-        const float top = (1.f - lx) * a00 + lx * a01;
-        const float bot = (1.f - lx) * a10 + lx * a11;
-        acc += e * ((1.f - ly) * top + ly * bot);
-      }
-      res[v] = acc / den;
+      float mv[9];
+#pragma unroll
+      for (int k = 0; k < 9; ++k) mv[k] = m[k][v];
+      res[v] = ts_tail::unet_combine(mv, pd, lx, ly, x1 > x0, iy);
     }
     float* op = out + static_cast<size_t>(b) * HWo + static_cast<size_t>(oy) * Wo + oxv;
     if constexpr (V == 4) *reinterpret_cast<float4*>(op) = make_float4(res[0], res[1], res[2], res[3]);
@@ -386,9 +345,7 @@
     lin_src(sh, oy, h, y0, y1, ly);
     lin_src(sw, ox, w, xa, xb, lx);
     const float* p = x + static_cast<size_t>(bc) * h * w;
-    const float top = (1.f - lx) * p[y0 * w + xa] + lx * p[y0 * w + xb];
-    const float bot = (1.f - lx) * p[y1 * w + xa] + lx * p[y1 * w + xb];
-    out[i] = ((1.f - ly) * top + ly * bot) * vscale;
+    out[i] = ts_tail::bilinear_value(p[y0 * w + xa], p[y0 * w + xb], p[y1 * w + xa], p[y1 * w + xb], ly, lx, vscale);
   }
 }
 
diff --git a/temporalstereo_amd/csrc/regress.hip b/temporalstereo_amd/csrc/regress.hip
--- a/temporalstereo_amd/csrc/regress.hip
+++ b/temporalstereo_amd/csrc/regress.hip
@@ -1,3 +1,4 @@
+#include "regress_tails.hpp"
 #include "ts_common.hpp"
 
 namespace {
@@ -15,39 +16,13 @@
     const int b = static_cast<int>(i / HW);
     const int p = static_cast<int>(i - static_cast<long long>(b) * HW);
     const size_t base = static_cast<size_t>(b) * D * HW + p;
-    float bc[K];
+    float bc[K], td[K];
     int bi[K];
-#pragma unroll
-    for (int j = 0; j < K; ++j) { bc[j] = -INFINITY; bi[j] = -1; }
-    for (int d0 = 0; d0 < D; d0 += 8) {
-      float cc[8];
-#pragma unroll
-      for (int u = 0; u < 8; ++u) cc[u] = cost[base + static_cast<size_t>(min(d0 + u, D - 1)) * HW];
-#pragma unroll
-      for (int u = 0; u < 8; ++u) {
-        float c = cc[u];
-        int ci = d0 + u;
-        const bool real = ci < D;
-#pragma unroll
-        for (int j = 0; j < K; ++j) {
-          const bool take = real && ((c > bc[j]) || (bi[j] < 0));
-          const float tc = bc[j];
-          const int ti = bi[j];
-          if (take) { bc[j] = c; bi[j] = ci; c = tc; ci = ti; }
-        }
-      }
-    }
-    float w[K], den = 0.f;
-#pragma unroll
-    for (int j = 0; j < K; ++j) { w[j] = expf(bc[j] - bc[0]); den += w[j]; }
-    float acc = 0.f;
+    const float acc = ts_tail::topk_softargmax_pixel<K>(cost + base, samp + base, off + base, D, HW, bc, bi, td);
 #pragma unroll
     for (int j = 0; j < K; ++j) {
-      const size_t o = base + static_cast<size_t>(bi[j]) * HW;
-      const float td = samp[o] + off[o];
-      acc += (w[j] / den) * td;
       const size_t ko = (static_cast<size_t>(b) * K + j) * HW + p;
-      tdisp[ko] = td;
+      tdisp[ko] = td[j];
       tcost[ko] = bc[j];
       if (tidx) tidx[ko] = bi[j];
     }
@@ -91,6 +66,125 @@
       if (gsamp) gsamp[o] = g * pj + (gtd ? gtd[ko] : 0.f);
     }
   }
+}
+
+constexpr int RT = 8;
+
+template <int K>
+__global__ void __launch_bounds__(256)
+regress_convex_upsample_fwd(const float* __restrict__ cost, const float* __restrict__ samp, const float* __restrict__ off,
+                            const float* __restrict__ mask, float* __restrict__ out, float* __restrict__ low,
+                            float* __restrict__ high, float* __restrict__ cand, int D, int H, int W, int r, float disp_scale,
+                            float range, int coff, int ctot) {
+  constexpr int HT = RT + 2;
+  __shared__ float sd[HT * HT];
+  const int tiles_x = (W + RT - 1) / RT;
+  const int ty0 = static_cast<int>(blockIdx.x / tiles_x) * RT, tx0 = static_cast<int>(blockIdx.x % tiles_x) * RT;
+  const int b = blockIdx.y;
+  const int HW = H * W, Ho = H * r, Wo = W * r;
+  const int E = RT * r, n_out = E * E;
+  const size_t kstride = static_cast<size_t>(r) * r * HW;
+  const float* mb = mask + static_cast<size_t>(b) * 9 * kstride;
+  auto place = [&](int t, int& oy, int& ox, int& y, int& x, const float*& mp) {
+    const int ly = t / E, lx = t - ly * E;
+    oy = ty0 * r + ly; ox = tx0 * r + lx;
+    y = oy / r; x = ox / r;
+    const int ry = oy - y * r, rx = ox - x * r;
+    mp = mb + static_cast<size_t>(ry * r + rx) * HW + static_cast<size_t>(y) * W + x;
+    return t < n_out && oy < Ho && ox < Wo;
+  };
+  float m[9], mx = 0.f;
+  int oy, ox, y, x;
+  const float* mp;
+  bool ok = place(threadIdx.x, oy, ox, y, x, mp);
+  if (ok) mx = ts_tail::convex_logits(mp, kstride, m);
+  for (int q = threadIdx.x; q < HT * HT; q += blockDim.x) {
+    const int hy = ty0 - 1 + q / HT, hx = tx0 - 1 + q % HT;
+    float d = 0.f;
+    if (hy >= 0 && hy < H && hx >= 0 && hx < W) {
+      const size_t base = static_cast<size_t>(b) * D * HW + static_cast<size_t>(hy) * W + hx;
+      float bc[K], td[K];
+      int bi[K];
+      d = ts_tail::topk_softargmax_pixel<K>(cost + base, samp + base, off + base, D, HW, bc, bi, td);
+    }
+    sd[q] = d;
+  }
+  __syncthreads();
+  const size_t HWo = static_cast<size_t>(Ho) * Wo;
+  for (int t = threadIdx.x; t < n_out; t += blockDim.x) {
+    if (t != static_cast<int>(threadIdx.x)) {
+      ok = place(t, oy, ox, y, x, mp);
+      if (ok) mx = ts_tail::convex_logits(mp, kstride, m);
+    }
+    if (!ok) continue;
+    const float dup = ts_tail::convex_combine(m, mx, [&](int k) {
+      const int yy = y + k / 3 - 1, xx = x + k % 3 - 1;
+      const float dv = sd[(yy - ty0 + 1) * HT + (xx - tx0 + 1)];
+      return ts_tail::convex_tap_value(dv, yy >= 0 && yy < H && xx >= 0 && xx < W, disp_scale);
+    });
+    const size_t o = static_cast<size_t>(b) * HWo + static_cast<size_t>(oy) * Wo + ox;
+    out[o] = dup;
+    ts_tail::convex_store_range(dup, range, low + o, high + o,
+                                cand + (static_cast<size_t>(b) * ctot + coff) * HWo + static_cast<size_t>(oy) * Wo + ox, HWo);
+  }
+}
+
+constexpr int HQ = 8, HF = 2 * HQ + 1;
+
+template <int K>
+__global__ void __launch_bounds__(320)
+topk_softargmax_half_fwd(const float* __restrict__ cost, const float* __restrict__ samp, const float* __restrict__ off,
+                         float* __restrict__ disp, float* __restrict__ mem_s, float* __restrict__ mem_c, int D, int H, int W,
+                         float sh, float sw, float vs0, float vs1) {
+  __shared__ float s_td[K][HF * HF], s_tc[K][HF * HF];
+  const int Ho = H / 2, Wo = W / 2, HW = H * W;
+  const int tiles_x = (Wo + HQ - 1) / HQ;
+  const int oy0 = static_cast<int>(blockIdx.x / tiles_x) * HQ, ox0 = static_cast<int>(blockIdx.x % tiles_x) * HQ;
+  const int b = blockIdx.y;
+  for (int q = threadIdx.x; q < HF * HF; q += blockDim.x) {
+    const int ly = q / HF, lx = q - ly * HF;
+    const int y = 2 * oy0 + ly, x = 2 * ox0 + lx;
+    float bc[K], td[K];
+    int bi[K];
+#pragma unroll
+    for (int j = 0; j < K; ++j) { bc[j] = 0.f; td[j] = 0.f; }
+    if (y < H && x < W) {
+      const size_t base = static_cast<size_t>(b) * D * HW + static_cast<size_t>(y) * W + x;
+      const float acc = ts_tail::topk_softargmax_pixel<K>(cost + base, samp + base, off + base, D, HW, bc, bi, td);
+      if (ly < 2 * HQ && lx < 2 * HQ) disp[static_cast<size_t>(b) * HW + static_cast<size_t>(y) * W + x] = acc;
+    }
+#pragma unroll
+    for (int j = 0; j < K; ++j) { s_td[j][q] = td[j]; s_tc[j][q] = bc[j]; }
+  }
+  __syncthreads();
+  for (int t = threadIdx.x; t < HQ * HQ * K * 2; t += blockDim.x) {
+    const int lxo = t % HQ;
+    int r = t / HQ;
+    const int lyo = r % HQ;
+    r /= HQ;
+    const int j = r % K, which = r / K;
+    const int oy = oy0 + lyo, ox = ox0 + lxo;
+    if (oy >= Ho || ox >= Wo) continue;
+    int y0, y1, xa, xb;
+    float ly, lx;
+    ts_tail::lin_src(sh, oy, H, y0, y1, ly);
+    ts_tail::lin_src(sw, ox, W, xa, xb, lx);
+    y0 = min(max(y0 - 2 * oy0, 0), HF - 1); y1 = min(max(y1 - 2 * oy0, 0), HF - 1);
+    xa = min(max(xa - 2 * ox0, 0), HF - 1); xb = min(max(xb - 2 * ox0, 0), HF - 1);
+    const float* s = which ? s_tc[j] : s_td[j];
+    const float v = ts_tail::bilinear_value(s[y0 * HF + xa], s[y0 * HF + xb], s[y1 * HF + xa], s[y1 * HF + xb], ly, lx, which ? vs1 : vs0);
+    (which ? mem_c : mem_s)[((static_cast<size_t>(b) * K + j) * Ho + oy) * Wo + ox] = v;
+  }
+}
+
+bool half_resize_in_reach(int in_size, int out_size) {
+  const float scale = out_size > 1 ? static_cast<float>(in_size - 1) / static_cast<float>(out_size - 1) : 0.f;
+  for (int o = 0; o < out_size; ++o) {
+    const int i0 = static_cast<int>(scale * static_cast<float>(o));
+    const int i1 = i0 + ((i0 < in_size - 1) ? 1 : 0);
+    if (i0 < 2 * o || i1 > 2 * o + 2) return false;
+  }
+  return true;
 }
 
 struct Partial { float m, s, ws; };
@@ -238,6 +332,54 @@
   return ts::launched("topk_softargmax_fwd");
 }
 
+extern "C" int ts_regress_convex_upsample_fwd(const float* cost, const float* sample, const float* offset, const float* mask,
+                                              float* out, float* low, float* high, float* candidates, int B, int D, int H, int W,
+                                              int k, int factor, float disp_scale, float range, int channel_offset,
+                                              int channels_total, void* stream) {
+  if (int rc = check_bdhw(B, D, H, W, "regress_convex_upsample")) return rc;
+  TS_REQUIRE(k >= 1 && k <= KMAX && k <= D, TS_ERR_UNSUPPORTED, "regress_convex_upsample: k=%d outside 1..min(%d, D)", k, KMAX);
+  TS_REQUIRE(factor >= 1, TS_ERR_SHAPE, "regress_convex_upsample: bad factor");
+  TS_REQUIRE(channel_offset >= 0 && channel_offset + 5 <= channels_total, TS_ERR_SHAPE, "regress_convex_upsample: bad channel slice");
+  TS_REQUIRE(factor <= 8 && B <= 65535 && static_cast<long long>(H) * W * factor * factor < (1ll << 31), TS_ERR_UNSUPPORTED,
+             "regress_convex_upsample: factor, batch or upsampled plane too large");
+  TS_REQUIRE_PTR(cost); TS_REQUIRE_PTR(sample); TS_REQUIRE_PTR(offset); TS_REQUIRE_PTR(mask);
+  TS_REQUIRE_PTR(out); TS_REQUIRE_PTR(low); TS_REQUIRE_PTR(high); TS_REQUIRE_PTR(candidates);
+  const dim3 grid(static_cast<unsigned>(((H + RT - 1) / RT) * ((W + RT - 1) / RT)), static_cast<unsigned>(B));
+  hipStream_t st = ts::as_stream(stream);
+#define TS_CASE(KK)                                                                                                       \
+  case KK:                                                                                                                \
+    hipLaunchKernelGGL(regress_convex_upsample_fwd<KK>, grid, dim3(256), 0, st, cost, sample, offset, mask, out, low, high, \
+                       candidates, D, H, W, factor, disp_scale, range, channel_offset, channels_total);                   \
+    break;
+  switch (k) { TS_CASE(1) TS_CASE(2) TS_CASE(3) TS_CASE(4) TS_CASE(5) TS_CASE(6) TS_CASE(7) TS_CASE(8) }
+#undef TS_CASE
+  return ts::launched("regress_convex_upsample_fwd");
+}
+
+extern "C" int ts_topk_softargmax_half_fwd(const float* cost, const float* sample, const float* offset, float* disp,
+                                           float* mem_sample, float* mem_cost, int B, int D, int H, int W, int k, void* stream) {
+  if (int rc = check_bdhw(B, D, H, W, "topk_softargmax_half")) return rc;
+  TS_REQUIRE(k >= 1 && k <= KMAX && k <= D, TS_ERR_UNSUPPORTED, "topk_softargmax_half: k=%d outside 1..min(%d, D)", k, KMAX);
+  TS_REQUIRE(H % 2 == 0 && W % 2 == 0, TS_ERR_UNSUPPORTED, "topk_softargmax_half: odd size %d x %d", H, W);
+  TS_REQUIRE(B <= 65535 && half_resize_in_reach(H, H / 2) && half_resize_in_reach(W, W / 2), TS_ERR_UNSUPPORTED,
+             "topk_softargmax_half: batch or size beyond the tile's reach");
+  TS_REQUIRE_PTR(cost); TS_REQUIRE_PTR(sample); TS_REQUIRE_PTR(offset);
+  TS_REQUIRE_PTR(disp); TS_REQUIRE_PTR(mem_sample); TS_REQUIRE_PTR(mem_cost);
+  const int Ho = H / 2, Wo = W / 2;
+  const float sh = Ho > 1 ? static_cast<float>(H - 1) / static_cast<float>(Ho - 1) : 0.f;
+  const float sw = Wo > 1 ? static_cast<float>(W - 1) / static_cast<float>(Wo - 1) : 0.f;
+  const dim3 grid(static_cast<unsigned>(((Ho + HQ - 1) / HQ) * ((Wo + HQ - 1) / HQ)), static_cast<unsigned>(B));
+  hipStream_t st = ts::as_stream(stream);
+#define TS_CASE(KK)                                                                                                     \
+  case KK:                                                                                                              \
+    hipLaunchKernelGGL(topk_softargmax_half_fwd<KK>, grid, dim3(320), 0, st, cost, sample, offset, disp, mem_sample,     \
+                       mem_cost, D, H, W, sh, sw, 0.5f, 1.f);                                                            \
+    break;
+  switch (k) { TS_CASE(1) TS_CASE(2) TS_CASE(3) TS_CASE(4) TS_CASE(5) TS_CASE(6) TS_CASE(7) TS_CASE(8) }
+#undef TS_CASE
+  return ts::launched("topk_softargmax_half_fwd");
+}
+
 extern "C" int ts_topk_softargmax_bwd(const float* topk_disp, const float* topk_cost, const int* topk_index,
                                       const float* disp, const float* grad_disp, const float* grad_topk_disp,
                                       const float* grad_topk_cost, float* grad_cost, float* grad_sample,
diff --git a/temporalstereo_amd/csrc/regress_tails.hpp b/temporalstereo_amd/csrc/regress_tails.hpp
--- /dev/null
+++ b/temporalstereo_amd/csrc/regress_tails.hpp
@@ -0,0 +1,116 @@
+#pragma once
+#include <hip/hip_runtime.h>
+
+namespace ts_tail {
+
+__device__ __forceinline__ void lin_src(float scale, int dst, int in_size, int& i0, int& i1, float& l1) {
+  const float s = scale * static_cast<float>(dst);
+  i0 = static_cast<int>(s);
+  i1 = i0 + ((i0 < in_size - 1) ? 1 : 0);
+  l1 = s - static_cast<float>(i0);
+}
+
+template <int K>
+__device__ __forceinline__ float topk_softargmax_pixel(const float* __restrict__ cost, const float* __restrict__ samp,
+                                                       const float* __restrict__ off, int D, int HW, float (&bc)[K], int (&bi)[K],
+                                                       float (&td)[K]) {
+#pragma unroll
+  for (int j = 0; j < K; ++j) { bc[j] = -INFINITY; bi[j] = -1; }
+  for (int d0 = 0; d0 < D; d0 += 8) {
+    float cc[8];
+#pragma unroll
+    for (int u = 0; u < 8; ++u) cc[u] = cost[static_cast<size_t>(min(d0 + u, D - 1)) * HW];
+#pragma unroll
+    for (int u = 0; u < 8; ++u) {
+      float c = cc[u];
+      int ci = d0 + u;
+      const bool real = ci < D;
+#pragma unroll
+      for (int j = 0; j < K; ++j) {
+        const bool take = real && ((c > bc[j]) || (bi[j] < 0));
+        const float tc = bc[j];
+        const int ti = bi[j];
+        if (take) { bc[j] = c; bi[j] = ci; c = tc; ci = ti; }
+      }
+    }
+  }
+  float w[K], den = 0.f;
+#pragma unroll
+  for (int j = 0; j < K; ++j) { w[j] = expf(bc[j] - bc[0]); den += w[j]; }
+  float acc = 0.f;
+#pragma unroll
+  for (int j = 0; j < K; ++j) {
+    const size_t o = static_cast<size_t>(bi[j]) * HW;
+    td[j] = samp[o] + off[o];
+    acc += (w[j] / den) * td[j];
+  }
+  return acc;
+}
+
+__device__ __forceinline__ float convex_logits(const float* __restrict__ mp, size_t kstride, float (&m)[9]) {
+  float mx = -INFINITY;
+#pragma unroll
+  for (int k = 0; k < 9; ++k) { m[k] = mp[static_cast<size_t>(k) * kstride]; mx = fmaxf(mx, m[k]); }
+  return mx;
+}
+
+template <class Tap>
+__device__ __forceinline__ float convex_combine(const float (&m)[9], float mx, Tap tap) {
+  float den = 0.f, acc = 0.f;
+#pragma unroll
+  for (int k = 0; k < 9; ++k) {
+    const float e = expf(m[k] - mx);
+    den += e;
+    const float v = tap(k);
+    acc += e * v;
+  }
+  return acc / den;
+}
+
+__device__ __forceinline__ float convex_tap_value(float dv, bool inside, float disp_scale) { return inside ? dv * disp_scale : 0.f; }
+
+__device__ __forceinline__ void convex_store_range(float dup, float range, float* __restrict__ low, float* __restrict__ high,
+                                                   float* __restrict__ c, size_t HWo) {
+  const float lo = dup - range, hi = dup + range;
+  *low = lo; *high = hi;
+  const float span = fabsf(hi - lo), base = fminf(lo, hi);
+  c[0] = span * 0.f + base;
+  c[HWo] = span * 0.375f + base;
+  c[2 * HWo] = span * 0.5f + base;
+  c[3 * HWo] = span * 0.625f + base;
+  c[4 * HWo] = span * 1.f + base;
+}
+
+__device__ __forceinline__ float unet_patch_value(const float* __restrict__ dp, int yy, int xx, int h, int w, int Wo) {
+  const float dv = dp[min(max(yy, 0), h - 1) * w + min(max(xx, 0), w - 1)];
+  return (yy >= 0 && yy < h && xx >= 0 && xx < w) ? dv * static_cast<float>(Wo) / static_cast<float>(w) : 0.f;
+}
+
+__device__ __forceinline__ float unet_combine(const float (&m)[9], const float (&pd)[4][4], float lx, float ly, bool ix, bool iy) {
+  float mx = -INFINITY;
+#pragma unroll
+  for (int k = 0; k < 9; ++k) mx = fmaxf(mx, m[k]);
+  float den = 0.f, acc = 0.f;
+#pragma unroll
+  for (int k = 0; k < 9; ++k) {
+    const float e = expf(m[k] - mx);
+    den += e;
+    const int ry = k / 3, rx = k % 3;
+    const float a00 = pd[ry][rx];
+    const float a01 = ix ? pd[ry][rx + 1] : a00;
+    const float a10 = iy ? pd[ry + 1][rx] : a00;
+    const float a11 = iy ? (ix ? pd[ry + 1][rx + 1] : pd[ry + 1][rx]) : a01;
+    const float top = (1.f - lx) * a00 + lx * a01;
+    const float bot = (1.f - lx) * a10 + lx * a11;
+    acc += e * ((1.f - ly) * top + ly * bot);
+  }
+  return acc / den;
+}
+
+__device__ __forceinline__ float bilinear_value(float v00, float v01, float v10, float v11, float ly, float lx, float vscale) {
+  const float top = (1.f - lx) * v00 + lx * v01;
+  const float bot = (1.f - lx) * v10 + lx * v11;
+  return ((1.f - ly) * top + ly * bot) * vscale;
+}
+
+}
diff --git a/temporalstereo_amd/csrc/ts_common.hpp b/temporalstereo_amd/csrc/ts_common.hpp
--- a/temporalstereo_amd/csrc/ts_common.hpp
+++ b/temporalstereo_amd/csrc/ts_common.hpp
@@ -9,7 +9,7 @@
 
 #include "../../include/ts_hip.h"
 
-#define TS_ABI_VERSION 18
+#define TS_ABI_VERSION 19
 
 namespace ts {
 
```
